# martin-velas/SLAM_plus_plus

Measured on AMD Instinct MI355X. Metric: Lambda solve GFLOP/s (algorithmic factor+solve flops / wall-clock), 100k-pose SE(3), higher is better.
Workload: dtype f64; 1 GPU; C3: synthetic 100000-pose SE(3) chain + loop closures, 6x6 blocks, 201998 upper blocks, n=600000; numeric factor + 2 substitutions per step (symbolic analysis cached, inputs resident in HBM); parallelism=1 GPU

## Files before the change

slam_plus_plus_amd/csrc/simt_factor_ahead.hip:

```cpp
#include <hip/hip_runtime.h>
#include "sparse_kernels.h"

#include <algorithm>

namespace slampp {

#include "simt_device.inl"

template <int D, int AHEAD>
struct TFactorAheadSet {
	double d[D][D];
	double b[D];
	double c[AHEAD][D / 2][D];
};

template <int D, int AHEAD>
constexpr int factor_ahead_fetch_loads()
{
	int n = D / 2;
	for(int r = 0; r < D; ++ r)
		n += r / 2 + 1;
	return n + AHEAD * (D / 2) * D;
}
template <int D> constexpr int factor_ahead_half_block_stores() { return D * ((D / 2) / 2 + (D / 2) % 2); }
template <int D> constexpr int factor_ahead_diagonal_stores() { return D / 2 + (D / 2) * (D / 2); }
template <int D> constexpr int factor_ahead_newer_stores() { return (factor_ahead_half_block_stores<D>() < factor_ahead_diagonal_stores<D>())? factor_ahead_half_block_stores<D>() : factor_ahead_diagonal_stores<D>(); }

template <int D, int AHEAD>
__device__ __forceinline__ void factor_ahead_pin(TFactorAheadSet<D, AHEAD> &s)
{
	#pragma unroll
	for(int r = 0; r < D; ++ r) {
		#pragma unroll
		for(int q = 0; q < 2 * (r / 2 + 1); ++ q)
			asm volatile("" : "+a"(s.d[r][q]));
		asm volatile("" : "+a"(s.b[r]));
	}
	#pragma unroll
	for(int k = 0; k < AHEAD; ++ k) {
		#pragma unroll
		for(int i = 0; i < D / 2; ++ i) {
			#pragma unroll
			for(int q = 0; q < D; ++ q)
				asm volatile("" : "+a"(s.c[k][i][q]));
		}
	}
}

template <int D, int W, int AHEAD>
__device__ __forceinline__ void factor_ahead_fetch(TFactorAheadSet<D, AHEAD> &s, int ci, int n_blk, int nb, int f_blk, int r0, const long long *T,
	const double *__restrict__ A, const double *__restrict__ b)
{
	{
		const long long enc = T[W * (f_blk + n_blk)];
		long long n_off = (enc < 0)? 0 : (enc >> 1);
		asm volatile("" : "+v"(n_off));
		const double *src = A + n_off;
		#pragma unroll
		for(int r = 0; r < D; ++ r) {
			#pragma unroll
			for(int i = 0; i <= r / 2; ++ i) {
				const double2 t = *reinterpret_cast<const double2*>(src + r * D + 2 * i);
				s.d[r][2 * i] = t.x;
				s.d[r][2 * i + 1] = t.y;
			}
		}
		load_column<D>(b + T[W * (4 * ci + 3)], s.b);
	}
	#pragma unroll
	for(int k = 0; k < AHEAD; ++ k) {
		const bool b_exists = k + 1 < nb;
		const long long enc = T[W * (f_blk + n_blk + (b_exists? k + 1 : 0))];
		const bool b_trans = b_exists && enc >= 0 && (enc & 1) != 0;
		long long n_off = (b_exists && enc >= 0)? (enc >> 1) : 0;
		int n_row_stride = b_trans? D : 1, n_col_stride = b_trans? 1 : D;
		asm volatile("" : "+v"(n_off), "+v"(n_row_stride), "+v"(n_col_stride));
		const double *src = A + n_off + r0 * n_row_stride;
		#pragma unroll
		for(int i = 0; i < D / 2; ++ i) {
			#pragma unroll
			for(int q = 0; q < D; ++ q)
				s.c[k][i][q] = src[i * n_row_stride + q * n_col_stride];
		}
	}
	asm volatile("" ::: "memory");
}

template <int D>
__device__ __forceinline__ void store_half_columns(double *p, const double (&m)[D][D], int n_half)
{
	double *p_out = p + n_half * (D / 2) * D;
	#pragma unroll
	for(int q = 0; q < D / 2; ++ q) {
		#pragma unroll
		for(int r = 0; r < D; r += 2)
			*reinterpret_cast<double2*>(p_out + r + q * D) = double2{n_half? m[r][q + D / 2] : m[r][q], n_half? m[r + 1][q + D / 2] : m[r + 1][q]};
	}
}

__device__ __forceinline__ void factor_ahead_stage_table(long long *p_dst, const long long *__restrict__ p_src, int n_entries, int n_lane)
{
	enum { N_FLIGHT = 8 };
	for(int n_base = 0; n_base < n_entries; n_base += N_FLIGHT * 64) {
		long long v[N_FLIGHT];
		#pragma unroll
		for(int u = 0; u < N_FLIGHT; ++ u) {
			const int i = n_base + u * 64 + n_lane;
			v[u] = p_src[(i < n_entries)? i : n_entries - 1];
		}
		#pragma unroll
		for(int u = 0; u < N_FLIGHT; ++ u) {
			const int i = n_base + u * 64 + n_lane;
			if(i < n_entries)
				p_dst[i] = v[u];
		}
	}
}

template <int D, int W, bool b_linv, int AHEAD>
__device__ __forceinline__ bool factor_ahead_columns(const int32_t *P, const long long *T, const int n_half, const double *__restrict__ A, double *L, double *Linv,
	const double *__restrict__ b, double *w, long long *p_tm, int &n_tm)
{
	enum { DD = D * D, DH = D / 2 };
	const int r0 = n_half * DH;
	const int n_cols = P[0], n_blocks = P[1], n_ops = P[2];
	const int f_blk = 4 * n_cols, f_op = f_blk + n_blocks, f_y = f_op + n_ops;
	int pc = 4, blk0 = 0;
	bool b_bad = false;
	TFactorAheadSet<D, AHEAD> t_set;
	factor_ahead_fetch<D, W, AHEAD>(t_set, 0, 0, P[pc], f_blk, r0, T, A, b);
	__builtin_amdgcn_s_waitcnt(simt_wait_imm(0));
	factor_ahead_pin<D, AHEAD>(t_set);
	for(int ci = 0; ci < n_cols; ++ ci) {
		const int nb = P[pc], nr = P[pc + 1], n_touch = P[pc + 2];
		pc += 3;
		pc += n_touch;
		const long long l_base = T[W * (4 * ci)], linv_off = T[W * (4 * ci + 1)], cs_new = T[W * (4 * ci + 2)];
		__builtin_amdgcn_s_waitcnt(simt_wait_imm(factor_ahead_newer_stores<D>()));
		factor_ahead_pin<D, AHEAD>(t_set);
		double a[D][D], y[D], acc[AHEAD][DH][D];
		{
			const long long enc = T[W * (f_blk + blk0)];
			#pragma unroll
			for(int r = 0; r < D; ++ r) {
				#pragma unroll
				for(int q = 0; q < D; ++ q)
					a[r][q] = (q <= r && enc >= 0)? t_set.d[r][q] : 0.0;
			}
			#pragma unroll
			for(int r = 0; r < D; ++ r)
				y[r] = t_set.b[r];
			#pragma unroll
			for(int k = 0; k < AHEAD; ++ k) {
				const bool b_have = k + 1 < nb && T[W * (f_blk + blk0 + ((k + 1 < nb)? k + 1 : 0))] >= 0;
				#pragma unroll
				for(int i = 0; i < DH; ++ i) {
					#pragma unroll
					for(int q = 0; q < D; ++ q)
						acc[k][i][q] = b_have? t_set.c[k][i][q] : 0.0;
				}
			}
		}
		simt_row_entries<D, W>(a, y, pc, nr, f_op, f_y, P, T, L, w);
		SIMT_TICK();
		if(ci + 1 < n_cols) {
			asm volatile("" ::: "memory");
			factor_ahead_fetch<D, W, AHEAD>(t_set, ci + 1, blk0 + nb, P[pc_next_column(P, pc, nb, 0)], f_blk, r0, T, A, b);
		}
		double x[D][D];
		simt_cholesky_inverse<D>(a, x, b_bad);
		{
			double yn[D];
			simt_forward_substitution<D>(yn, a, x, y);
			#pragma unroll
			for(int r = 0; r < D; r += 2)
				*reinterpret_cast<double2*>(w + cs_new + r) = double2{yn[r], yn[r + 1]};
			store_half_columns<D>(L + l_base, a, n_half);
			if constexpr(b_linv)
				store_half_columns<D>(Linv + linv_off, x, n_half);
		}
		SIMT_TICK();
		#pragma unroll
		for(int k = 0; k < AHEAD; ++ k) {
			if(k + 1 < nb) {
				const int np = P[pc ++];
				simt_update_pairs<D, W, 2>(acc[k], pc, np, f_op, r0, P, T, L);
				simt_block_product<D, 2>(acc[k], x, r0, L + l_base + (k + 1) * DD);
				SIMT_TICK();
			}
		}
		for(int kb = AHEAD + 1; kb < nb; ++ kb) {
			const int np = P[pc ++];
			double acc_more[DH][D];
			simt_load_lambda_block<D, 2>(acc_more, T[W * (f_blk + blk0 + kb)], r0, A);
			simt_update_pairs<D, W, 2>(acc_more, pc, np, f_op, r0, P, T, L);
			simt_block_product<D, 2>(acc_more, x, r0, L + l_base + kb * DD);
			SIMT_TICK();
		}
		blk0 += nb;
	}
	return b_bad;
}

template <int D, int W, int LPT, bool b_linv, int AHEAD>
__global__ void __launch_bounds__(64)
factor_simt_kernel_ahead(const TSimtChunk *__restrict__ chunks, const int32_t *__restrict__ prog, const long long *__restrict__ tab,
	const double *__restrict__ A, double *L, double *Linv, const double *__restrict__ b, double *w, int *p_flag,
	long long *p_timing, TBatch t_batch)
{	{ const int64_t n_member = blockIdx.y; A += n_member * t_batch.a; L += n_member * t_batch.l; Linv = Linv? Linv + n_member * t_batch.linv : Linv; b += n_member * t_batch.b; w += n_member * t_batch.w; p_flag += n_member; }

	static_assert(LPT == 2 && D % 2 == 0 && AHEAD >= 1, "two lanes per task, even block sizes");
	enum { DD = D * D, DH = D / 2 };
	extern __shared__ long long s_tab[];
	const TSimtChunk ch = chunks[blockIdx.x];
	{
		const int n_entries = (4 * prog[ch.prog_off] + prog[ch.prog_off + 1] + prog[ch.prog_off + 2] + prog[ch.prog_off + 3]) * W;
		factor_ahead_stage_table(s_tab, tab + ch.tab_off, n_entries, int(threadIdx.x));
		__syncthreads();
	}
	if(int(threadIdx.x) >= W * LPT)
		return;
	const int n_half = int(threadIdx.x) & 1;
	int n_tm = 0;
	long long *p_tm = simt_timing_begin(p_timing, n_tm);
	const bool b_bad = factor_ahead_columns<D, W, b_linv, AHEAD>(prog + ch.prog_off, s_tab + threadIdx.x / LPT, n_half, A, L, Linv, b, w, p_tm, n_tm);
	if(b_bad)
		atomicOr(p_flag, 1);
}

template <int D, int W, bool b_linv, int AHEAD>
__global__ void __launch_bounds__(128)
factor_simt_kernel_branches(const TSimtBranchGroup *__restrict__ groups, const int32_t *__restrict__ prog, const long long *__restrict__ tab,
	const double *__restrict__ A, double *L, double *Linv, const double *__restrict__ b, double *w, int *p_flag,
	long long *p_timing, TBatch t_batch, int n_region)
{	{ const int64_t n_member = blockIdx.y; A += n_member * t_batch.a; L += n_member * t_batch.l; Linv = Linv? Linv + n_member * t_batch.linv : Linv; b += n_member * t_batch.b; w += n_member * t_batch.w; p_flag += n_member; }

	static_assert(D % 2 == 0 && AHEAD >= 1 && W * 2 <= 64, "two lanes per task, even block sizes");
	extern __shared__ long long s_tab[];
	const int n_wave = __builtin_amdgcn_readfirstlane(int(threadIdx.x) >> 6), n_lane = int(threadIdx.x) & 63;
	long long *s_mine = s_tab + n_wave * n_region;
	int n_tm = 0;
	long long *p_tm = simt_timing_begin(p_timing, n_tm);
	bool b_bad = false;
	for(int n_pass = 0; n_pass < 2; ++ n_pass) {
		const TSimtChunk ch = groups[blockIdx.x].seg[n_pass? 2 : n_wave];
		if(ch.n_tasks > 0 && (n_pass == 0 || n_wave == 0)) {
			const int32_t *P = prog + ch.prog_off;
			const int n_entries = (4 * P[0] + P[1] + P[2] + P[3]) * W;
			factor_ahead_stage_table(s_mine, tab + ch.tab_off, n_entries, n_lane);
			__builtin_amdgcn_fence(__ATOMIC_ACQ_REL, "workgroup");
			__builtin_amdgcn_wave_barrier();
			if(n_lane < W * 2) {
				const bool b_bad_here = factor_ahead_columns<D, W, b_linv, AHEAD>(P, s_mine + n_lane / 2, n_lane & 1, A, L, Linv, b, w, p_tm, n_tm);
				b_bad = b_bad || b_bad_here;
			}
		}
		if(n_pass == 0)
			__syncthreads();
	}
	if(b_bad)
		atomicOr(p_flag, 1);
}

template <int W>
static const void *p_Factor_Branches_Kernel(bool b_store_linv)
{
	return b_store_linv? reinterpret_cast<const void*>(&factor_simt_kernel_branches<6, W, true, SIMT_FACTOR_AHEAD>) :
		reinterpret_cast<const void*>(&factor_simt_kernel_branches<6, W, false, SIMT_FACTOR_AHEAD>);
}

static const void *p_Factor_Branches_Kernel(int n_dim, int n_width, bool b_store_linv)
{
	if(n_dim != 6)
		return 0;
	return (n_width == 16)? p_Factor_Branches_Kernel<16>(b_store_linv) : (n_width == 32)? p_Factor_Branches_Kernel<32>(b_store_linv) : 0;
}

bool factor_simt_branches_exists(int n_dim, int n_width)
{
	return p_Factor_Branches_Kernel(n_dim, n_width, false) != 0;
}

int factor_simt_branches_groups(int n_dim, int n_width, int n_lds_bytes)
{
	if(!factor_simt_branches_exists(n_dim, n_width) || n_lds_bytes <= 0)
		return 0;
	return std::min(simt_resident_workgroups(p_Factor_Branches_Kernel(n_dim, n_width, false), 128, n_lds_bytes),
		simt_resident_workgroups(p_Factor_Branches_Kernel(n_dim, n_width, true), 128, n_lds_bytes));
}

bool launch_factor_simt_branches(const TSimtBranchGroup *groups, int n_groups, int n_width, int n_lds_bytes, const int32_t *prog, const int64_t *tab, int n_dim,
	const double *A, double *L, double *Linv, const double *b, double *w, int *p_flag, hipStream_t stream, long long *p_timing, const TBatch &t_batch)
{
	if(!factor_simt_branches_exists(n_dim, n_width) || n_groups <= 0 || n_lds_bytes <= 0 || n_lds_bytes % 16 != 0)
		return false;
	const long long *t = reinterpret_cast<const long long*>(tab);
	const int n_region = n_lds_bytes / 16;
#define BRANCHES_LAUNCH(W_, b_linv_) hipLaunchKernelGGL((factor_simt_kernel_branches<6, W_, b_linv_, SIMT_FACTOR_AHEAD>), dim3(n_groups, t_batch.n), dim3(128), n_lds_bytes, stream, \
	groups, prog, t, A, L, Linv, b, w, p_flag, p_timing, t_batch, n_region)
	if(n_width == 16) {
		if(Linv) BRANCHES_LAUNCH(16, true); else BRANCHES_LAUNCH(16, false);
	} else {
		if(Linv) BRANCHES_LAUNCH(32, true); else BRANCHES_LAUNCH(32, false);
	}
#undef BRANCHES_LAUNCH
	return true;
}

template <int W>
static const void *p_Factor_Ahead_Kernel(bool b_store_linv)
{
	return b_store_linv? reinterpret_cast<const void*>(&factor_simt_kernel_ahead<6, W, 2, true, SIMT_FACTOR_AHEAD>) :
		reinterpret_cast<const void*>(&factor_simt_kernel_ahead<6, W, 2, false, SIMT_FACTOR_AHEAD>);
}

static const void *p_Factor_Ahead_Kernel(int n_dim, int n_width, bool b_store_linv)
{
	if(n_dim != 6)
		return 0;
	return (n_width == 16)? p_Factor_Ahead_Kernel<16>(b_store_linv) : (n_width == 32)? p_Factor_Ahead_Kernel<32>(b_store_linv) : 0;
}

bool factor_simt_ahead_exists(int n_dim, int n_width)
{
	return p_Factor_Ahead_Kernel(n_dim, n_width, false) != 0;
}

int factor_simt_ahead_waves(int n_dim, int n_width, int n_lds_bytes)
{
	if(!factor_simt_ahead_exists(n_dim, n_width))
		return 0;
	return std::min(simt_resident_workgroups(p_Factor_Ahead_Kernel(n_dim, n_width, false), 64, n_lds_bytes),
		simt_resident_workgroups(p_Factor_Ahead_Kernel(n_dim, n_width, true), 64, n_lds_bytes));
}

bool launch_factor_simt_ahead(const TSimtChunk *chunks, int n_chunks, int n_width, int n_lds_bytes, const int32_t *prog, const int64_t *tab, int n_dim,
	const double *A, double *L, double *Linv, const double *b, double *w, int *p_flag, hipStream_t stream, long long *p_timing, const TBatch &t_batch)
{
	if(!factor_simt_ahead_exists(n_dim, n_width))
		return false;
	const long long *t = reinterpret_cast<const long long*>(tab);
#define AHEAD_LAUNCH(W_, b_linv_) hipLaunchKernelGGL((factor_simt_kernel_ahead<6, W_, 2, b_linv_, SIMT_FACTOR_AHEAD>), dim3(n_chunks, t_batch.n), dim3(64), n_lds_bytes, stream, \
	chunks, prog, t, A, L, Linv, b, w, p_flag, p_timing, t_batch)
	if(n_width == 16) {
		if(Linv) AHEAD_LAUNCH(16, true); else AHEAD_LAUNCH(16, false);
	} else {
		if(Linv) AHEAD_LAUNCH(32, true); else AHEAD_LAUNCH(32, false);
	}
#undef AHEAD_LAUNCH
	return true;
}

}

#include "preload.h"
SLAMPP_PRELOAD_UNIT(simt_factor_ahead)
```

slam_plus_plus_amd/csrc/simt_kernel.hip:

```cpp
#include <hip/hip_runtime.h>
#include "sparse_kernels.h"

#include <algorithm>
#include <cstdio>

namespace slampp {

#include "simt_device.inl"

template <int D, int W, int LPT, bool b_linv>
__global__ void __launch_bounds__(64)
factor_simt_kernel(const TSimtChunk *__restrict__ chunks, const int32_t *__restrict__ prog, const long long *__restrict__ tab,
	const double *__restrict__ A, double *L, double *Linv, const double *__restrict__ b, double *w, int *p_flag,
	long long *p_timing, TBatch t_batch)
{	{ const int64_t n_member = blockIdx.y; A += n_member * t_batch.a; L += n_member * t_batch.l; Linv = Linv? Linv + n_member * t_batch.linv : Linv; b += n_member * t_batch.b; w += n_member * t_batch.w; p_flag += n_member; }

	enum { DD = D * D };
	extern __shared__ long long s_tab[];
	const TSimtChunk ch = chunks[blockIdx.x];
	{
		const int n_entries = (4 * prog[ch.prog_off] + prog[ch.prog_off + 1] + prog[ch.prog_off + 2] + prog[ch.prog_off + 3]) * W;
		for(int i = threadIdx.x; i < n_entries; i += 64)
			s_tab[i] = tab[ch.tab_off + i];
		__syncthreads();
	}
	if(int(threadIdx.x) >= W * LPT)
		return;
	const int n_half = (LPT == 2)? int(threadIdx.x) & 1 : 0;
	enum { DH = (LPT == 2)? D / 2 : D };
	const int r0 = n_half * DH;
	int n_tm = 0;
	long long *p_tm = simt_timing_begin(p_timing, n_tm);
	const int32_t *P = prog + ch.prog_off;
	const long long *T = s_tab + threadIdx.x / LPT;
	const int n_cols = P[0], n_blocks = P[1], n_ops = P[2];
	const int f_blk = 4 * n_cols, f_op = f_blk + n_blocks, f_y = f_op + n_ops;
	int pc = 4, blk0 = 0;
	bool b_bad = false;
	double f_touched = 0;
	for(int ci = 0; ci < n_cols; ++ ci) {
		const int nb = P[pc], nr = P[pc + 1], n_touch = P[pc + 2];
		pc += 3;
		pc += n_touch;
		if(ci + 1 < n_cols) {
			const int nb_next = P[pc_next_column(P, pc, nb, nr)];
			for(int kb = 0; kb < nb_next; ++ kb) {
				const long long enc = T[W * (f_blk + blk0 + nb + kb)];
				const double *p_src = A + ((enc < 0)? 0 : (enc >> 1));
				f_touched += p_src[0] + p_src[16] + p_src[DD - 1];
			}
		}
		const long long l_base = T[W * (4 * ci)], linv_off = T[W * (4 * ci + 1)], cs_new = T[W * (4 * ci + 2)],
			cs_src = T[W * (4 * ci + 3)];
		double a[D][D], y[D];
		{
			const long long enc = T[W * (f_blk + blk0)];
			const double *src = A + ((enc < 0)? 0 : (enc >> 1));
			#pragma unroll
			for(int r = 0; r < D; ++ r) {
				double c[D];
				load_column<D>(src + r * D, c);
				#pragma unroll
				for(int q = 0; q < D; ++ q)
					a[r][q] = (q <= r && enc >= 0)? c[q] : 0.0;
			}
			load_column<D>(b + cs_src, y);
		}
		simt_row_entries<D, W>(a, y, pc, nr, f_op, f_y, P, T, L, w);
		SIMT_TICK();
		double x[D][D];
		simt_cholesky_inverse<D>(a, x, b_bad);
		{
			double yn[D];
			simt_forward_substitution<D>(yn, a, x, y);
			if(n_half == 0) {
				#pragma unroll
				for(int r = 0; r < D; ++ r)
					w[cs_new + r] = yn[r];
				store_block<D>(L + l_base, a);
				if constexpr(b_linv)
					store_block<D>(Linv + linv_off, x);
			}
		}
		SIMT_TICK();
		for(int kb = 1; kb < nb; ++ kb) {
			const int np = P[pc ++];
			double acc[DH][D];
			simt_load_lambda_block<D, LPT>(acc, T[W * (f_blk + blk0 + kb)], r0, A);
			simt_update_pairs<D, W, LPT>(acc, pc, np, f_op, r0, P, T, L);
			double *p_out = L + l_base + kb * DD;
			if constexpr(D % 2 == 0)
				simt_block_product<D, LPT>(acc, x, r0, p_out);
			else {
				static_assert(LPT == 1, "odd D: one lane per task, the lane has all D rows of the block");
				#pragma unroll
				for(int q = 0; q < D; ++ q) {
					double out[D];
					#pragma unroll
					for(int r = 0; r < D; ++ r) {
						double sum = 0;
						#pragma unroll
						for(int t = 0; t <= q; ++ t)
							sum += acc[r][t] * x[q][t];
						out[r] = sum;
					}
					#pragma unroll
					for(int r = 0; r < D; ++ r)
						p_out[r + q * D] = out[r];
				}
			}
			SIMT_TICK();
		}
		blk0 += nb;
	}
	if(b_bad || f_touched == 1.2345e301)
		atomicOr(p_flag, 1);
}

bool launch_factor_simt(const TSimtChunk *chunks, int n_chunks, int n_width, int n_lds_bytes, const int32_t *prog, const int64_t *tab, int n_dim,
	const double *A, double *L, double *Linv, const double *b, double *w, int *p_flag, hipStream_t stream, long long *p_timing, const TBatch &t_batch,
	int n_ahead_waves, const TSimtBranchLaunch *p_branches)
{
	if(n_chunks <= 0)
		return true;
	const long long *t = reinterpret_cast<const long long*>(tab);
#define SIMT_LAUNCH(D_, W_, LPT_) do { if(Linv) hipLaunchKernelGGL((factor_simt_kernel<D_, W_, LPT_, true>), dim3(n_chunks, t_batch.n), dim3(64), n_lds_bytes, stream, chunks, prog, t, \
	A, L, Linv, b, w, p_flag, p_timing, t_batch); else hipLaunchKernelGGL((factor_simt_kernel<D_, W_, LPT_, false>), dim3(n_chunks, t_batch.n), dim3(64), n_lds_bytes, stream, chunks, prog, t, \
	A, L, Linv, b, w, p_flag, p_timing, t_batch); } while(0)
#define SIMT_WIDTHS(D_) do { if(n_width == 16) { if(b_pairs && D_ % 2 == 0) SIMT_LAUNCH(D_, 16, (D_ % 2 == 0)? 2 : 1); else SIMT_LAUNCH(D_, 16, 1); } \
	else if(n_width == 32) { if(b_pairs && D_ % 2 == 0) SIMT_LAUNCH(D_, 32, (D_ % 2 == 0)? 2 : 1); else SIMT_LAUNCH(D_, 32, 1); } \
	else SIMT_LAUNCH(D_, 64, 1); } while(0)
	const int n_pairs_env = dev_knob("SLAMPP_HIP_DEV_SIMT_PAIRS", -1);
	const bool b_pairs = (n_pairs_env >= 0)? n_pairs_env != 0 : n_chunks <= 2048;
	const int n_ahead_env = dev_knob("SLAMPP_HIP_DEV_SIMT_FACTOR_AHEAD", -1);
	const int n_lpt = (b_pairs && n_dim % 2 == 0 && (n_width == 16 || n_width == 32))? 2 : 1;
	const bool b_ahead = n_lpt == 2 && factor_simt_ahead_exists(n_dim, n_width) &&
		((n_ahead_env >= 0)? n_ahead_env != 0 : int64_t(n_chunks) * std::max<int64_t>(t_batch.n, 1) <= n_ahead_waves);
	const int n_branches_env = dev_knob("SLAMPP_HIP_DEV_SIMT_FACTOR_BRANCHES", -1);
	const bool b_branches = p_branches && p_branches->n_groups > 0 && n_lpt == 2 && factor_simt_branches_exists(n_dim, n_width) &&
		((n_branches_env >= 0)? n_branches_env != 0 : b_ahead && int64_t(p_branches->n_groups) * std::max<int64_t>(t_batch.n, 1) <= p_branches->n_round_groups &&
		p_branches->n_tstar < p_branches->n_longest_task && p_branches->n_stage_tasks >= 2048);
	if(b_branches) {
		if(p_timing)
			fprintf(stderr, "stage_timing lane-per-task factor branches launch: %d workgroups of two waves, %d split chunks, %d whole chunks, width %d, block size %d, %d members\n",
				p_branches->n_groups, p_branches->n_split_chunks, p_branches->n_whole_chunks, n_width, n_dim, int(t_batch.n));
		return launch_factor_simt_branches(p_branches->groups, p_branches->n_groups, n_width, p_branches->n_lds_bytes, prog, tab, n_dim, A, L, Linv, b, w, p_flag,
			stream, p_timing, t_batch);
	}
	if(p_timing)
		fprintf(stderr, "stage_timing lane-per-task factor launch: %d chunks, width %d, block size %d, %d members, LPT %d, %s\n", n_chunks, n_width, n_dim,
			int(t_batch.n), n_lpt, b_ahead? "fetch ahead" : "fetch by column");
	if(b_ahead)
		return launch_factor_simt_ahead(chunks, n_chunks, n_width, n_lds_bytes, prog, tab, n_dim, A, L, Linv, b, w, p_flag, stream, p_timing, t_batch);
	switch(n_dim) {
	case 3:
		SIMT_WIDTHS(3);
		return true;
	case 6:
		SIMT_WIDTHS(6);
		return true;
	case 7:
		SIMT_WIDTHS(7);
		return true;
	default:
		return false;
	}
#undef SIMT_WIDTHS
#undef SIMT_LAUNCH
}

template <int D, int W>
__global__ void __launch_bounds__(64)
backward_simt_kernel(const TSimtChunk *__restrict__ chunks, const int32_t *__restrict__ prog, const long long *__restrict__ tab,
	const double *__restrict__ L, double *w, double *x_out, TBatch t_batch)
{	{ const int64_t n_member = blockIdx.y; L += n_member * t_batch.l; w += n_member * t_batch.w; x_out += n_member * t_batch.b; }

	enum { DD = D * D };
	extern __shared__ long long s_tab[];
	const TSimtChunk ch = chunks[blockIdx.x];
	const int32_t *P = prog + ch.prog_off;
	const int n_cols = P[0], n_below = P[1];
	{
		const int n_entries = (3 * n_cols + n_below) * W;
		for(int i = threadIdx.x; i < n_entries; i += 64)
			s_tab[i] = tab[ch.tab_off + i];
		__syncthreads();
	}
	if(int(threadIdx.x) >= W)
		return;
	const long long *T = s_tab + threadIdx.x;
	double *s_x = reinterpret_cast<double*>(s_tab + (3 * n_cols + n_below) * W) + threadIdx.x;
	const int32_t *p_local = P + 2 + n_cols;
	int n_blk_end = n_below;
	double f_touched = 0;
	for(int ci = n_cols - 1; ci >= 0; -- ci) {
		const int nb = P[2 + ci];
		const long long l_base = T[W * (3 * ci)], cs_new = T[W * (3 * ci + 1)], cs_src = T[W * (3 * ci + 2)];
		const int n_blk0 = n_blk_end - (nb - 1);
		double acc[D], a[D][D];
		load_column<D>(w + cs_new, acc);
		load_block<D>(L + l_base, a);
		asm volatile("" ::: "memory");
		double f_touch_now = 0;
		if(ci > 1 || (ci == n_cols - 1 && ci > 0)) {
			const int c_first = (ci > 1)? ci - 2 : ci - 1, c_last = (ci == n_cols - 1)? ci - 1 : c_first;
			for(int c = c_last; c >= c_first; -- c) {
				const int nb_next = P[2 + c];
				const double *p_next = L + T[W * (3 * c)];
				for(int kb = 0; kb < nb_next; ++ kb)
					f_touch_now += p_next[kb * DD] + p_next[kb * DD + 16] + p_next[kb * DD + DD - 1];
			}
		}
		asm volatile("" ::: "memory");
		double rd[D];
		#pragma unroll
		for(int q = 0; q < D; ++ q)
			rd[q] = simt_refined_rcp(a[q][q]);
		for(int kb = 1; kb < nb; ++ kb) {
			const long long xcs = T[W * (3 * n_cols + n_blk0 + kb - 1)];
			const int n_local = p_local[n_blk0 + kb - 1];
			double c[D][D], xi[D];
			load_block<D>(L + l_base + kb * DD, c);
			if(n_local >= 0)
				simt_local_x<D, W>(xi, s_x, n_local);
			else
				load_column<D>(w + xcs, xi);
			simt_backward_block<D>(acc, c, xi);
		}
		double x[D];
		simt_solve_transposed<D>(x, acc, a, rd);
		simt_store_local_x<D, W>(s_x, ci, x);
		f_touched += f_touch_now;
		simt_store_x<D>(w + cs_new, x_out + cs_src, x);
		n_blk_end = n_blk0;
	}
	if(f_touched == 1.2345e301)
		w[0] = f_touched;
}

template <int D, int AHEAD>
struct TBwdAheadSet {
	double y[D], a[D][D], c[AHEAD][D][D], xs[D];
	int nb, n_blk0;
	int n_xk;
	int n_local[AHEAD];
};

template <int D, int W, int AHEAD>
__device__ __forceinline__ void bwd_ahead_fetch(TBwdAheadSet<D, AHEAD> &s, int ci, int n_blk_end, int n_cols, const int32_t *P, const int32_t *p_local,
	const long long *T, const double *__restrict__ L, const double *w)
{
	enum { DD = D * D };
	s.nb = P[2 + ci];
	const long long l_base = T[W * (3 * ci)];
	s.n_blk0 = n_blk_end - (s.nb - 1);
	load_column<D>(w + T[W * (3 * ci + 1)], s.y);
	load_lower<D>(L + l_base, s.a);
	s.n_xk = -1;
	int n_x_field = 3 * ci + 1;
	#pragma unroll
	for(int k = 0; k < AHEAD; ++ k) {
		const bool b_have = k + 1 < s.nb;
		s.n_local[k] = b_have? p_local[s.n_blk0 + k] : 0;
		if(b_have && s.n_local[k] < 0 && s.n_xk < 0) {
			s.n_xk = k;
			n_x_field = 3 * n_cols + s.n_blk0 + k;
		}
		int n_blk_off = b_have? (k + 1) * DD : 0;
		asm volatile("" : "+s"(n_blk_off));
		load_block<D>(L + l_base + n_blk_off, s.c[k]);
	}
	asm volatile("" : "+s"(n_x_field));
	load_column<D>(w + T[W * n_x_field], s.xs);
	asm volatile("" ::: "memory");
}

template <int D, int AHEAD>
constexpr int bwd_ahead_fetch_loads()
{
	if(D % 2 != 0)
		return D + D * (D + 1) / 2 + AHEAD * (D * D) + D;
	int n = D / 2;
	for(int q = 0; q < D; ++ q)
		n += (D - (q & ~1)) / 2;
	return n + AHEAD * (D * D / 2) + D / 2;
}
template <int D> constexpr int bwd_ahead_solve_stores() { return (D % 2 == 0)? D : 2 * D; }

template <int D, int W, int AHEAD, int N_NEWER >
__device__ __forceinline__ void bwd_ahead_solve(TBwdAheadSet<D, AHEAD> &s, int ci, int n_cols, const int32_t *p_local, const long long *T, double *s_x,
	const double *__restrict__ L, double *w, double *x_out)
{
	enum { DD = D * D };
	__builtin_amdgcn_s_waitcnt(simt_wait_imm(N_NEWER));
	#pragma unroll
	for(int q = 0; q < D; ++ q)
		s.a[q][q] = simt_refined_rcp(s.a[q][q]);
	double acc[D];
	#pragma unroll
	for(int q = 0; q < D; ++ q)
		acc[q] = s.y[q];
	#pragma unroll
	for(int k = 0; k < AHEAD; ++ k) {
		if(k + 1 < s.nb) {
			double xi[D];
			if(s.n_local[k] >= 0)
				simt_local_x<D, W>(xi, s_x, s.n_local[k]);
			else if(s.n_xk == k) {
				#pragma unroll
				for(int r = 0; r < D; ++ r)
					xi[r] = s.xs[r];
			} else {
				load_column<D>(w + T[W * (3 * n_cols + s.n_blk0 + k)], xi);
				__builtin_amdgcn_s_waitcnt(simt_wait_imm(0));
			}
			simt_backward_block<D>(acc, s.c[k], xi);
		}
	}
	const long long l_base = (s.nb > AHEAD + 1)? T[W * (3 * ci)] : 0;
	for(int kb = AHEAD + 1; kb < s.nb; kb += AHEAD) {
		double xr[AHEAD][D];
		#pragma unroll
		for(int i = 0; i < AHEAD; ++ i) {
			if(kb + i < s.nb) {
				load_block<D>(L + l_base + (kb + i) * DD, s.c[i]);
				const int n_local = p_local[s.n_blk0 + kb + i - 1];
				if(n_local >= 0)
					simt_local_x<D, W>(xr[i], s_x, n_local);
				else
					load_column<D>(w + T[W * (3 * n_cols + s.n_blk0 + kb + i - 1)], xr[i]);
			}
		}
		asm volatile("" ::: "memory");
		__builtin_amdgcn_s_waitcnt(simt_wait_imm(0));
		#pragma unroll
		for(int i = 0; i < AHEAD; ++ i) {
			if(kb + i < s.nb)
				simt_backward_block<D>(acc, s.c[i], xr[i]);
		}
	}
	double x[D];
	#pragma unroll
	for(int q = D - 1; q >= 0; -- q) {
		double sum = acc[q];
		#pragma unroll
		for(int r = q + 1; r < D; ++ r)
			sum -= s.a[q][r] * x[r];
		x[q] = sum * s.a[q][q];
	}
	simt_store_local_x<D, W>(s_x, ci, x);
	const long long cs_new = T[W * (3 * ci + 1)], cs_src = T[W * (3 * ci + 2)];
	simt_store_x<D>(w + cs_new, x_out + cs_src, x);
}

template <int D, int W, int AHEAD>
__global__ void __launch_bounds__(64)
backward_simt_ahead_kernel(const TSimtChunk *__restrict__ chunks, const int32_t *__restrict__ prog, const long long *__restrict__ tab,
	const double *__restrict__ L, double *w, double *x_out, TBatch t_batch)
{	{ const int64_t n_member = blockIdx.y; L += n_member * t_batch.l; w += n_member * t_batch.w; x_out += n_member * t_batch.b; }

	extern __shared__ long long s_tab[];
	const TSimtChunk ch = chunks[blockIdx.x];
	const int32_t *P = prog + ch.prog_off;
	const int n_cols = P[0], n_below = P[1];
	{
		const int n_entries = (3 * n_cols + n_below) * W;
		for(int i = threadIdx.x; i < n_entries; i += 64)
			s_tab[i] = tab[ch.tab_off + i];
		__syncthreads();
	}
	if(int(threadIdx.x) >= W)
		return;
	const long long *T = s_tab + threadIdx.x;
	double *s_x = reinterpret_cast<double*>(s_tab + (3 * n_cols + n_below) * W) + threadIdx.x;
	const int32_t *p_local = P + 2 + n_cols;
	TBwdAheadSet<D, AHEAD> t_even, t_odd;
	enum { N_FETCH = bwd_ahead_fetch_loads<D, AHEAD>(), N_STORES = bwd_ahead_solve_stores<D>() };
	int ci = n_cols - 1;
	bwd_ahead_fetch<D, W, AHEAD>(t_even, ci, n_below, n_cols, P, p_local, T, L, w);
	for(; ci >= 2; ci -= 2) {
		bwd_ahead_fetch<D, W, AHEAD>(t_odd, ci - 1, t_even.n_blk0, n_cols, P, p_local, T, L, w);
		bwd_ahead_solve<D, W, AHEAD, N_FETCH>(t_even, ci, n_cols, p_local, T, s_x, L, w, x_out);
		bwd_ahead_fetch<D, W, AHEAD>(t_even, ci - 2, t_odd.n_blk0, n_cols, P, p_local, T, L, w);
		bwd_ahead_solve<D, W, AHEAD, N_STORES + N_FETCH>(t_odd, ci - 1, n_cols, p_local, T, s_x, L, w, x_out);
	}
	if(ci == 1) {
		bwd_ahead_fetch<D, W, AHEAD>(t_odd, 0, t_even.n_blk0, n_cols, P, p_local, T, L, w);
		bwd_ahead_solve<D, W, AHEAD, N_FETCH>(t_even, 1, n_cols, p_local, T, s_x, L, w, x_out);
		bwd_ahead_solve<D, W, AHEAD, N_STORES>(t_odd, 0, n_cols, p_local, T, s_x, L, w, x_out);
	} else
		bwd_ahead_solve<D, W, AHEAD, 0>(t_even, 0, n_cols, p_local, T, s_x, L, w, x_out);
}

template <int D> struct TBwdAheadDim { enum { b_have = (D == 6) }; };

template <int D, int W>
static const void *p_Backward_Ahead_Kernel()
{
	if constexpr(TBwdAheadDim<D>::b_have)
		return reinterpret_cast<const void*>(&backward_simt_ahead_kernel<D, W, SIMT_BWD_AHEAD>);
	else
		return 0;
}

static const void *p_Backward_Ahead_Kernel(int n_dim, int n_width)
{
#define BWD_AHEAD_WIDTHS(D_) return (n_width == 16)? p_Backward_Ahead_Kernel<D_, 16>() : (n_width == 32)? p_Backward_Ahead_Kernel<D_, 32>() : p_Backward_Ahead_Kernel<D_, 64>()
	switch(n_dim) {
	case 3:
		BWD_AHEAD_WIDTHS(3);
	case 6:
		BWD_AHEAD_WIDTHS(6);
	case 7:
		BWD_AHEAD_WIDTHS(7);
	default:
		return 0;
	}
#undef BWD_AHEAD_WIDTHS
}

template <int D, int W>
static void Launch_Backward_Simt(bool b_ahead, const TSimtChunk *chunks, int n_chunks, int n_lds_bytes, const int32_t *prog, const long long *t,
	const double *L, double *w, double *x_out, hipStream_t stream, const TBatch &t_batch)
{
	if constexpr(TBwdAheadDim<D>::b_have) {
		if(b_ahead) {
			hipLaunchKernelGGL((backward_simt_ahead_kernel<D, W, SIMT_BWD_AHEAD>), dim3(n_chunks, t_batch.n), dim3(64), n_lds_bytes, stream,
				chunks, prog, t, L, w, x_out, t_batch);
			return;
		}
	}
	hipLaunchKernelGGL((backward_simt_kernel<D, W>), dim3(n_chunks, t_batch.n), dim3(64), n_lds_bytes, stream, chunks, prog, t, L, w, x_out, t_batch);
}

int backward_simt_ahead_waves(int n_dim, int n_width, int n_lds_bytes)
{
	return simt_resident_workgroups(p_Backward_Ahead_Kernel(n_dim, n_width), 64, n_lds_bytes);
}

bool launch_backward_simt(const TSimtChunk *chunks, int n_chunks, int n_width, int n_lds_bytes, size_t n_lds_limit, int n_ahead_waves, const int32_t *prog, const int64_t *tab,
	int n_dim, const double *L, double *w, double *x_out, hipStream_t stream, const TBatch &t_batch, bool b_report)
{
	if(n_chunks <= 0)
		return true;
	if(n_lds_bytes < 0 || size_t(n_lds_bytes) > n_lds_limit)
		return false;
	const long long *t = reinterpret_cast<const long long*>(tab);
	const int n_ahead_env = dev_knob("SLAMPP_HIP_DEV_SIMT_BWD_AHEAD", -1);
	const void *p_ahead = p_Backward_Ahead_Kernel(n_dim, n_width);
	const bool b_ahead = p_ahead && ((n_ahead_env >= 0)? n_ahead_env != 0 : int64_t(n_chunks) * std::max<int64_t>(t_batch.n, 1) <= n_ahead_waves);
	if(b_report)
		fprintf(stderr, "stage_timing lane-per-task backward launch: %d chunks, width %d, block size %d, %d members, %s\n", n_chunks, n_width, n_dim,
			int(t_batch.n), b_ahead? "fetch ahead" : "fetch by column");
#define BWD_LAUNCH(D_, W_) Launch_Backward_Simt<D_, W_>(b_ahead, chunks, n_chunks, n_lds_bytes, prog, t, L, w, x_out, stream, t_batch)
#define BWD_WIDTHS(D_) do { if(n_width == 16) BWD_LAUNCH(D_, 16); else if(n_width == 32) BWD_LAUNCH(D_, 32); else BWD_LAUNCH(D_, 64); } while(0)
	switch(n_dim) {
	case 3:
		BWD_WIDTHS(3);
		break;
	case 6:
		BWD_WIDTHS(6);
		break;
	case 7:
		BWD_WIDTHS(7);
		break;
	default:
		return false;
	}
#undef BWD_WIDTHS
#undef BWD_LAUNCH
	return hipGetLastError() == hipSuccess;
}

template <int D>
__global__ void invert_diagonals_kernel(TDevPlan p, int64_t col_begin, int64_t col_end, const double *__restrict__ L, double *Linv)
{
	const int64_t c = col_begin + int64_t(blockIdx.x) * blockDim.x + threadIdx.x;
	if(c >= col_end)
		return;
	const TColDesc &cd = p.cols[c];
	const double *a = L + p.blks[cd.k0].loff;
	double x[D][D];
	#pragma unroll
	for(int q = 0; q < D; ++ q) {
		#pragma unroll
		for(int r = 0; r < D; ++ r) {
			if(r < q)
				x[r][q] = 0.0;
			else {
				double sum = (r == q)? 1.0 : 0.0;
				#pragma unroll
				for(int t = q; t < r; ++ t)
					sum -= a[r + t * D] * x[t][q];
				x[r][q] = sum / a[r + r * D];
			}
		}
	}
	double *p_out = Linv + cd.linv_off;
	#pragma unroll
	for(int q = 0; q < D; ++ q) {
		#pragma unroll
		for(int r = 0; r < D; ++ r)
			p_out[r + q * D] = x[r][q];
	}
}

bool launch_invert_diagonals(const TDevPlan &p, int64_t col_begin, int64_t col_end, const double *L, double *Linv, hipStream_t stream)
{
	if(col_end <= col_begin)
		return true;
	const unsigned n_grid = unsigned((col_end - col_begin + 127) / 128);
	switch(p.uniform_dim) {
	case 3:
		hipLaunchKernelGGL((invert_diagonals_kernel<3>), dim3(n_grid), dim3(128), 0, stream, p, col_begin, col_end, L, Linv);
		return true;
	case 6:
		hipLaunchKernelGGL((invert_diagonals_kernel<6>), dim3(n_grid), dim3(128), 0, stream, p, col_begin, col_end, L, Linv);
		return true;
	case 7:
		hipLaunchKernelGGL((invert_diagonals_kernel<7>), dim3(n_grid), dim3(128), 0, stream, p, col_begin, col_end, L, Linv);
		return true;
	default:
		return false;
	}
}

}

#include "preload.h"
SLAMPP_PRELOAD_UNIT(simt_kernel)
```

slam_plus_plus_amd/csrc/solver.h:

```cpp
#pragma once
#include <hip/hip_runtime.h>
#include <chrono>
#include <cstdint>
#include <new>
#include <stdexcept>
#include <string>
#include <vector>
#include <thread>
#include <memory>
#include <mutex>

#include "../../include/slampp_hip.h"
#include "plan.h"
#include "host_pool.h"
#include "sparse_records.h"
#include <utility>
#include "sparse_kernels.h"
#include "dense_chol.h"

namespace slampp {

struct CDeviceError : public std::runtime_error {
	explicit CDeviceError(const std::string &s) :std::runtime_error(s) {}
};

#define SLAMPP_HIP_CHECK(call) do { hipError_t e_ = (call); if(e_ != hipSuccess) { \
	throw slampp::CDeviceError(std::string(#call) + ": " + hipGetErrorString(e_)); } } while(0)

extern thread_local bool g_b_keep_device_memory;

template <class T>
class CDevArray {
	T *m_p;
	size_t m_n, m_cap;
public:
	CDevArray() :m_p(0), m_n(0), m_cap(0) {}
	~CDevArray() { Release(); }
	CDevArray(const CDevArray&) = delete;
	CDevArray &operator =(const CDevArray&) = delete;
	void Release() { if(m_p) (void)hipFree(m_p); m_p = 0; m_n = 0; m_cap = 0; }
	void Free() { m_n = 0; if(!g_b_keep_device_memory) Release(); }
	void Alloc(size_t n)
	{
		if(!n)
			n = 1;
		if(n <= m_cap && m_p) {
			m_n = std::max(m_n, n);
			return;
		}
		Release();
		hipError_t e = hipMalloc((void**)&m_p, n * sizeof(T));
		if(e == hipErrorOutOfMemory || e == hipErrorMemoryAllocation) {
			(void)hipGetLastError();
			m_p = 0;
			throw std::bad_alloc();
		}
		if(e != hipSuccess) {
			m_p = 0;
			throw CDeviceError(std::string("hipMalloc: ") + hipGetErrorString(e));
		}
		m_n = m_cap = n;
	}
	template <class CAlloc>
	void Upload(const std::vector<T, CAlloc> &v, hipStream_t s)
	{
		Alloc(v.size());
		if(!v.empty())
			SLAMPP_HIP_CHECK(hipMemcpyAsync(m_p, v.data(), v.size() * sizeof(T), hipMemcpyHostToDevice, s));
	}
	T *p() const { return m_n? m_p : 0; }
	size_t n() const { return m_n; }
	size_t n_Bytes() const { return m_p? m_n * sizeof(T) : 0; }
	void Swap(CDevArray &r_other) { std::swap(m_p, r_other.m_p); std::swap(m_n, r_other.m_n); std::swap(m_cap, r_other.m_cap); }
};


struct CKeepDeviceMemory {
	bool b_before;
	CKeepDeviceMemory() :b_before(g_b_keep_device_memory) { g_b_keep_device_memory = true; }
	~CKeepDeviceMemory() { g_b_keep_device_memory = b_before; }
};

struct CSchurState;
struct CDeviceGroup;
struct CSparseInverse;
struct CCovariance;
struct CAssemblyState;
struct CMultiplyState;
struct CPatternOuterState;

}

struct slampp_hip_assembly {
	slampp_hip_solver *p_solver;
	slampp::CAssemblyState *p_state;
	bool b_stale;
	bool b_robust = false;
	slampp_hip_robust t_robust;
	slampp::CDevArray<double> d_robust_weight;
};

struct slampp_hip_solver {
	int n_device;
	hipStream_t stream;
	std::string s_error;
	slampp::PlanOptions opt;
	int n_dense_nb;
	int b_shard_primary;
	int n_shard_rank, n_shard_world;
	int n_marginals_dense;
	int n_assembly_groups = 1 << 20;
	int n_schur_tiles = -1;
	int n_schur_incremental = 0;
	int n_schur_keep = 0;
	int n_schur_sparse;

	bool b_has_structure, b_analyzed, b_factored;
	uint64_t n_factor_gen = 0, n_schur_cov_gen = 0;
	uint64_t n_schur_keep_gen = 0;
	void Factor_Installed(bool b_resolvable = true) { b_factored = b_resolvable; ++ n_factor_gen; }
	void Factor_Dropped() { Factor_Installed(false); }
	void Schur_Kept() { n_schur_keep_gen = n_factor_gen; }
	void Schur_Cov_Left() { n_schur_cov_gen = n_factor_gen; }
	slampp::CMultiplyState *p_mul = 0;
	bool b_mul_valid = false;
	int n_multiply_long_row = SLAMPP_HIP_MULTIPLY_LONG_ROW;
	slampp::CDevArray<double> d_reduce, d_refine_r, d_mul_x, d_mul_y, d_refine_resid;
	slampp::CDevArray<double> d_gram;
	void Require_Multiply();
	slampp::CPatternOuterState *p_outer = 0;
	bool b_outer_valid = false;
	slampp::CDevArray<double> d_outer_out;
	void Require_Pattern_Outer();
	slampp::CDevArray<int64_t> d_logdet_tab;
	std::vector<int64_t> logdet_tab_host;
	bool b_logdet_valid = false;
	void Require_Logdet_Table();
	int n_mode;
	int64_t n_matrix_cut;
	std::vector<int64_t> cumsum, bcol_ptr;
	std::vector<int32_t> brow;
	int64_t n_values, n_scalars;

	bool b_refined = false;
	int64_t n_refined_values = 0;
	std::vector<int64_t> refined_cumsum, refined_bcol_ptr;
	std::vector<int32_t> refined_brow;
	slampp::CDevArray<int64_t> d_refine_map;
	slampp::CDevArray<double> d_refined;
	void Refine_Structure();
	bool b_schur_fallback = false;
	int n_staging_ahead = 0;
	int n_schur_fallback_option = 1;
	slampp::Plan plan;
	slampp::SparseLaunchLists lists;
	slampp::TDevPlan dplan;
	slampp::CDevArray<slampp::TColDesc> d_cols;
	slampp::CDevArray<slampp::TBlkDesc> d_blks;
	slampp::CDevArray<slampp::TRowEnt> d_rents;
	slampp::CDevArray<longlong2> d_pairs;
	slampp::CDevArray<int64_t> d_task_ptr, d_task_pkg;
	slampp::CDevArray<longlong2> d_pkg;
	slampp::CDevArray<long long> d_timing;
	slampp::CDevArray<slampp::TSimtChunk> d_simt_chunks;
	slampp::CDevArray<int32_t> d_simt_prog, d_simt_rest;
	int n_panel = -1;
	int n_panel_rows = -1;
	slampp::CDevArray<longlong2> d_panel_pkg;
	slampp::CDevArray<int64_t> d_panel_off, d_panel_out_off;
	slampp::CDevArray<double> d_handup;
	int n_panel_handup = 1;
	slampp::CDevArray<int32_t> d_panel_rest;
	int n_panel_backward = -1;
	size_t n_lds_limit = 0;
	slampp::CDevArray<longlong2> d_bwd_rec;
	slampp::CDevArray<int64_t> d_bwd_off;
	slampp::CDevArray<slampp::TUpdSlot> d_panel_upd_slots;
	slampp::CDevArray<slampp::TUpdEnt> d_panel_upd_ents;
	slampp::CDevArray<int64_t> d_simt_tab;
	slampp::CDevArray<slampp::TSimtChunk> d_simt_bwd_chunks;
	slampp::CDevArray<int32_t> d_simt_bwd_prog;
	slampp::CDevArray<int64_t> d_simt_bwd_tab;
	std::vector<int32_t> simt_factor_ahead_waves;
	slampp::CDevArray<slampp::TSimtBranchGroup> d_simt_br_groups;
	std::vector<int32_t> simt_branches_round_groups;
	std::vector<int32_t> simt_bwd_ahead_waves;
	bool b_leaf_linv_wanted = false, b_leaf_linv_valid = true;
	slampp::TBatch t_batch = slampp::t_No_Batch();
	slampp::CDevArray<double> d_batch_L, d_batch_Linv, d_batch_w, d_batch_handup;
	slampp::CDevArray<int> d_batch_flag;
	int n_batch_owner_member = -1;
	int *p_host_batch_flag = 0;
	int n_batch_pending = 0;
	int n_simt_backward = -1;
	void Ensure_Leaf_Inverses();
	int n_simt = -1;
	int n_wide_min_tasks = 8192;
	int n_simt_width = 32;
	int n_simt_stages = 1;
	void Upload_Simt(const slampp::SparseRecords &r_rec);
	void Report_Simt_Backward(const slampp::SparseRecords &r_rec) const;
	void Report_Simt_Factor(const slampp::SparseRecords &r_rec) const;
	slampp::CDevArray<slampp::TDenseBlk> d_dense_blks;
	slampp::CDevArray<int64_t> d_dense_blk_loff;
	slampp::CDevArray<double> d_dense, d_dense_invdiag, d_dense_z, d_dense_x;
	slampp::CDevArray<int32_t> d_dense_gaps;
	int n_dense_gaps;
	slampp::CDevArray<uint8_t> d_dense_unit;
	slampp::CDevArray<longlong2> d_dense_dst;
	slampp::CTileSchedule dense_tiles;
	bool b_dense_tiles;
	bool b_dense_clean;
	int n_dense_top_tiles;
	int n_dense_blks, n_dense_cols, n_dense_dim, n_dense_pad;
	slampp::CDevArray<double> d_A, d_rhs, d_L, d_Linv, d_w, d_cov;
	slampp::CSparseInverse *p_sinv = 0;
	bool b_sinv_tried = false;
	slampp::CCovariance *p_cov = 0;
	slampp::CDevArray<double> d_Z;
	slampp::CDevArray<double> d_Zd, d_Zd_work;
	slampp::CDevArray<int64_t> d_diag_zoff;
	slampp::CDevArray<int32_t> d_diag_dim;
	slampp::CDevArray<int64_t> d_diag_out_off;
	slampp::CDevArray<int64_t> d_damp_off;
	bool b_damp_valid = false;
	bool Require_Damping_Offsets();
	slampp::CDevArray<double> d_lm_reduce;
	slampp::CDevArray<int64_t> d_state_cumsum;
	bool b_state_cumsum_valid = false;
	slampp::CDevArray<int> d_flag;
	int *p_flag_shared = 0;
	int *p_host_flag;

	double *p_pin_values = 0, *p_pin_rhs = 0;
	size_t n_pin_values = 0, n_pin_rhs = 0;
	bool b_pin_values_registered = false, b_pin_rhs_registered = false;
	bool b_pin_values_deferred = false, b_pin_rhs_deferred = false;
	bool b_staging_ever = false;
	std::thread t_staging_registration;
	void Register_Staging_Later();
	void Join_Staging_Registration();
	slampp::CTrashList analysis_trash;
	std::thread t_discard;
	void Join_Discard() { if(t_discard.joinable()) t_discard.join(); }
	std::thread t_bringup;
	std::mutex m_bringup;
	int n_bringup_status = SLAMPP_HIP_OK;
	int n_Join_Bringup()
	{
		std::lock_guard<std::mutex> t_lock(m_bringup);
		if(t_bringup.joinable()) {
			const double t0 = slampp::wall_ms();
			t_bringup.join();
			if(getenv("SLAMPP_HIP_PLAN_TIMING"))
				fprintf(stderr, "[bring-up] waited for %.2f ms\n", slampp::wall_ms() - t0);
		}
		return n_bringup_status;
	}
	void Join_Bringup()
	{
		if(n_Join_Bringup() != SLAMPP_HIP_OK)
			throw slampp::CDeviceError("the handle's streams could not be created");
	}
	hipStream_t copy_stream = 0;
	hipEvent_t copy_done = 0;
	int64_t n_uploaded = 0;
	void Require_Staging();
	void Free_Staging();
	void Upload_Values(const double *p_values);

	slampp::CSchurState *p_schur;
	slampp::CDeviceGroup *p_group = 0;
	bool b_group_active = false;
	std::vector<int> group_devices;
	std::vector<std::pair<std::string, int64_t> > group_options;
	std::vector<slampp_hip_assembly*> assemblies;

	slampp_hip_allreduce_fn p_allreduce;
	void *p_allreduce_context;
	typedef int (*TDenseFactorFn)(void *p_context, double *p_S, int n_pad, int n, double *p_invdiag, int *p_flag, void *p_hip_stream);
	TDenseFactorFn p_dense_factor = 0;
	void *p_dense_factor_context = 0;
	int n_schur_distributed = 0;

	slampp_hip_times times;

	struct TPhaseRecord { int n_label; hipEvent_t start, stop; };
	int b_profile;
	std::vector<std::string> phase_names;
	std::vector<double> phase_ms;
	std::vector<int64_t> phase_count;
	std::vector<TPhaseRecord> phase_pending;
	std::vector<hipEvent_t> event_pool;
	int n_open_phase;
	void Phase_Begin(const char *p_s_label);
	void Phase_End();
	void Phase_Collect();

	slampp_hip_solver();
	~slampp_hip_solver();
	void Free_Device(bool b_keep_multiply = false);
	size_t n_Device_Bytes() const;
	void Analyze_Sparse();
	void Enqueue_Sparse(const double *p_values_dev, double *p_rhs_dev, bool b_factor, bool b_factor_only = false);
};


namespace slampp {

void schur_destroy(CSchurState *p);
CSchurState *schur_analyze(slampp_hip_solver &s);
void schur_enqueue(slampp_hip_solver &s, const double *p_values_dev, double *p_rhs_dev);
bool schur_keeps_for_resolve(const slampp_hip_solver &s);
void schur_resolve_enqueue(slampp_hip_solver &s, double *p_rhs_dev, bool b_from_covariance);
void schur_enqueue_marginal_poses(slampp_hip_solver &s, const double *p_values_dev, double *p_rhs_dev);
void damping_enqueue(const int64_t *p_off_dim_dev, int64_t n_first, int64_t n_last, double f_alpha, double *p_values_dev,
	hipStream_t stream);
void schur_enqueue_marginals(slampp_hip_solver &s, const double *p_values_dev, double *p_cam_cov_dev, double *p_point_cov_dev);
void schur_cov_pattern_enqueue(slampp_hip_solver &s, const double *p_values_dev, double *p_cov_dev);
void schur_cov_columns_enqueue(slampp_hip_solver &s, const double *p_values_dev, int n_cols, const int64_t *p_bcols, double *p_out_dev);
void schur_cov_pairs_enqueue(slampp_hip_solver &s, const double *p_values_dev, int64_t n_pairs, const int64_t *p_brows,
	const int64_t *p_bcols, double *p_out_dev);
size_t schur_device_bytes(const CSchurState *p);
void schur_invalidate_previous(CSchurState *p);
void schur_set_changed_points(slampp_hip_solver &s, const int64_t *p_points, int64_t n_points);
void schur_fill_stats(const CSchurState *p, slampp_hip_stats &st);
bool schur_reduced_stats(const CSchurState *p, slampp_hip_stats &st);

CDeviceGroup *group_create(const int *p_device_ids, int n_devices);
void group_destroy(CDeviceGroup *p_group);
int group_set_option(CDeviceGroup &g, const char *p_s_name, int64_t n_value);
void group_analyze(slampp_hip_solver &r_front, int64_t n_cut);
int group_factor_solve(slampp_hip_solver &r_front, const double *p_values, double *p_rhs_inout);
int group_check_staging(slampp_hip_solver &r_front, double *p_values, double *p_rhs);
int group_solve_marginal_poses(slampp_hip_solver &r_front, const double *p_values, double *p_rhs_inout);
int group_schur_marginals(slampp_hip_solver &r_front, const double *p_values, double *p_cam_cov, double *p_point_cov);
int group_free_memory(CDeviceGroup &g);
void group_fill_stats(CDeviceGroup &g, slampp_hip_stats &r_stats);
const char *group_exchange_name(const CDeviceGroup &g);
int group_member_num(const CDeviceGroup &g);
int64_t group_exchange_count(const CDeviceGroup &g);
slampp_hip_solver *group_member(CDeviceGroup &g, int n_member);
void shard_bounds(int64_t n_bcols, int64_t n_cut, const int64_t *p_bcol_ptr, int n_world, std::vector<int64_t> &r_bounds);

CAssemblyState *assembly_setup(slampp_hip_solver &s, int64_t n_edges, const int64_t *v0, const int64_t *v1, int rd);
void assembly_destroy(CAssemblyState *p);
void assembly_enqueue(CAssemblyState &a, const double *J0, const double *J1, const double *Si, const double *err,
	const double *wgt, int64_t n_unary_vertex, const double *p_unary_factor, const double *p_unary_error,
	double *values_out, double *eta_out, int b_accumulate);
size_t assembly_device_bytes(const CAssemblyState *p);
struct TAsmEdgeView {
	int64_t n_edges;
	int d0, d1, rd;
	const int64_t *p_state_off0, *p_state_off1, *p_vertex0;
};
void assembly_edge_view(const CAssemblyState &a, TAsmEdgeView &r_view);

}

void Parallel_Copy(double *p_dst, const double *p_src, size_t n);
void Upload_Rhs_And_Join(slampp_hip_solver &s, const double *p_rhs);
void Upload_Values_And_Join(slampp_hip_solver &s, const double *p_values);
```

slam_plus_plus_amd/csrc/solver.hip:

```cpp
#include <execinfo.h>
#include <signal.h>
#include <unistd.h>
#include <pthread.h>
#include "solver.h"
#include <unordered_map>
#include <sys/mman.h>
#include "sparse_inverse.h"
#include "covariance.h"
#include "multiply.h"
#include "pattern_outer.h"

#include <algorithm>
#include <atomic>
#include <chrono>
#include <cstdio>
#include <cstdlib>
#include <cstring>
#include <map>
#include <thread>
#include <mutex>
#include <condition_variable>
#include <functional>
#include <sys/mman.h>

using namespace slampp;

namespace slampp {
thread_local bool g_b_keep_device_memory = false;
}

slampp_hip_solver::slampp_hip_solver()
	:n_device(0), stream(0), n_dense_nb(64), b_shard_primary(1), n_shard_rank(-1), n_shard_world(0), n_marginals_dense(0), n_schur_sparse(-1), b_has_structure(false),
	b_analyzed(false), b_factored(false), n_mode(SLAMPP_HIP_MODE_SPARSE), n_matrix_cut(0),
	n_values(0), n_scalars(0), n_dense_gaps(0), b_dense_tiles(false), b_dense_clean(false), n_dense_top_tiles(-1), n_dense_blks(0), n_dense_cols(0),
	n_dense_dim(0), n_dense_pad(0),
	p_host_flag(0), p_schur(0), p_allreduce(0), p_allreduce_context(0),
	b_profile(0), n_open_phase(-1)
{
	memset(&dplan, 0, sizeof(dplan));
	memset(&times, 0, sizeof(times));
}

slampp_hip_solver::~slampp_hip_solver()
{
	(void)n_Join_Bringup();
	Join_Discard();
	host_pool_release();
	Free_Device();
	for(size_t i = 0; i < phase_pending.size(); ++ i) {
		(void)hipEventDestroy(phase_pending[i].start);
		(void)hipEventDestroy(phase_pending[i].stop);
	}
	for(size_t i = 0; i < event_pool.size(); ++ i)
		(void)hipEventDestroy(event_pool[i]);
	if(p_host_flag)
		(void)hipHostFree(p_host_flag);
	if(p_host_batch_flag)
		(void)hipHostFree(p_host_batch_flag);
	Free_Staging();
	if(copy_done)
		(void)hipEventDestroy(copy_done);
	if(copy_stream)
		(void)hipStreamDestroy(copy_stream);
	if(stream)
		(void)hipStreamDestroy(stream);
}

void slampp_hip_solver::Free_Device(bool b_keep_multiply)
{
	d_cols.Free(); d_blks.Free(); d_rents.Free(); d_pairs.Free(); d_task_ptr.Free(); d_task_pkg.Free(); d_pkg.Free();
	d_simt_chunks.Free(); d_simt_prog.Free(); d_simt_rest.Free(); d_simt_tab.Free();
	d_simt_bwd_chunks.Free(); d_simt_bwd_prog.Free(); d_simt_bwd_tab.Free(); d_simt_br_groups.Free();
	b_leaf_linv_valid = true;
	d_panel_pkg.Free(); d_panel_off.Free(); d_panel_out_off.Free(); d_handup.Free(); d_panel_rest.Free(); d_bwd_rec.Free(); d_bwd_off.Free(); d_panel_upd_slots.Free(); d_panel_upd_ents.Free();
	lists = SparseLaunchLists();
	d_dense_blks.Free(); d_dense_blk_loff.Free(); d_dense.Free(); d_dense_invdiag.Free(); d_dense_z.Free(); d_dense_x.Free();
	n_dense_blks = n_dense_cols = n_dense_dim = n_dense_pad = 0;
	dense_tiles.Free();
	b_dense_tiles = false;
	d_dense_gaps.Free(); d_dense_unit.Free(); d_dense_dst.Free();
	n_dense_gaps = 0;
	d_A.Free(); d_rhs.Free(); d_L.Free(); d_Linv.Free(); d_w.Free(); d_flag.Free();
	d_cov.Free(); d_damp_off.Free(); d_timing.Free();
	d_refine_map.Free(); d_refined.Free();
	b_damp_valid = false;
	d_state_cumsum.Free();
	b_state_cumsum_valid = false;
	dplan.p_timing = 0;
	n_uploaded = 0;
	if(p_sinv) {
		sparse_inverse_destroy(p_sinv);
		p_sinv = 0;
	}
	b_sinv_tried = false;
	if(p_cov) {
		covariance_destroy(p_cov);
		p_cov = 0;
	}
	d_Z.Free(); d_diag_zoff.Free(); d_diag_dim.Free(); d_diag_out_off.Free(); d_Zd.Free(); d_Zd_work.Free();
	if(p_schur) {
		schur_destroy(p_schur);
		p_schur = 0;
	}
	if(p_mul && !b_keep_multiply) {
		multiply_destroy(p_mul);
		p_mul = 0;
		b_mul_valid = false;
	}
	if(p_outer && !b_keep_multiply) {
		pattern_outer_destroy(p_outer);
		p_outer = 0;
		b_outer_valid = false;
	}
	d_outer_out.Free();
	d_logdet_tab.Free();
	std::vector<int64_t>().swap(logdet_tab_host);
	b_logdet_valid = false;
	d_reduce.Free(); d_lm_reduce.Free(); d_gram.Free(); d_refine_r.Free(); d_mul_x.Free(); d_mul_y.Free(); d_refine_resid.Free();
	b_analyzed = false;
	Factor_Dropped();
}

size_t slampp_hip_solver::n_Device_Bytes() const
{
	return d_dense_blks.n_Bytes() + d_dense_unit.n_Bytes() + d_dense_dst.n_Bytes() + d_dense.n_Bytes() + d_dense_invdiag.n_Bytes() + dense_tiles.n_Bytes() +
		d_dense_z.n_Bytes() + d_dense_x.n_Bytes() + d_cols.n_Bytes() + d_blks.n_Bytes() + d_rents.n_Bytes() +
		d_task_ptr.n_Bytes() + d_task_pkg.n_Bytes() + d_pkg.n_Bytes() + d_pairs.n_Bytes() + d_A.n_Bytes() +
		d_simt_chunks.n_Bytes() + d_simt_prog.n_Bytes() + d_simt_rest.n_Bytes() + d_simt_tab.n_Bytes() +
		d_simt_bwd_chunks.n_Bytes() + d_simt_bwd_prog.n_Bytes() + d_simt_bwd_tab.n_Bytes() + d_simt_br_groups.n_Bytes() +
		d_panel_pkg.n_Bytes() + d_panel_off.n_Bytes() + d_panel_out_off.n_Bytes() + d_handup.n_Bytes() + d_panel_rest.n_Bytes() + d_bwd_rec.n_Bytes() + d_bwd_off.n_Bytes() + d_panel_upd_slots.n_Bytes() + d_panel_upd_ents.n_Bytes() +
		d_rhs.n_Bytes() + d_L.n_Bytes() + d_Linv.n_Bytes() + d_w.n_Bytes() + d_cov.n_Bytes() + d_flag.n_Bytes() +
		d_Z.n_Bytes() + d_diag_zoff.n_Bytes() + d_Zd.n_Bytes() + d_Zd_work.n_Bytes() + sparse_inverse_bytes(p_sinv) + covariance_bytes(p_cov) +
		(p_schur? schur_device_bytes(p_schur) : 0) + multiply_device_bytes(p_mul) + pattern_outer_device_bytes(p_outer) + d_outer_out.n_Bytes() + d_logdet_tab.n_Bytes() +d_reduce.n_Bytes() + d_lm_reduce.n_Bytes() + d_refine_r.n_Bytes() +
		d_mul_x.n_Bytes() + d_mul_y.n_Bytes() + d_refine_resid.n_Bytes() + d_gram.n_Bytes();
}

void slampp_hip_solver::Phase_Begin(const char *p_s_label)
{
	if(!b_profile)
		return;
	if(b_profile == 3) {
		static const char *p_kept[] = {"factor_leaves", "schur_tiles", "schur_gather", "dense_chol"};
		bool b_kept = false;
		for(size_t i = 0; i < sizeof(p_kept) / sizeof(p_kept[0]); ++ i)
			b_kept = b_kept || !strcmp(p_s_label, p_kept[i]);
		if(!b_kept)
			return;
	}
	int n_label = -1;
	for(size_t i = 0; i < phase_names.size(); ++ i) {
		if(phase_names[i] == p_s_label)
			n_label = int(i);
	}
	if(n_label < 0) {
		n_label = int(phase_names.size());
		phase_names.push_back(p_s_label);
		phase_ms.push_back(0);
		phase_count.push_back(0);
	}
	TPhaseRecord r;
	r.n_label = n_label;
	for(int i = 0; i < 2; ++ i) {
		hipEvent_t e;
		if(!event_pool.empty()) {
			e = event_pool.back();
			event_pool.pop_back();
		} else
			SLAMPP_HIP_CHECK(hipEventCreate(&e));
		(i? r.stop : r.start) = e;
	}
	SLAMPP_HIP_CHECK(hipEventRecord(r.start, stream));
	phase_pending.push_back(r);
	n_open_phase = int(phase_pending.size()) - 1;
}

void slampp_hip_solver::Phase_End()
{
	if(!b_profile || n_open_phase < 0)
		return;
	SLAMPP_HIP_CHECK(hipEventRecord(phase_pending[n_open_phase].stop, stream));
	n_open_phase = -1;
}

void slampp_hip_solver::Phase_Collect()
{
	for(size_t i = 0; i < phase_pending.size(); ++ i) {
		float f_ms = 0;
		if(hipEventElapsedTime(&f_ms, phase_pending[i].start, phase_pending[i].stop) == hipSuccess) {
			phase_ms[phase_pending[i].n_label] += f_ms;
			++ phase_count[phase_pending[i].n_label];
		} else
			(void)hipGetLastError();
		event_pool.push_back(phase_pending[i].start);
		event_pool.push_back(phase_pending[i].stop);
	}
	phase_pending.clear();
}
```

slam_plus_plus_amd/csrc/sparse_enqueue.hip:

```cpp
#include <execinfo.h>
#include <signal.h>
#include <unistd.h>
#include <pthread.h>
#include "solver.h"
#include "sparse_inverse.h"

#include <algorithm>
#include <atomic>
#include <chrono>
#include <cstdio>
#include <cstdlib>
#include <cstring>
#include <map>
#include <thread>
#include <mutex>
#include <condition_variable>
#include <functional>
#include <sys/mman.h>

using namespace slampp;

void slampp_hip_solver::Enqueue_Sparse(const double *p_values_dev, double *p_rhs_dev, bool b_factor, bool b_factor_only)
{
	const Plan &P = plan;
	const int n_stages = int(P.stage_ptr.size()) - 1;
	int *p_flag = p_flag_shared? p_flag_shared : d_flag.p();
	if(b_factor && b_refined) {
		launch_gather_values(d_refine_map.p(), n_refined_values, p_values_dev, d_refined.p(), stream);
		p_values_dev = d_refined.p();
	}
	const bool b_simt_backward_wanted = (n_simt_backward < 0)? P.stage_ptr.size() > 1 && P.stage_ptr[1] - P.stage_ptr[0] >= 12288 : n_simt_backward != 0;
	const bool b_simt_bwd = b_simt_backward_wanted && !lists.simt_chunk_ptr.empty() && d_simt_bwd_chunks.p() &&
		(P.max_dim % 2 != 0 || ((reinterpret_cast<uintptr_t>(p_rhs_dev) & 15) == 0 && t_batch.b % 2 == 0));
	if(b_factor)
		b_leaf_linv_valid = true;
	else
		Ensure_Leaf_Inverses();
	if(b_factor) {
		const bool b_simt = !lists.simt_chunk_ptr.empty() && (P.max_dim % 2 != 0 ||
			(((reinterpret_cast<uintptr_t>(p_values_dev) | reinterpret_cast<uintptr_t>(p_rhs_dev)) & 15) == 0 && (t_batch.a | t_batch.b) % 2 == 0));
		const int n_wide_end = std::min(lists.n_bottom_stages, n_stages);
		bool b_panel_fused = false;
		for(size_t i = 0; i < lists.panel_ride.size(); ++ i)
			b_panel_fused = b_panel_fused || lists.panel_ride[i] != 0;
		b_panel_fused = b_panel_fused || lists.b_any_hand_up;
		auto Launch_Panels = [&](int s, bool b_bottom) {
			const int n_panels = lists.panel_ptr[s + 1] - lists.panel_ptr[s];
			const bool b_rode = lists.panel_ride[s] != 0;
			if(!b_rode)
				launch_panel_update(P.max_dim, d_panel_upd_slots.p() + lists.panel_upd_ptr[s], lists.panel_upd_ptr[s + 1] - lists.panel_upd_ptr[s],
					d_panel_upd_ents.p(), p_values_dev, d_L.p(), p_rhs_dev, d_w.p(), stream, t_batch);
			const int n_next = (s + 1 < n_stages && lists.panel_ride[s + 1] == 1)? lists.panel_upd_ptr[s + 2] - lists.panel_upd_ptr[s + 1] : 0;
			if(!launch_factor_panel(P.max_dim, b_panel_fused, (n_panel_rows < 0)? P.max_dim >= 6 : n_panel_rows != 0, lists.panel_cfg[s], d_panel_pkg.p(), d_panel_off.p() + lists.panel_ptr[s],
				d_panel_out_off.p() + lists.panel_ptr[s], n_panels,
				d_panel_upd_slots.p() + ((n_next > 0)? lists.panel_upd_ptr[s + 1] : 0), n_next, d_panel_upd_ents.p(), p_values_dev, p_rhs_dev,
				d_L.p(), d_Linv.p(), d_w.p(), d_handup.p(), p_flag, stream, dplan.p_timing, t_batch))
				throw CDeviceError("panel launch refused: block size or LDS request outside what the analysis planned for");
			if(lists.panel_rest_ptr[s + 1] > lists.panel_rest_ptr[s]) {
				TDevPlan t_rest = dplan;
				t_rest.task_map = d_panel_rest.p();
				launch_factor_stage(t_rest, p_values_dev, d_L.p(), d_Linv.p(), p_rhs_dev, d_w.p(), lists.panel_rest_ptr[s],
					lists.panel_rest_ptr[s + 1] - lists.panel_rest_ptr[s], b_bottom, p_flag, stream, t_batch);
			}
		};
		for(int s = 0; s < n_stages; ++ s) {
			if(s == 0)
				Phase_Begin("factor_leaves");
			else if(s == 1 && (b_profile >= 2 || n_wide_end <= 1))
				Phase_Begin((s < n_wide_end)? "factor_wide" : "factor_upper");
			else if(s == 1)
				Phase_Begin("factor_rest");
			else if(s == n_wide_end && b_profile >= 2)
				Phase_Begin("factor_upper");
			if(b_simt && s + 1 < int(lists.simt_chunk_ptr.size())) {
				const int n_chunks = lists.simt_chunk_ptr[s + 1] - lists.simt_chunk_ptr[s], n_rest = lists.simt_rest_ptr[s + 1] - lists.simt_rest_ptr[s];
				const bool b_store_linv = b_leaf_linv_wanted || !b_simt_backward_wanted;
				TSimtBranchLaunch t_branches = {0, 0, 0, 0, 0, 0, 0, 0, 0};
				if(size_t(s) < lists.simt_br.size() && size_t(s) < simt_branches_round_groups.size() && lists.simt_br[size_t(s)].n_groups > 0 && d_simt_br_groups.p()) {
					const TSimtBranchStage &r_br = lists.simt_br[size_t(s)];
					const TSimtBranchLaunch t_have = {d_simt_br_groups.p() + r_br.n_first, r_br.n_groups, r_br.n_split_chunks, r_br.n_whole_chunks, r_br.n_lds_bytes,
						simt_branches_round_groups[size_t(s)], r_br.n_tstar, r_br.n_longest_task, r_br.n_stage_tasks};
					t_branches = t_have;
				}
				launch_factor_simt(d_simt_chunks.p() + lists.simt_chunk_ptr[s], n_chunks, n_simt_width, lists.simt_lds_bytes[s], d_simt_prog.p(), d_simt_tab.p(), P.max_dim,
					p_values_dev, d_L.p(), b_store_linv? d_Linv.p() : 0, p_rhs_dev, d_w.p(), p_flag, stream, dplan.p_timing, t_batch,
					(size_t(s) < simt_factor_ahead_waves.size())? simt_factor_ahead_waves[size_t(s)] : 0, t_branches.n_groups? &t_branches : 0);
				b_leaf_linv_valid = b_leaf_linv_valid && b_store_linv;
				if(n_rest > 0) {
					TDevPlan t_rest = dplan;
					t_rest.task_map = d_simt_rest.p();
					launch_factor_stage(t_rest, p_values_dev, d_L.p(), d_Linv.p(), p_rhs_dev, d_w.p(), lists.simt_rest_ptr[s], n_rest,
						true, p_flag, stream, t_batch);
				}
			} else if(s == 0 && !lists.panel_ptr.empty() && lists.panel_ptr[1] > lists.panel_ptr[0]) {
				Launch_Panels(s, true);
			} else if(s > 0 && s < lists.n_bottom_stages && dplan.task_pkg)
				launch_factor_wide(dplan, p_values_dev, d_L.p(), d_Linv.p(), p_rhs_dev, d_w.p(), P.stage_ptr[s],
					P.stage_ptr[s + 1] - P.stage_ptr[s], p_flag, stream, t_batch);
			else if(s >= lists.n_bottom_stages && !lists.panel_ptr.empty()) {
				Launch_Panels(s, false);
			} else
			launch_factor_stage(dplan, p_values_dev, d_L.p(), d_Linv.p(), p_rhs_dev, d_w.p(), P.stage_ptr[s],
				P.stage_ptr[s + 1] - P.stage_ptr[s], s < lists.n_bottom_stages, p_flag, stream, t_batch);
			if(s == 0 || (s == n_wide_end - 1 && b_profile >= 2) || s == n_stages - 1)
				Phase_End();
		}
	} else {
		Phase_Begin("forward");
		for(int s = 0; s < n_stages; ++ s) {
			launch_forward_stage(dplan, d_L.p(), d_Linv.p(), p_rhs_dev, d_w.p(), P.stage_ptr[s],
				P.stage_ptr[s + 1] - P.stage_ptr[s], stream);
		}
		Phase_End();
	}
	if(b_factor_only && !n_dense_dim) {
		SLAMPP_HIP_CHECK(hipGetLastError());
		return;
	}
	if(n_dense_dim) {
		const int ld = n_dense_pad;
		if(b_factor) {
			Phase_Begin("dense_assemble");
			if(b_dense_tiles && b_dense_clean)
				tile_zero(dense_tiles, d_dense.p(), ld, stream, d_dense_unit.p());
			else {
				SLAMPP_HIP_CHECK(hipMemsetAsync(d_dense.p(), 0, size_t(ld) * ld * sizeof(double), stream));
				b_dense_clean = b_dense_tiles;
				dense_prepare_padding(d_dense.p(), ld, n_dense_dim, stream);
				dense_prepare_gaps(d_dense.p(), ld, d_dense_gaps.p(), n_dense_gaps, stream);
			}
			launch_dense_assemble(dplan, d_dense_blks.p(), n_dense_blks, p_values_dev, d_L.p(), p_rhs_dev, d_w.p(),
				d_dense.p(), ld, false, stream);
			Phase_End();
			Phase_Begin("dense_chol");
			if(b_dense_tiles)
				tile_cholesky(dense_tiles, d_dense.p(), ld, n_dense_dim, d_dense_invdiag.p(), p_flag, stream);
			else
				dense_cholesky(d_dense.p(), ld, n_dense_dim, d_dense_invdiag.p(), p_flag, stream);
			Phase_End();
			if(b_factor_only) {
				launch_dense_gather_factor(d_dense_blks.p(), d_dense_blk_loff.p(), n_dense_blks, d_dense.p(), ld, d_L.p(), stream);
				SLAMPP_HIP_CHECK(hipGetLastError());
				return;
			}
		} else {
			Phase_Begin("dense_forward");
			launch_dense_assemble(dplan, d_dense_blks.p(), n_dense_blks, 0, d_L.p(), p_rhs_dev, d_w.p(),
				d_dense.p(), ld, true, stream);
			dense_forwardsolve(d_dense.p(), ld, d_dense_invdiag.p(), stream);
			Phase_End();
		}
		Phase_Begin("dense_solve");
		if(b_dense_tiles)
			tile_backsolve(dense_tiles, d_dense.p(), ld, n_dense_dim, d_dense_invdiag.p(), d_dense_z.p(), d_dense_x.p(), stream,
				d_dense_dst.p(), d_w.p(), p_rhs_dev);
		else
		dense_backsolve(d_dense.p(), ld, n_dense_dim, d_dense_invdiag.p(), d_dense_z.p(), d_dense_x.p(), stream,
			d_dense_dst.p(), d_w.p(), p_rhs_dev);
		Phase_End();
	}
	const bool b_slice_bwd = n_panel_backward != 0 && !lists.panel_ptr.empty() && d_bwd_rec.p() && d_bwd_off.p() &&
		(P.max_dim == 3 || P.max_dim == 6 || P.max_dim == 7) && P.uniform_dim;
	const int n_slice_max_tasks = dev_knob("SLAMPP_HIP_DEV_BWD_SLICE_MAX_TASKS", 1024);
	Phase_Begin("backward");
	for(int s = n_stages; s > 0; -- s) {
		if(b_simt_bwd && s < int(lists.simt_chunk_ptr.size())) {
			const int n_chunks = lists.simt_chunk_ptr[s] - lists.simt_chunk_ptr[s - 1], n_rest = lists.simt_rest_ptr[s] - lists.simt_rest_ptr[s - 1];
			if(!launch_backward_simt(d_simt_bwd_chunks.p() + lists.simt_chunk_ptr[s - 1], n_chunks, n_simt_width, lists.simt_bwd_lds_bytes[s - 1], n_lds_limit,
				(size_t(s - 1) < simt_bwd_ahead_waves.size())? simt_bwd_ahead_waves[s - 1] : 0, d_simt_bwd_prog.p(), d_simt_bwd_tab.p(), P.max_dim, d_L.p(), d_w.p(), p_rhs_dev, stream, t_batch,
				dplan.p_timing != 0))
				throw CDeviceError("lane-per-task backward launch refused: block size or LDS request outside what the analysis planned for");
			if(n_rest > 0) {
				TDevPlan t_rest = dplan;
				t_rest.task_map = d_simt_rest.p();
				launch_backward_stage(t_rest, d_L.p(), d_Linv.p(), d_w.p(), p_rhs_dev, lists.simt_rest_ptr[s - 1], n_rest, stream, t_batch);
			}
			continue;
		}
		if(s < int(lists.simt_chunk_ptr.size()))
			Ensure_Leaf_Inverses();
		if(b_slice_bwd && lists.panel_ptr[s] > lists.panel_ptr[s - 1] && (n_panel_backward > 0 || P.stage_ptr[s] - P.stage_ptr[s - 1] <= n_slice_max_tasks)) {
			if(!launch_backward_slice(P.max_dim, lists.bwd_cfg[s - 1], n_lds_limit, d_bwd_rec.p(), d_bwd_off.p() + lists.panel_ptr[s - 1],
			   lists.panel_ptr[s] - lists.panel_ptr[s - 1], d_L.p(), d_Linv.p(), d_w.p(), p_rhs_dev, stream, t_batch))
				throw CDeviceError("backward slice launch refused: block size or LDS request outside what the analysis planned for");
			if(lists.panel_rest_ptr[s] > lists.panel_rest_ptr[s - 1]) {
				TDevPlan t_rest = dplan;
				t_rest.task_map = d_panel_rest.p();
				launch_backward_stage(t_rest, d_L.p(), d_Linv.p(), d_w.p(), p_rhs_dev, lists.panel_rest_ptr[s - 1],
					lists.panel_rest_ptr[s] - lists.panel_rest_ptr[s - 1], stream, t_batch);
			}
			continue;
		}
		launch_backward_stage(dplan, d_L.p(), d_Linv.p(), d_w.p(), p_rhs_dev, P.stage_ptr[s - 1],
			P.stage_ptr[s] - P.stage_ptr[s - 1], stream, t_batch);
	}
	Phase_End();
	SLAMPP_HIP_CHECK(hipGetLastError());
}
```

slam_plus_plus_amd/csrc/sparse_kernels.h:

```cpp
#pragma once
#include <hip/hip_runtime.h>
#include <stdint.h>
#include "plan.h"

namespace slampp {

struct TBatch {
	int n;
	int64_t a, l, linv, b, w, h;
};
inline TBatch t_No_Batch() { TBatch t = {1, 0, 0, 0, 0, 0, 0}; return t; }



struct TColDesc {
	int64_t k0;
	int32_t nb, dj;
	int64_t linv_off;
	int64_t cs_new;
	int64_t cs_src;
	int64_t r0;
	int32_t nr;
	int32_t np;
	int64_t p0;
};

struct TBlkDesc {
	int64_t loff;
	int64_t asrc;
	int64_t p0;
	uint32_t np_di;
	int32_t xcs;
};

struct TRowEnt {
	int64_t off;
	int32_t ycs;
	int32_t dc;
};

struct TDenseBlk {
	int64_t asrc;
	int64_t p0;
	int64_t dst;
	int64_t r0;
	int32_t np, nr;
	int32_t di, dj;
	int64_t cs_src;
	int32_t pos;
	int32_t pad;
};

struct TDenseCol {
	int64_t cs_new, cs_src;
	int32_t pos, dj;
};

enum { PANEL_W = 8, PANEL_COLS = 8, PANEL_UNITS = 1024, PANEL_UPD_W = 4 };
struct TPanelHead {
	int32_t n_cols, n_slots, n_units, n_int_rows;
	int32_t ext_ptr[12];
};
struct TPanelOut {
	int32_t op0, onp;
	int64_t dst;
};
struct TPanelCol {
	int64_t linv_off, cs_new, cs_src;
	int32_t slot0, nb;
	int32_t ir0, inr;
	int32_t sub, pad;
};
struct TPanelSlot {
	int64_t loff, asrc;
	int32_t ip0, inp;
	int64_t pad;
};
struct TPanelExt {
	int64_t a_off, b_off;
	int32_t ycs;
	uint16_t slot, kind;
	int32_t col;
	int32_t pad;
};
struct TUpdSlot {
	int64_t loff, asrc;
	int64_t e0;
	int32_t ne, kind;
	int64_t cs_src, cs_new;
	int64_t pad[2];
};
struct TUpdEnt {
	int64_t a_off;
	int64_t b_off;
};
inline int panel_slot_cap(int n_dim) { return (n_dim == 6)? 96 : (n_dim == 7)? 72 : 256; }

struct TPanelLaunch {
	int32_t n_waves, n_cap_units, n_cap_blk, n_cap_cols, n_cap_lvl;
	int32_t n_cap_out;
	int32_t b_from_lambda;
};
enum { PANEL_UPD_BATCH = 8 };
inline __host__ __device__ constexpr int panel_fresh_batch(int n_waves) { return (n_waves == 4)? 8 : 4; }
enum { PANEL_FETCH_BLOCKS = 3 };
inline __host__ __device__ constexpr int panel_fetch_pass(int n_waves) { return 2 * panel_fresh_batch(n_waves) / (2 * PANEL_FETCH_BLOCKS) * PANEL_FETCH_BLOCKS; }
inline __host__ __device__ constexpr int panel_fetch_group(int n_waves) { return (n_waves == 2)? 3 * panel_fetch_pass(n_waves) : 2 * panel_fetch_pass(n_waves); }
struct TPanelLds {
	int IMAGE, VEC, LINV, TILE, OPS, YV, OUT, TOTAL;
};
enum { PANEL_LDS_BUDGET = 156 * 1024 };
inline __host__ __device__ TPanelLds panel_lds(int D, bool b_fused, const TPanelLaunch &c)
{
	const int DD = D * D, W = c.n_waves;
	TPanelLds l;
	l.IMAGE = 2 * c.n_cap_units;
	l.VEC = l.IMAGE + c.n_cap_blk * DD;
	l.LINV = l.VEC + c.n_cap_cols * 8;
	l.TILE = l.LINV + c.n_cap_cols * 64;
	l.OPS = l.TILE + W * 64;
	l.YV = l.OPS + (b_fused? W * 2 * panel_fresh_batch(W) * DD : 0);
	l.OUT = l.YV + (b_fused? W * panel_fresh_batch(W) * 8 : 0);
	const int n_panel_end = l.OUT + 2 * c.n_cap_out;
	const int n_upd_end = b_fused? W * 2 * PANEL_UPD_BATCH * DD + W * PANEL_UPD_BATCH * 8 + W * 64 : 0;
	l.TOTAL = (n_panel_end > n_upd_end)? n_panel_end : n_upd_end;
	return l;
}

bool launch_factor_panel(int n_dim, bool b_fused, bool b_rows, const TPanelLaunch &r_cfg, const longlong2 *pkg, const int64_t *pkg_off, const int64_t *out_off,
	int n_tasks, const TUpdSlot *upd_slots, int n_upd_slots, const TUpdEnt *upd_ents, const double *A, const double *b, double *L, double *Linv, double *w,
	double *H, int *p_flag, hipStream_t stream, long long *p_timing = 0, const TBatch &t_batch = t_No_Batch());
void launch_panel_update(int n_dim, const TUpdSlot *slots, int n_slots, const TUpdEnt *ents, const double *A, double *L,
	const double *b, double *w, hipStream_t stream, const TBatch &t_batch = t_No_Batch());

enum { BWD_OFF_BITS = 48 };
struct TBwdHead {
	int32_t n_cols, n_levels, n_blks, n_units;
	int32_t lvl_ptr[PANEL_COLS + 1];
	int32_t pad[3];
};
struct TBwdCol {
	int64_t linv_off, cs_src;
	int32_t cs_new;
	int32_t blk0, nb;
	int32_t level;
};
struct TBwdBlk {
	int64_t loff;
	int32_t xsrc;
	int32_t pad;
};
struct TBwdLaunch {
	int32_t n_waves, n_cols_per_wave, n_cap_units;
};
inline size_t plain_launch_lds_limit()
{
	int n_device = 0, n_bytes = 0;
	if(hipGetDevice(&n_device) != hipSuccess || hipDeviceGetAttribute(&n_bytes, hipDeviceAttributeMaxSharedMemoryPerBlock, n_device) != hipSuccess)
		return 0;
	return size_t((n_bytes < 64 * 1024)? ((n_bytes > 0)? n_bytes : 0) : 64 * 1024);
}
inline size_t backward_slice_lds_bytes(const TBwdLaunch &c) { return size_t(c.n_cap_units) * 16 + PANEL_COLS * 8 * sizeof(double); }
bool launch_backward_slice(int n_dim, const TBwdLaunch &r_cfg, size_t n_lds_limit, const longlong2 *rec, const int64_t *rec_off, int n_tasks,
	const double *L, const double *Linv, double *w, double *x_out, hipStream_t stream, const TBatch &t_batch = t_No_Batch());

enum { UP_CHUNK = 16, UP_NR = 128, UP_NP = 512, WIDE_CHUNK = 8, WIDE_NR = 32, WIDE_NP = 48 };
enum { PKG_SPECULATIVE = 512 };

inline __host__ __device__ int package_units(int nb, int ne)
{
	return 4 + 2 * nb + ne + (ne + 3) / 4 + (ne + 15) / 16;
}

struct TDevPlan {
	const TColDesc *cols;
	const TBlkDesc *blks;
	const longlong2 *pairs;
	const TRowEnt *rents;
	const int64_t *task_ptr;
	int uniform_dim;
	int64_t n_blks, n_pairs, n_rents;
	const longlong2 *pkg;
	const int64_t *task_pkg;
	const int32_t *task_map;
	long long *p_timing;
};

struct TSimtChunk {
	int32_t prog_off;
	int32_t n_tasks;
	int64_t tab_off;
};

bool launch_factor_simt(const TSimtChunk *chunks, int n_chunks, int n_width ,
	int n_lds_bytes ,
	const int32_t *prog, const int64_t *tab, int n_dim,
	const double *A, double *L, double *Linv , const double *b, double *w, int *p_flag, hipStream_t stream,
	long long *p_timing = 0 , const TBatch &t_batch = t_No_Batch(),
	int n_ahead_waves = 0 ,
	const struct TSimtBranchLaunch *p_branches = 0 );
enum { SIMT_FACTOR_AHEAD = 2 };
bool factor_simt_ahead_exists(int n_dim, int n_width);
bool launch_factor_simt_ahead(const TSimtChunk *chunks, int n_chunks, int n_width, int n_lds_bytes, const int32_t *prog, const int64_t *tab, int n_dim,
	const double *A, double *L, double *Linv, const double *b, double *w, int *p_flag, hipStream_t stream, long long *p_timing, const TBatch &t_batch);
int factor_simt_ahead_waves(int n_dim, int n_width, int n_lds_bytes);
struct TSimtBranchGroup {
	TSimtChunk seg[3];
};
struct TSimtBranchLaunch {
	const TSimtBranchGroup *groups;
	int n_groups, n_split_chunks, n_whole_chunks;
	int n_lds_bytes;
	int n_round_groups;
	int n_tstar, n_longest_task, n_stage_tasks;
};
bool factor_simt_branches_exists(int n_dim, int n_width);
int factor_simt_branches_groups(int n_dim, int n_width, int n_lds_bytes);
bool launch_factor_simt_branches(const TSimtBranchGroup *groups, int n_groups, int n_width, int n_lds_bytes, const int32_t *prog, const int64_t *tab, int n_dim,
	const double *A, double *L, double *Linv, const double *b, double *w, int *p_flag, hipStream_t stream, long long *p_timing, const TBatch &t_batch);
enum { SIMT_BWD_AHEAD = 2 };
bool launch_backward_simt(const TSimtChunk *chunks, int n_chunks, int n_width, int n_lds_bytes, size_t n_lds_limit ,
	int n_ahead_waves, const int32_t *prog, const int64_t *tab,
	int n_dim, const double *L, double *w, double *x_out, hipStream_t stream, const TBatch &t_batch = t_No_Batch(), bool b_report = false);
int backward_simt_ahead_waves(int n_dim, int n_width, int n_lds_bytes);
bool launch_invert_diagonals(const TDevPlan &p, int64_t col_begin, int64_t col_end, const double *L, double *Linv, hipStream_t stream);

void launch_factor_stage(const TDevPlan &p, const double *A, double *L, double *Linv, const double *b,
	double *w, int task_begin, int n_tasks, bool b_bottom_stage, int *p_flag, hipStream_t stream, const TBatch &t_batch = t_No_Batch());
bool launch_factor_subtree_image(const TDevPlan &p, const double *A, double *L, double *Linv, const double *b,
	double *w, int task_begin, int n_tasks, int *p_flag, hipStream_t stream, const TBatch &t_batch = t_No_Batch());
void launch_factor_wide(const TDevPlan &p, const double *A, double *L, double *Linv, const double *b,
	double *w, int task_begin, int n_tasks, int *p_flag, hipStream_t stream, const TBatch &t_batch = t_No_Batch());
void launch_forward_stage(const TDevPlan &p, const double *L, const double *Linv, const double *b,
	double *w, int task_begin, int n_tasks, hipStream_t stream);
void launch_backward_stage(const TDevPlan &p, const double *L, const double *Linv, double *w,
	double *x_out, int task_begin, int n_tasks, hipStream_t stream, const TBatch &t_batch = t_No_Batch());

void launch_dense_assemble(const TDevPlan &p, const TDenseBlk *blks, int n_blks, const double *A, const double *L,
	const double *b, const double *w, double *Dm, int ld, bool b_rhs_only, hipStream_t stream);
void launch_dense_gather_factor(const TDenseBlk *blks, const int64_t *loffs, int n_blks, const double *Dm, int ld, double *L, hipStream_t stream);
void launch_gather_values(const int64_t *p_map, int64_t n, const double *p_src, double *p_dst, hipStream_t stream);

}
```

slam_plus_plus_amd/csrc/sparse_records.cpp:

```cpp
#include "sparse_records.h"

#include <climits>
#include <atomic>
#include <cstdio>
#include <cstring>
#include <map>
#include <stdexcept>
#include <unordered_map>

namespace slampp {

static bool b_Package_Dim(const Plan &P)
{
	return P.uniform_dim && (P.max_dim == 3 || P.max_dim == 6 || P.max_dim == 7);
}

int count_bottom_stages(const Plan &P, const SparseRecordOptions &t_opt)
{
	int n_bottom_stages = 1;
	while(n_bottom_stages < int(P.stage_ptr.size()) - 1 &&
	   P.stage_ptr[n_bottom_stages + 1] - P.stage_ptr[n_bottom_stages] > t_opt.n_wide_min_tasks)
		++ n_bottom_stages;
	return n_bottom_stages;
}
// ... 772 lines not shown
			dense_blks.push_back(b);
			r_rec.dense_blk_loff.push_back(P.loff[k]);
		}
	}
	std::vector<char> covered(size_t(P.dense_dim), 0);
	for(size_t k = 0; k < dense_cols.size(); ++ k)
		std::fill(covered.begin() + dense_cols[k].pos, covered.begin() + dense_cols[k].pos + dense_cols[k].dj, char(1));
	for(int32_t q = 0; q < P.dense_dim; ++ q) {
		if(!covered[q])
			r_rec.gaps.push_back(q);
	}
	r_rec.unit.assign(size_t(n_dense_pad), uint8_t(1));
	r_rec.dst.assign(size_t(n_dense_pad), longlong2{-1, -1});
	for(size_t k = 0; k < dense_cols.size(); ++ k) {
		for(int q = 0; q < dense_cols[k].dj; ++ q) {
			r_rec.unit[dense_cols[k].pos + q] = 0;
			r_rec.dst[dense_cols[k].pos + q] = longlong2{(long long)(dense_cols[k].cs_new + q), (long long)(dense_cols[k].cs_src + q)};
		}
	}
}


namespace {

enum { SIMT_MIN_GROUP = 1, SIMT_MAX_PROG = 4096, SIMT_MAX_TABLE_BYTES = 40960 };
struct TSimtTask { int32_t n_task; bool b_fits; uint64_t n_hash; std::vector<int32_t> prog, ops, ys; };
struct TSimtChunkJob { int32_t n_group; size_t n_first; int n_fields, n_bwd_fields; int64_t n_tab_off, n_bwd_tab_off; };

void Simt_Task_Program(const Plan &P, int32_t t, const int32_t *p_cols, int32_t n_cols, size_t W, int32_t *op_index, int32_t *y_index,
	std::vector<int32_t> &touch, std::vector<int32_t> &body, TSimtTask &tt)
{
	std::vector<int32_t> &prog = tt.prog;
	prog.assign(4, 0);
	tt.ops.clear();
	tt.ys.clear();
	tt.n_task = t;
	int32_t n_blocks = 0;
	bool b_fits = true;
	auto op_of = [&](int32_t n_blk) {
		if(op_index[n_blk] < 0) {
			op_index[n_blk] = int32_t(tt.ops.size());
			tt.ops.push_back(n_blk);
		}
		return op_index[n_blk];
	};
	for(int32_t i = 0; i < n_cols && b_fits; ++ i) {
		const int32_t j = p_cols[i];
		const int32_t nb = int32_t(P.lptr[j + 1] - P.lptr[j]), nr = int32_t(P.rptr[j + 1] - P.rptr[j]);
		prog.push_back(nb);
		prog.push_back(nr);
		const size_t n_touch_at = prog.size();
		prog.push_back(0);
		n_blocks += nb;
		touch.clear();
		body.clear();
		auto touch_op = [&](int32_t n_op) {
			if(std::find(touch.begin(), touch.end(), n_op) == touch.end())
				touch.push_back(n_op);
			return n_op;
		};
		for(int64_t e = P.rptr[j]; e < P.rptr[j + 1]; ++ e) {
			const int32_t n_blk = P.rblk[e], c = P.blk_col[n_blk];
			if(y_index[c] < 0) {
				y_index[c] = int32_t(tt.ys.size());
				tt.ys.push_back(c);
			}
			body.push_back(touch_op(op_of(n_blk)));
			body.push_back(y_index[c]);
		}
		for(int64_t k = P.lptr[j] + 1; k < P.lptr[j + 1]; ++ k) {
			body.push_back(int32_t(P.pptr[k + 1] - P.pptr[k]));
			for(int64_t e = P.pptr[k]; e < P.pptr[k + 1]; ++ e) {
				body.push_back(touch_op(op_of(P.pa[e])));
				body.push_back(touch_op(op_of(P.pb[e])));
			}
		}
		prog[n_touch_at] = int32_t(touch.size());
		prog.insert(prog.end(), touch.begin(), touch.end());
		prog.insert(prog.end(), body.begin(), body.end());
		b_fits = prog.size() <= SIMT_MAX_PROG;
	}
	for(size_t k = 0; k < tt.ops.size(); ++ k)
		op_index[tt.ops[k]] = -1;
	for(size_t k = 0; k < tt.ys.size(); ++ k)
		y_index[tt.ys[k]] = -1;
	for(int32_t i = 0; i < n_cols && b_fits; ++ i) {
		const int32_t j = p_cols[i];
		for(int64_t k = P.lptr[j] + 1; k < P.lptr[j + 1]; ++ k) {
			int32_t n_local = -1;
			for(int32_t i2 = i + 1; i2 < n_cols && n_local < 0; ++ i2) {
				if(p_cols[i2] == P.lrow[k])
					n_local = i2;
			}
			prog.push_back(n_local);
		}
	}
	prog[0] = n_cols;
	prog[1] = n_blocks;
	prog[2] = int32_t(tt.ops.size());
	prog[3] = int32_t(tt.ys.size());
	tt.b_fits = b_fits && size_t(4 * n_cols + n_blocks) + tt.ops.size() + tt.ys.size() <= SIMT_MAX_TABLE_BYTES / (8 * W);
	uint64_t h = 0x9e3779b97f4a7c15ull ^ prog.size();
	for(size_t k = 0; k < prog.size(); ++ k) {
		h ^= uint64_t(uint32_t(prog[k])) + 0x9e3779b97f4a7c15ull + (h << 6) + (h >> 2);
		h *= 0xff51afd7ed558ccdull;
	}
	tt.n_hash = h;
}

void Group_Simt_Shapes(const std::vector<TSimtTask> &tasks_all, std::vector<int32_t> &rest, std::vector<std::vector<int32_t> > &groups)
{
	std::unordered_map<uint64_t, std::vector<int32_t> > by_hash;
	for(int32_t n_i = 0; n_i < int32_t(tasks_all.size()); ++ n_i) {
		const TSimtTask &tt = tasks_all[size_t(n_i)];
		if(!tt.b_fits) {
			rest.push_back(tt.n_task);
			continue;
		}
		std::vector<int32_t> &r_shapes = by_hash[tt.n_hash];
		int32_t n_group = -1;
		for(size_t k = 0; k < r_shapes.size() && n_group < 0; ++ k) {
			if(tasks_all[size_t(groups[size_t(r_shapes[k])][0])].prog == tt.prog)
				n_group = r_shapes[k];
		}
		if(n_group < 0) {
			n_group = int32_t(groups.size());
			groups.push_back(std::vector<int32_t>());
			r_shapes.push_back(n_group);
		}
		groups[size_t(n_group)].push_back(n_i);
	}
	std::sort(groups.begin(), groups.end(), [&](const std::vector<int32_t> &r_a, const std::vector<int32_t> &r_b) {
		return tasks_all[size_t(r_a[0])].prog < tasks_all[size_t(r_b[0])].prog; });
}

std::pair<int32_t, int32_t> Layout_Simt_Chunks(const Plan &P, size_t W, const std::vector<TSimtTask> &tasks_all,
	const std::vector<std::vector<int32_t> > &groups, SparseRecords &r_rec, size_t &n_tab_size, size_t &n_bwd_tab_size, std::vector<TSimtChunkJob> &jobs)
{
	int32_t n_stage_lds = 0, n_stage_bwd_lds = 0;
	for(size_t g = 0; g < groups.size(); ++ g) {
		const std::vector<int32_t> &r_members = groups[g];
		const std::vector<int32_t> &prog = tasks_all[size_t(r_members[0])].prog;
		if(r_members.size() < SIMT_MIN_GROUP) {
			for(int32_t n_i : r_members)
				r_rec.simt_rest.push_back(tasks_all[size_t(n_i)].n_task);
			continue;
		}
		const int32_t n_prog_off = int32_t(r_rec.simt_prog.size());
		r_rec.simt_prog.insert(r_rec.simt_prog.end(), prog.begin(), prog.end());
		const int n_cols = prog[0], n_blocks = prog[1], n_ops = prog[2], n_ys = prog[3];
		const int n_fields = 4 * n_cols + n_blocks + n_ops + n_ys;
		n_stage_lds = std::max(n_stage_lds, int32_t(n_fields * W * 8));
		const int32_t n_bwd_prog_off = int32_t(r_rec.simt_bwd_prog.size());
		const int n_bwd_fields = 3 * n_cols + (n_blocks - n_cols);
		n_stage_bwd_lds = std::max(n_stage_bwd_lds, int32_t((n_bwd_fields + n_cols * P.max_dim) * W * 8));
		r_rec.simt_bwd_prog.push_back(n_cols);
		r_rec.simt_bwd_prog.push_back(n_blocks - n_cols);
		{
			const TSimtTask &tt = tasks_all[size_t(r_members[0])];
			for(int64_t i = P.task_ptr[tt.n_task]; i < P.task_ptr[tt.n_task + 1]; ++ i)
				r_rec.simt_bwd_prog.push_back(int32_t(P.lptr[P.task_cols[i] + 1] - P.lptr[P.task_cols[i]]));
			r_rec.simt_bwd_prog.insert(r_rec.simt_bwd_prog.end(), prog.end() - (n_blocks - n_cols), prog.end());
		}
		for(size_t n_first = 0; n_first < r_members.size(); n_first += W) {
			const size_t n_in_chunk = std::min<size_t>(W, r_members.size() - n_first);
			TSimtChunk ch;
			ch.prog_off = n_prog_off;
			ch.n_tasks = int32_t(n_in_chunk);
			ch.tab_off = int64_t(n_tab_size);
			r_rec.simt_chunks.push_back(ch);
			TSimtChunk ch_bwd;
			ch_bwd.prog_off = n_bwd_prog_off;
			ch_bwd.n_tasks = int32_t(n_in_chunk);
			ch_bwd.tab_off = int64_t(n_bwd_tab_size);
			r_rec.simt_bwd_chunks.push_back(ch_bwd);
			TSimtChunkJob t_job = {int32_t(g), n_first, n_fields, n_bwd_fields, ch.tab_off, ch_bwd.tab_off};
			jobs.push_back(t_job);
			n_tab_size += size_t(n_fields) * W;
			n_bwd_tab_size += size_t(n_bwd_fields) * W;
		}
	}
	return std::make_pair(n_stage_lds, n_stage_bwd_lds);
}

int Fill_Simt_Forward_Lane(const Plan &P, size_t W, int64_t *p_tab, int n_lane, const int32_t *p_cols, int32_t n_cols,
	const std::vector<int32_t> &r_ops, const std::vector<int32_t> &r_ys)
{
	int f = 0;
	for(int32_t i = 0; i < n_cols; ++ i) {
		const int32_t j = p_cols[i];
		p_tab[W * (f ++) + n_lane] = P.loff[P.lptr[j]];
		p_tab[W * (f ++) + n_lane] = P.linv_off[j];
		p_tab[W * (f ++) + n_lane] = P.cs_new[j];
		p_tab[W * (f ++) + n_lane] = P.cs_src[j];
	}
	for(int32_t i = 0; i < n_cols; ++ i) {
		const int32_t j = p_cols[i];
		for(int64_t k = P.lptr[j]; k < P.lptr[j + 1]; ++ k)
			p_tab[W * (f ++) + n_lane] = (P.asrc[k] < 0)? -1 : P.asrc[k] * 2 + P.atrans[k];
	}
	for(int32_t n_blk : r_ops)
		p_tab[W * (f ++) + n_lane] = P.loff[n_blk];
	for(int32_t c : r_ys)
		p_tab[W * (f ++) + n_lane] = P.cs_new[c];
	return f;
}

void Fill_Simt_Chunk_Tables(const Plan &P, size_t W, const std::vector<TSimtTask> &tasks_all, const std::vector<std::vector<int32_t> > &groups,
	const TSimtChunkJob &r_job, SparseRecords &r_rec)
{
	const std::vector<int32_t> &r_members = groups[size_t(r_job.n_group)];
	const size_t n_first = r_job.n_first, n_in_chunk = std::min<size_t>(W, r_members.size() - n_first);
	const int n_fields = r_job.n_fields, n_bwd_fields = r_job.n_bwd_fields;
	int64_t *p_tab = &r_rec.simt_tab[size_t(r_job.n_tab_off)];
	for(int n_lane = 0; n_lane < int(W); ++ n_lane) {
		const TSimtTask &tt = tasks_all[size_t(r_members[n_first + std::min<size_t>(n_lane, n_in_chunk - 1)])];
		const int f = Fill_Simt_Forward_Lane(P, W, p_tab, n_lane, P.task_cols.data() + P.task_ptr[tt.n_task],
			int32_t(P.task_ptr[tt.n_task + 1] - P.task_ptr[tt.n_task]), tt.ops, tt.ys);
		if(f != n_fields)
			throw std::logic_error("lane-per-task tables: field count mismatch");
	}
	int64_t *p_bwd = &r_rec.simt_bwd_tab[size_t(r_job.n_bwd_tab_off)];
	for(int n_lane = 0; n_lane < int(W); ++ n_lane) {
		const TSimtTask &tt = tasks_all[size_t(r_members[n_first + std::min<size_t>(n_lane, n_in_chunk - 1)])];
		int f = 0;
		for(int64_t i = P.task_ptr[tt.n_task]; i < P.task_ptr[tt.n_task + 1]; ++ i) {
			const int32_t j = P.task_cols[i];
			p_bwd[W * (f ++) + n_lane] = P.loff[P.lptr[j]];
			p_bwd[W * (f ++) + n_lane] = P.cs_new[j];
			p_bwd[W * (f ++) + n_lane] = P.cs_src[j];
		}
		for(int64_t i = P.task_ptr[tt.n_task]; i < P.task_ptr[tt.n_task + 1]; ++ i) {
			const int32_t j = P.task_cols[i];
			for(int64_t k = P.lptr[j] + 1; k < P.lptr[j + 1]; ++ k) {
				if(P.loff[k] != P.loff[P.lptr[j]] + (k - P.lptr[j]) * int64_t(P.max_dim) * P.max_dim)
					throw std::logic_error("lane-per-task tables: the blocks of a column are not contiguous");
				p_bwd[W * (f ++) + n_lane] = P.cs_new[P.lrow[k]];
			}
		}
		if(f != n_bwd_fields)
			throw std::logic_error("lane-per-task tables: backward field count mismatch");
	}
}

}

void simt_task_parents(const Plan &P, int32_t t, std::vector<int32_t> &r_parent)
{
	const int32_t *p_cols = P.task_cols.data() + P.task_ptr[t];
	const int32_t n_cols = int32_t(P.task_ptr[t + 1] - P.task_ptr[t]);
	r_parent.assign(size_t(n_cols), -1);
	for(int32_t i = 0; i < n_cols; ++ i) {
		const int32_t j = p_cols[i];
		for(int64_t k = P.lptr[j] + 1; k < P.lptr[j + 1]; ++ k) {
			for(int32_t i2 = i + 1; i2 < n_cols && (r_parent[size_t(i)] < 0 || i2 < r_parent[size_t(i)]); ++ i2) {
				if(p_cols[i2] == P.lrow[k])
					r_parent[size_t(i)] = i2;
			}
		}
	}
}

int32_t simt_task_segments(const std::vector<int32_t> &r_parent, TSimtSegments &r_seg)
{
	const int32_t n = int32_t(r_parent.size());
	std::vector<int32_t> n_children(size_t(n), 0);
	std::vector<char> b_join(size_t(n), 0);
	for(int32_t i = 0; i < n; ++ i) {
		if(r_parent[size_t(i)] >= 0)
			++ n_children[size_t(r_parent[size_t(i)])];
	}
	for(int32_t i = 0; i < n; ++ i) {
		b_join[size_t(i)] = b_join[size_t(i)] || n_children[size_t(i)] >= 2;
		if(b_join[size_t(i)] && r_parent[size_t(i)] >= 0)
			b_join[size_t(r_parent[size_t(i)])] = 1;
	}
	std::vector<std::vector<int32_t> > chains;
	for(int32_t i = 0; i < n; ++ i) {
		if(n_children[size_t(i)] != 0)
			continue;
		chains.push_back(std::vector<int32_t>());
		for(int32_t c = i; c >= 0 && !b_join[size_t(c)]; c = r_parent[size_t(c)])
			chains.back().push_back(c);
	}
	r_seg.n_tips = int32_t(chains.size());
	for(int k = 0; k < 3; ++ k)
		r_seg.seg[k].clear();
	std::stable_sort(chains.begin(), chains.end(), [](const std::vector<int32_t> &r_a, const std::vector<int32_t> &r_b) { return r_a.size() > r_b.size(); });
	for(size_t c = 0; c < chains.size(); ++ c) {
		std::vector<int32_t> &r_bin = r_seg.seg[(r_seg.seg[1].size() < r_seg.seg[0].size() && chains.size() > 1)? 1 : 0];
		r_bin.insert(r_bin.end(), chains[c].begin(), chains[c].end());
	}
	for(int32_t i = 0; i < n; ++ i) {
		if(b_join[size_t(i)])
			r_seg.seg[2].push_back(i);
	}
	std::sort(r_seg.seg[0].begin(), r_seg.seg[0].end());
	std::sort(r_seg.seg[1].begin(), r_seg.seg[1].end());
	return int32_t(std::max(r_seg.seg[0].size(), r_seg.seg[1].size()) + r_seg.seg[2].size());
}

namespace {

void Build_Simt_Branches(const Plan &P, size_t W, bool b_split_all, int32_t n_stage_tasks, const std::vector<TSimtTask> &tasks_all,
	const std::vector<std::vector<int32_t> > &groups, const std::vector<TSimtChunkJob> &jobs, size_t n_chunk0, raw_vector<int32_t> &index_pool,
	SparseRecords &r_rec, TSimtBranchStage &r_stage, std::vector<int32_t> &br_prog, raw_vector<int64_t> &br_tab, std::vector<char> &br_split)
{
	r_stage = TSimtBranchStage();
	r_stage.n_first = int32_t(r_rec.simt_br_groups.size());
	r_stage.n_stage_tasks = n_stage_tasks;
	std::vector<TSimtSegments> segs(groups.size());
	std::vector<int32_t> chain(groups.size(), 0), parent;
	for(size_t g = 0; g < groups.size(); ++ g) {
		const TSimtTask &tt = tasks_all[size_t(groups[g][0])];
		simt_task_parents(P, tt.n_task, parent);
		chain[g] = simt_task_segments(parent, segs[g]);
		const int32_t n_cols = int32_t(parent.size());
		if(segs[g].seg[1].empty())
			chain[g] = n_cols;
		r_stage.n_tstar = std::max(r_stage.n_tstar, std::min(n_cols, chain[g]));
		r_stage.n_longest_task = std::max(r_stage.n_longest_task, n_cols);
	}
	std::vector<char> split(groups.size(), 0);
	bool b_any_split = false;
	for(size_t g = 0; g < groups.size(); ++ g) {
		const int32_t n_cols = tasks_all[size_t(groups[g][0])].prog[0];
		split[g] = !segs[g].seg[1].empty() && chain[g] < n_cols && (b_split_all || n_cols > r_stage.n_tstar);
		b_any_split = b_any_split || split[g];
	}
	if(!b_any_split && !b_split_all)
		return;
	std::vector<TSimtTask> seg_tasks(groups.size() * 3);
	std::vector<std::vector<int32_t> > seg_op_map(groups.size() * 3), seg_y_map(groups.size() * 3);
	{
		int32_t *op_index = &index_pool[0], *y_index = op_index + P.lrow.size();
		std::vector<int32_t> touch, body, cols;
		for(size_t g = 0; g < groups.size(); ++ g) {
			if(!split[g])
				continue;
			const TSimtTask &r_first = tasks_all[size_t(groups[g][0])];
			for(size_t k = 0; k < 3; ++ k) {
				const std::vector<int32_t> &r_local = segs[g].seg[k];
				cols.resize(r_local.size());
				for(size_t i = 0; i < r_local.size(); ++ i)
					cols[i] = P.task_cols[size_t(P.task_ptr[r_first.n_task] + r_local[i])];
				TSimtTask &r_seg = seg_tasks[g * 3 + k];
				Simt_Task_Program(P, r_first.n_task, cols.data(), int32_t(cols.size()), W, op_index, y_index, touch, body, r_seg);
				for(int32_t n_blk : r_seg.ops) {
					const size_t n_at = size_t(std::find(r_first.ops.begin(), r_first.ops.end(), n_blk) - r_first.ops.begin());
					if(n_at == r_first.ops.size())
						throw std::logic_error("lane-per-task segments: an operand the whole task does not have");
					seg_op_map[g * 3 + k].push_back(int32_t(n_at));
				}
				for(int32_t c : r_seg.ys) {
					const size_t n_at = size_t(std::find(r_first.ys.begin(), r_first.ys.end(), c) - r_first.ys.begin());
					if(n_at == r_first.ys.size())
						throw std::logic_error("lane-per-task segments: a y column the whole task does not have");
					seg_y_map[g * 3 + k].push_back(int32_t(n_at));
				}
			}
		}
	}
	struct TItem { int32_t n_chain; TSimtBranchGroup t_group; char b_split; };
	struct TSegJob { size_t n_group, n_first; int n_seg, n_fields; int64_t n_tab_off; };
	std::vector<TItem> items;
	std::vector<std::pair<int32_t, size_t> > whole;
	std::vector<TSegJob> seg_jobs;
	std::map<std::pair<int32_t, int32_t>, int32_t> split_by;
	int32_t n_region_bytes = 0;
	const TSimtChunk t_none = {0, 0, 0};
	for(size_t n_job = 0; n_job < jobs.size(); ) {
		const size_t g = size_t(jobs[n_job].n_group);
		const int32_t n_cols = tasks_all[size_t(groups[g][0])].prog[0];
		if(!split[g]) {
			for(; n_job < jobs.size() && size_t(jobs[n_job].n_group) == g; ++ n_job) {
				whole.push_back(std::make_pair(n_cols, n_chunk0 + n_job));
				n_region_bytes = std::max(n_region_bytes, int32_t(jobs[n_job].n_fields * W * 8));
			}
			continue;
		}
		int32_t n_seg_prog_off[3] = {0, 0, 0};
		int n_seg_fields[3] = {0, 0, 0};
		for(size_t k = 0; k < 3; ++ k) {
			const std::vector<int32_t> &prog = seg_tasks[g * 3 + k].prog;
			n_seg_prog_off[k] = int32_t(br_prog.size());
			n_seg_fields[k] = 4 * prog[0] + prog[1] + prog[2] + prog[3];
			if(prog[0] > 0) {
				br_prog.insert(br_prog.end(), prog.begin(), prog.end());
				n_region_bytes = std::max(n_region_bytes, int32_t(n_seg_fields[k] * W * 8));
			}
		}
		const int32_t n_bin = int32_t(std::max(segs[g].seg[0].size(), segs[g].seg[1].size())), n_joins = int32_t(segs[g].seg[2].size());
		split_by[std::make_pair(n_bin, n_joins)] += int32_t(groups[g].size());
		r_stage.n_split_tasks += int32_t(groups[g].size());
		for(; n_job < jobs.size() && size_t(jobs[n_job].n_group) == g; ++ n_job) {
			const size_t n_first = jobs[n_job].n_first;
			TItem t_item;
			t_item.n_chain = chain[g];
			t_item.b_split = 1;
			for(size_t k = 0; k < 3; ++ k) {
				TSimtChunk &ch = t_item.t_group.seg[k];
				ch = t_none;
				if(!n_seg_fields[k])
					continue;
				ch.prog_off = n_seg_prog_off[k];
				ch.n_tasks = int32_t(std::min<size_t>(W, groups[g].size() - n_first));
				ch.tab_off = int64_t(br_tab.size());
				const TSegJob t_seg_job = {g, n_first, int(k), n_seg_fields[k], ch.tab_off};
				seg_jobs.push_back(t_seg_job);
				br_tab.resize(br_tab.size() + size_t(n_seg_fields[k]) * W);
			}
			items.push_back(t_item);
			++ r_stage.n_split_chunks;
		}
	}
	Parallel_Ranges(int64_t(seg_jobs.size()), 32, [&](int64_t n_b, int64_t n_e) {
		std::vector<int32_t> cols, ops, ys;
		for(int64_t n_j = n_b; n_j < n_e; ++ n_j) {
			const TSegJob &r_job = seg_jobs[size_t(n_j)];
			const std::vector<int32_t> &r_local = segs[r_job.n_group].seg[r_job.n_seg], &r_members = groups[r_job.n_group];
			const std::vector<int32_t> &r_op_map = seg_op_map[r_job.n_group * 3 + size_t(r_job.n_seg)], &r_y_map = seg_y_map[r_job.n_group * 3 + size_t(r_job.n_seg)];
			const size_t n_in_chunk = std::min<size_t>(W, r_members.size() - r_job.n_first);
			cols.resize(r_local.size());
			ops.resize(r_op_map.size());
			ys.resize(r_y_map.size());
			for(int n_lane = 0; n_lane < int(W); ++ n_lane) {
				const TSimtTask &tt = tasks_all[size_t(r_members[r_job.n_first + std::min<size_t>(size_t(n_lane), n_in_chunk - 1)])];
				for(size_t i = 0; i < r_local.size(); ++ i)
					cols[i] = P.task_cols[size_t(P.task_ptr[tt.n_task] + r_local[i])];
				for(size_t i = 0; i < r_op_map.size(); ++ i)
					ops[i] = tt.ops[size_t(r_op_map[i])];
				for(size_t i = 0; i < r_y_map.size(); ++ i)
					ys[i] = tt.ys[size_t(r_y_map[i])];
				if(Fill_Simt_Forward_Lane(P, W, &br_tab[size_t(r_job.n_tab_off)], n_lane, cols.data(), int32_t(cols.size()), ops, ys) != r_job.n_fields)
					throw std::logic_error("lane-per-task segments: field count mismatch");
			}
		}
	}, 8);
	std::stable_sort(whole.begin(), whole.end(), [](const std::pair<int32_t, size_t> &r_a, const std::pair<int32_t, size_t> &r_b) { return r_a.first > r_b.first; });
	for(size_t i = 0; i < whole.size(); i += 2) {
		TItem t_item;
		t_item.n_chain = whole[i].first;
		t_item.b_split = 0;
		t_item.t_group.seg[0] = r_rec.simt_chunks[whole[i].second];
		t_item.t_group.seg[1] = (i + 1 < whole.size())? r_rec.simt_chunks[whole[i + 1].second] : t_none;
		t_item.t_group.seg[2] = t_none;
		items.push_back(t_item);
	}
	r_stage.n_whole_chunks = int32_t(whole.size());
	std::stable_sort(items.begin(), items.end(), [](const TItem &r_a, const TItem &r_b) { return r_a.n_chain > r_b.n_chain; });
	if(2 * int64_t(n_region_bytes) > 64 * 1024) {
		r_stage.n_split_tasks = r_stage.n_split_chunks = r_stage.n_whole_chunks = 0;
		return;
	}
	for(size_t i = 0; i < items.size(); ++ i) {
		r_rec.simt_br_groups.push_back(items[i].t_group);
		br_split.push_back(items[i].b_split);
		r_stage.n_longest_chain = std::max(r_stage.n_longest_chain, items[i].n_chain);
	}
	r_stage.n_groups = int32_t(items.size());
	r_stage.n_lds_bytes = 2 * n_region_bytes;
	for(std::map<std::pair<int32_t, int32_t>, int32_t>::const_iterator p = split_by.begin(); p != split_by.end(); ++ p) {
		r_stage.split_by.push_back(p->first.first);
		r_stage.split_by.push_back(p->first.second);
		r_stage.split_by.push_back(p->second);
	}
}

}

void build_simt_tables(const Plan &P, const SparseRecordOptions &t_opt, SparseRecords &r_rec, SparseLaunchLists &r_lists)
{
	r_lists.simt_chunk_ptr.clear();
	r_lists.simt_rest_ptr.clear();
	r_lists.simt_lds_bytes.clear();
	r_rec.simt_chunks.clear(); r_rec.simt_prog.clear(); r_rec.simt_tab.clear(); r_rec.simt_rest.clear();
	r_lists.simt_bwd_lds_bytes.clear();
	r_lists.simt_br.clear();
	r_rec.simt_br_groups.clear();
	r_rec.simt_bwd_chunks.clear(); r_rec.simt_bwd_prog.clear(); r_rec.simt_bwd_tab.clear();
	if(!t_opt.n_simt || !b_Package_Dim(P))
		return;
	if(t_opt.n_simt < 0 && P.stage_ptr.size() > 1 && P.stage_ptr[1] - P.stage_ptr[0] < 2048)
		return;
	const int n_stages = int(P.stage_ptr.size()) - 1;
	std::vector<int32_t> &rest = r_rec.simt_rest;
	size_t n_tab_size = 0, n_bwd_tab_size = 0;
	r_lists.simt_chunk_ptr.push_back(0);
	r_lists.simt_rest_ptr.push_back(0);
	const size_t W = size_t(t_opt.n_simt_width);
	const int n_branches_env = dev_knob("SLAMPP_HIP_DEV_SIMT_FACTOR_BRANCHES", -1);
	const bool b_branches = n_branches_env != 0 && P.uniform_dim && P.max_dim == 6 && (W == 16 || W == 32);
	std::vector<int32_t> br_prog;
	raw_vector<int64_t> br_tab;
	std::vector<char> br_split;
	for(int s = 0; s < r_lists.n_bottom_stages && s < n_stages && s < t_opt.n_simt_stages; ++ s) {
		const int32_t t0 = P.stage_ptr[s], n_stage_tasks = P.stage_ptr[s + 1] - P.stage_ptr[s];
		double t_simt_phase = wall_ms();
		auto Simt_Phase = [&](const char *p_s_name) { if(t_opt.b_timing) { const double t_ = wall_ms();
			fprintf(stderr, "[shapes] stage %d %-12s %8.2f ms\n", s, p_s_name, t_ - t_simt_phase); t_simt_phase = t_; } };
		std::vector<TSimtTask> tasks_all(size_t(std::max(n_stage_tasks, 0)));
		enum { SIMT_THREADS = 8 };
		raw_vector<int32_t> index_pool((P.lrow.size() + size_t(P.n)) * SIMT_THREADS);
		std::atomic<int> n_next_slice(0);
		Parallel_Ranges(n_stage_tasks, 512, [&](int64_t n_b, int64_t n_e) {
			const size_t n_slice = size_t(n_next_slice.fetch_add(1)) % SIMT_THREADS;
			int32_t *op_index = &index_pool[(P.lrow.size() + size_t(P.n)) * n_slice], *y_index = op_index + P.lrow.size();
			std::fill(op_index, op_index + P.lrow.size() + size_t(P.n), -1);
			std::vector<int32_t> touch, body;
			for(int64_t n_i = n_b; n_i < n_e; ++ n_i)
				Simt_Task_Program(P, t0 + int32_t(n_i), P.task_cols.data() + P.task_ptr[t0 + n_i], int32_t(P.task_ptr[t0 + n_i + 1] - P.task_ptr[t0 + n_i]), W,
					op_index, y_index, touch, body, tasks_all[size_t(n_i)]);
		}, 8);
		Simt_Phase("programs");
		std::vector<std::vector<int32_t> > groups;
		Group_Simt_Shapes(tasks_all, rest, groups);
		Simt_Phase("grouping");
		std::vector<TSimtChunkJob> jobs;
		const std::pair<int32_t, int32_t> t_stage_lds = Layout_Simt_Chunks(P, W, tasks_all, groups, r_rec, n_tab_size, n_bwd_tab_size, jobs);
		if(b_branches) {
			r_rec.simt_tab.reserve(2 * n_tab_size);
			br_tab.reserve(n_tab_size);
		}
		r_rec.simt_tab.resize(n_tab_size);
		r_rec.simt_bwd_tab.resize(n_bwd_tab_size);
		Simt_Phase("layout");
		Parallel_Ranges(int64_t(jobs.size()), 32, [&](int64_t n_b, int64_t n_e) {
			for(int64_t n_job = n_b; n_job < n_e; ++ n_job)
				Fill_Simt_Chunk_Tables(P, W, tasks_all, groups, jobs[size_t(n_job)], r_rec);
		}, 8);
		Simt_Phase("tables");
		r_lists.simt_br.push_back(TSimtBranchStage());
		if(b_branches) {
			Build_Simt_Branches(P, W, n_branches_env == 1, n_stage_tasks, tasks_all, groups, jobs, r_rec.simt_chunks.size() - jobs.size(), index_pool,
				r_rec, r_lists.simt_br.back(), br_prog, br_tab, br_split);
			Simt_Phase("branches");
		}
		std::sort(rest.begin() + r_lists.simt_rest_ptr.back(), rest.end());
		r_lists.simt_chunk_ptr.push_back(int32_t(r_rec.simt_chunks.size()));
		r_lists.simt_rest_ptr.push_back(int32_t(rest.size()));
		r_lists.simt_lds_bytes.push_back(t_stage_lds.first);
		r_lists.simt_bwd_lds_bytes.push_back(t_stage_lds.second);
	}
	if(r_rec.simt_chunks.empty()) {
		r_lists.simt_chunk_ptr.clear();
		r_lists.simt_rest_ptr.clear();
	}
	if(r_rec.simt_br_groups.empty())
		r_lists.simt_br.clear();
	else {
		const int32_t n_prog_base = int32_t(r_rec.simt_prog.size());
		const int64_t n_tab_base = int64_t(r_rec.simt_tab.size());
		r_rec.simt_prog.insert(r_rec.simt_prog.end(), br_prog.begin(), br_prog.end());
		r_rec.simt_tab.resize(size_t(n_tab_base) + br_tab.size());
		std::copy(br_tab.begin(), br_tab.end(), r_rec.simt_tab.begin() + n_tab_base);
		for(size_t i = 0; i < r_rec.simt_br_groups.size(); ++ i) {
			for(int k = 0; k < 3 && br_split[i]; ++ k) {
				TSimtChunk &ch = r_rec.simt_br_groups[i].seg[k];
				if(ch.n_tasks > 0) {
					ch.prog_off += n_prog_base;
					ch.tab_off += n_tab_base;
				}
			}
		}
	}
}

}
```

slam_plus_plus_amd/csrc/sparse_records.h:

```cpp
#pragma once
#include "plan.h"
#include "sparse_kernels.h"
#include "host_pool.h"
#include "host_threads.h"

#include <algorithm>

namespace slampp {

struct SparseRecordOptions {
	int n_panel;
	int n_panel_handup;
	int n_simt;
	int n_simt_width;
	int n_simt_stages;
	int n_wide_min_tasks;
	bool b_small;
	bool b_timing;
};

struct TSimtBranchStage {
	int32_t n_first = 0, n_groups = 0;
	int32_t n_split_tasks = 0, n_split_chunks = 0, n_whole_chunks = 0;
	int32_t n_tstar = 0;
	int32_t n_longest_chain = 0;
	int32_t n_longest_task = 0, n_stage_tasks = 0;
	int32_t n_lds_bytes = 0;
	std::vector<int32_t> split_by;
};

struct SparseLaunchLists {
	int n_bottom_stages = 1;
	std::vector<int32_t> panel_ptr, panel_rest_ptr, panel_upd_ptr;
	std::vector<TPanelLaunch> panel_cfg;
	std::vector<TBwdLaunch> bwd_cfg;
	std::vector<char> panel_ride;
	bool b_any_hand_up = false;
	std::vector<int32_t> simt_chunk_ptr, simt_rest_ptr;
	std::vector<int32_t> simt_lds_bytes, simt_bwd_lds_bytes;
	std::vector<TSimtBranchStage> simt_br;
};

struct SparseRecords {
	raw_vector<TColDesc> cols;
	raw_vector<TBlkDesc> blks;
	raw_vector<longlong2> pairs;
	raw_vector<TRowEnt> rents;
	raw_vector<longlong2> pkg;
	std::vector<int64_t> task_pkg;
	raw_vector<longlong2> panel_pkg;
	std::vector<int64_t> panel_off, panel_out_off;
	std::vector<int32_t> panel_units;
	std::vector<int32_t> panel_rest;
	raw_vector<longlong2> bwd_rec;
	std::vector<int64_t> bwd_off;
	raw_vector<TUpdSlot> upd_slots;
	raw_vector<TUpdEnt> upd_ents;
	int64_t n_handup_doubles = 0;
	std::vector<TDenseBlk> dense_blks;
	std::vector<TDenseCol> dense_cols;
	std::vector<int64_t> dense_blk_loff;
	std::vector<int32_t> gaps;
	std::vector<uint8_t> unit;
	std::vector<longlong2> dst;
	std::vector<TSimtChunk> simt_chunks, simt_bwd_chunks;
	std::vector<int32_t> simt_prog, simt_rest, simt_bwd_prog;
	raw_vector<int64_t> simt_tab, simt_bwd_tab;
	std::vector<TSimtBranchGroup> simt_br_groups;
};

template <class F>
void Parallel_Ranges(int64_t n, int64_t n_min_per_thread, F f, int n_max_threads = 4)
{
	for_ranges(0, n, host_thread_count(n, n_min_per_thread, n_max_threads), [&](int, int64_t n_b, int64_t n_e) { f(n_b, n_e); });
}


int count_bottom_stages(const Plan &P, const SparseRecordOptions &t_opt);
int64_t first_upper_column(const Plan &P, const SparseRecordOptions &t_opt, const SparseLaunchLists &r_lists);
void alloc_column_records(const Plan &P, SparseRecords &r_rec);
void fill_column_records(const Plan &P, SparseRecords &r_rec, int64_t i_begin, int64_t i_end);
void fill_dense_top_column_records(const Plan &P, SparseRecords &r_rec);
void reserve_panel_packages(const Plan &P, const SparseLaunchLists &r_lists, int64_t n_upper_begin, SparseRecords &r_rec);
void build_panel_packages(const Plan &P, const SparseRecordOptions &t_opt, SparseRecords &r_rec, SparseLaunchLists &r_lists);
void build_column_packages(const Plan &P, const SparseLaunchLists &r_lists, SparseRecords &r_rec);
void build_dense_top_records(const Plan &P, int n_dense_pad, SparseRecords &r_rec);
struct TSimtSegments {
	std::vector<int32_t> seg[3];
	int32_t n_tips = 0;
};
void simt_task_parents(const Plan &P, int32_t t, std::vector<int32_t> &r_parent);
int32_t simt_task_segments(const std::vector<int32_t> &r_parent, TSimtSegments &r_seg);
void build_simt_tables(const Plan &P, const SparseRecordOptions &t_opt, SparseRecords &r_rec, SparseLaunchLists &r_lists);

}
```

slam_plus_plus_amd/csrc/sparse_setup.hip:

```cpp
#include <execinfo.h>
#include <signal.h>
#include <unistd.h>
#include <pthread.h>
#include "solver.h"
#include "sparse_inverse.h"
#include "sparse_records.h"

#include <algorithm>
#include <atomic>
#include <chrono>
#include <cstdio>
#include <cstdlib>
#include <cstring>
#include <map>
#include <string>
#include <unordered_map>
#include <thread>
#include <mutex>
#include <condition_variable>
#include <functional>
#include <sys/mman.h>

using namespace slampp;

// ... 137 lines not shown
	Phase("dense lists");
	s.d_dense.Alloc(size_t(n_dense_pad) * n_dense_pad);
	s.b_dense_clean = false;
	s.d_dense_invdiag.Alloc(size_t(n_dense_pad / dense_NB) * dense_NB * dense_NB);
	s.d_dense_z.Alloc(n_dense_pad);
	s.d_dense_x.Alloc(n_dense_pad);
	Phase("dense allocs");
	s.b_dense_tiles = false;
	if(s.n_dense_top_tiles == 0)
		return;
	std::vector<char> nonzero;
	const int T = dense_top_tile_pattern(P, nonzero);
	if(T != n_dense_pad / dense_NB)
		throw std::logic_error("dense top: tile count mismatch");
	if(s.dense_tiles.Build(T, nonzero, s.stream))
		s.b_dense_tiles = s.n_dense_top_tiles > 0 || 100 * s.dense_tiles.n_levels <= 85 * T;
	if(Phase.b_timing) {
		size_t n_nz = 0;
		for(size_t k = 0; k < nonzero.size(); ++ k)
			n_nz += nonzero[k];
		fprintf(stderr, "[setup] dense top: %d tiles per side, %zu of %d lower tiles nonzero before fill, %d levels, "
			"%d trsm tiles, %d update targets -> %s schedule\n", T, n_nz, T * (T + 1) / 2, s.dense_tiles.n_levels,
			s.dense_tiles.level_trsm_ptr.empty()? 0 : s.dense_tiles.level_trsm_ptr.back(),
			s.dense_tiles.level_tgt_ptr.empty()? 0 : s.dense_tiles.level_tgt_ptr.back(), s.b_dense_tiles? "tile" : "dense");
	}
}

}

void slampp_hip_solver::Analyze_Sparse()
{
	Join_Discard();
	if(p_sinv) {
		sparse_inverse_destroy(p_sinv);
		p_sinv = 0;
	}
	b_sinv_tried = false;
	TSetupPhases Phase = {getenv("SLAMPP_HIP_PLAN_TIMING") != 0, wall_ms()};
	const bool b_timing = Phase.b_timing;

	Build_Sparse_Plan(*this);
	Phase("build_plan");
	const Plan &P = plan;
	const int64_t n_lblocks = int64_t(P.lrow.size());
	const SparseRecordOptions t_opt = t_Record_Options(*this, b_timing);
	const bool b_small = t_opt.b_small;
	lists.n_bottom_stages = count_bottom_stages(P, t_opt);
	SparseRecords rec;

	std::exception_ptr p_simt_error;
	CJoinedThread t_simt_thread;
	const double t_simt = wall_ms();
	if(b_small)
		build_simt_tables(P, t_opt, rec, lists);
	else {
		t_simt_thread.t = std::thread([&]() {
			try {
				build_simt_tables(P, t_opt, rec, lists);
			} catch(...) {
				p_simt_error = std::current_exception();
			}
		});
	}

	alloc_column_records(P, rec);
	const int64_t n_upper_begin = first_upper_column(P, t_opt, lists), n_sched = int64_t(rec.cols.size());
	fill_column_records(P, rec, n_upper_begin, n_sched);
	reserve_panel_packages(P, lists, n_upper_begin, rec);

	std::exception_ptr p_panel_error;
	CJoinedThread t_panel_thread;
	if(b_small)
		build_panel_packages(P, t_opt, rec, lists);
	else {
		t_panel_thread.t = std::thread([&]() {
			try {
				const double t_panel = wall_ms();
				build_panel_packages(P, t_opt, rec, lists);
				if(b_timing)
					fprintf(stderr, "[setup] %-12s %8.2f ms on their own thread\n", "panel pkgs", wall_ms() - t_panel);
			} catch(...) {
				p_panel_error = std::current_exception();
			}
		});
	}

	Parallel_Ranges(n_upper_begin, 4096, [&](int64_t i_begin, int64_t i_end) { fill_column_records(P, rec, i_begin, i_end); }, 8);
	fill_dense_top_column_records(P, rec);

	build_column_packages(P, lists, rec);
	Phase("records");

	std::exception_ptr p_upload_error;
	CJoinedThread t_upload_thread;
	if(b_small) {
		Upload_Records(*this, rec);
		Phase("record uploads");
	} else {
		t_upload_thread.t = std::thread([&]() {
			try {
				Upload_Records(*this, rec);
			} catch(...) {
				p_upload_error = std::current_exception();
			}
		});
	}
	Join_Bringup();

	n_dense_dim = P.dense_dim;
	n_dense_pad = n_dense_dim? dense_padded_dim(n_dense_dim) : 0;
	build_dense_top_records(P, n_dense_pad, rec);
	if(n_dense_dim)
		Setup_Dense_Top(*this, rec, Phase);
	n_dense_blks = int(rec.dense_blks.size());
	n_dense_cols = int(rec.dense_cols.size());
	Phase("tile schedule");

	if(t_panel_thread.t.joinable())
		t_panel_thread.t.join();
	if(p_panel_error)
		std::rethrow_exception(p_panel_error);
	Phase("packages");
	d_panel_upd_slots.Upload(rec.upd_slots, stream);
	d_panel_upd_ents.Upload(rec.upd_ents, stream);
	d_panel_pkg.Upload(rec.panel_pkg, stream);
	d_panel_off.Upload(rec.panel_off, stream);
	d_panel_out_off.Upload(rec.panel_out_off, stream);
	d_handup.Alloc(size_t(std::max<int64_t>(rec.n_handup_doubles, int64_t(P.max_dim) * P.max_dim + 8)));
	d_panel_rest.Upload(rec.panel_rest, stream);
	n_lds_limit = plain_launch_lds_limit();
	d_bwd_rec.Upload(rec.bwd_rec, stream);
	d_bwd_off.Upload(rec.bwd_off, stream);
	if(t_upload_thread.t.joinable())
		t_upload_thread.t.join();
	if(p_upload_error)
		std::rethrow_exception(p_upload_error);
	Phase("uploads");
	d_L.Alloc(size_t(P.loff[n_lblocks]));
	d_Linv.Alloc(size_t(P.linv_off[P.n]));
	d_w.Alloc(size_t(P.cs_new[P.n]));
	d_flag.Alloc(1);
	SLAMPP_HIP_CHECK(hipMemsetAsync(d_flag.p(), 0, sizeof(int), stream));
	Phase("allocs");
	SLAMPP_HIP_CHECK(hipStreamSynchronize(stream));
	Phase("sync");

	dplan.cols = d_cols.p(); dplan.blks = d_blks.p(); dplan.pairs = d_pairs.p(); dplan.rents = d_rents.p();
	dplan.task_ptr = d_task_ptr.p();
	dplan.uniform_dim = P.uniform_dim? P.max_dim : 0;
	dplan.pkg = d_pkg.p();
	dplan.task_pkg = d_pkg.p()? d_task_pkg.p() : 0;
	dplan.n_blks = n_lblocks;
	dplan.n_pairs = int64_t(rec.pairs.size());
	dplan.n_rents = int64_t(rec.rents.size());
	dplan.p_timing = 0;
	dplan.task_map = 0;
	{
		const double t_wait = wall_ms();
		if(t_simt_thread.t.joinable())
			t_simt_thread.t.join();
		if(p_simt_error)
			std::rethrow_exception(p_simt_error);
		Upload_Simt(rec);
		if(b_timing)
			fprintf(stderr, "[setup] %-12s %8.2f ms since it was started, %.2f ms of them waited for\n", "shapes", wall_ms() - t_simt, wall_ms() - t_wait);
	}
	if(getenv("SLAMPP_HIP_STAGE_TIMING")) {
		d_timing.Alloc(1 + 32 * 4096);
		SLAMPP_HIP_CHECK(hipMemsetAsync(d_timing.p(), 0, (1 + 32 * 4096) * sizeof(long long), stream));
		dplan.p_timing = d_timing.p();
	}

	if(!b_small) {
		Join_Discard();
		Discard_Later(analysis_trash, rec.cols); Discard_Later(analysis_trash, rec.blks); Discard_Later(analysis_trash, rec.pairs);
		Discard_Later(analysis_trash, rec.rents); Discard_Later(analysis_trash, rec.pkg); Discard_Later(analysis_trash, rec.task_pkg);
		Discard_Later(analysis_trash, rec.panel_pkg); Discard_Later(analysis_trash, rec.upd_slots); Discard_Later(analysis_trash, rec.upd_ents);
		Discard_Later(analysis_trash, rec.simt_tab); Discard_Later(analysis_trash, rec.simt_bwd_tab);
		try {
			t_discard = std::thread([this]() { analysis_trash.clear(); host_pool_release(); });
		} catch(std::system_error&) {
			analysis_trash.clear();
			host_pool_release();
		}
	}
}

void slampp_hip_solver::Ensure_Leaf_Inverses()
{
	b_leaf_linv_wanted = true;
	if(b_leaf_linv_valid || lists.simt_chunk_ptr.empty())
		return;
	const Plan &P = plan;
	const int n_simt_stages_used = int(lists.simt_chunk_ptr.size()) - 1;
	const int64_t n_col_end = P.task_ptr[size_t(P.stage_ptr[size_t(n_simt_stages_used)])];
	launch_invert_diagonals(dplan, 0, n_col_end, d_L.p(), d_Linv.p(), stream);
	b_leaf_linv_valid = true;
}

void slampp_hip_solver::Report_Simt_Backward(const SparseRecords &r_rec) const
{
	enum { N_MAX = 16 };
	for(size_t s = 0; s + 1 < lists.simt_chunk_ptr.size(); ++ s) {
		long long n_by_cols[N_MAX + 1] = {0}, n_by_blocks[N_MAX + 1] = {0}, n_by_outside[SIMT_BWD_AHEAD + 1] = {0}, n_inside = 0, n_outside = 0, n_tasks = 0;
		int n_spare_chunks = 0;
		for(int32_t c = lists.simt_chunk_ptr[s]; c < lists.simt_chunk_ptr[s + 1]; ++ c) {
			const TSimtChunk &ch = r_rec.simt_bwd_chunks[size_t(c)];
			const int32_t *P = &r_rec.simt_bwd_prog[size_t(ch.prog_off)];
			const int n_cols = P[0], n_below = P[1];
			n_tasks += ch.n_tasks;
			n_spare_chunks += ch.n_tasks < n_simt_width;
			n_by_cols[std::min(n_cols, int(N_MAX))] += ch.n_tasks;
			for(int i = 0, n_blk0 = 0; i < n_cols; n_blk0 += P[2 + i] - 1, ++ i) {
				n_by_blocks[std::min(P[2 + i] - 1, int(N_MAX))] += ch.n_tasks;
				int n_set_outside = 0;
				for(int k = 0; k < SIMT_BWD_AHEAD && k < P[2 + i] - 1; ++ k)
					n_set_outside += P[2 + n_cols + n_blk0 + k] < 0;
				n_by_outside[n_set_outside] += ch.n_tasks;
			}
			for(int b = 0; b < n_below; ++ b)
				((P[2 + n_cols + b] >= 0)? n_inside : n_outside) += ch.n_tasks;
		}
		std::string s_cols, s_blocks, s_outside;
		for(int i = 0; i <= SIMT_BWD_AHEAD; ++ i)
			s_outside += " " + std::to_string(i) + ":" + std::to_string(n_by_outside[i]);
		for(int i = 0; i <= N_MAX; ++ i) {
			if(n_by_cols[i])
				s_cols += " " + std::to_string(i) + ":" + std::to_string(n_by_cols[i]);
			if(n_by_blocks[i])
				s_blocks += " " + std::to_string(i) + ":" + std::to_string(n_by_blocks[i]);
		}
		fprintf(stderr, "[setup] stage %zu backward lanes: %lld tasks in %d chunks of width %d, %d chunks with spare lanes, fetch ahead holds %d blocks, one round holds %d waves; "
			"tasks by columns:%s; columns by sub-diagonal blocks:%s; columns by rows outside the task among the blocks held:%s; blocks with the row inside the task: %lld, outside: %lld\n", s, n_tasks,
			lists.simt_chunk_ptr[s + 1] - lists.simt_chunk_ptr[s], n_simt_width, n_spare_chunks, int(SIMT_BWD_AHEAD),
			(s < simt_bwd_ahead_waves.size())? simt_bwd_ahead_waves[s] : 0, s_cols.c_str(), s_blocks.c_str(), s_outside.c_str(), n_inside, n_outside);
	}
}

void slampp_hip_solver::Report_Simt_Factor(const SparseRecords &r_rec) const
{
	enum { N_MAX = 16 };
	for(size_t s = 0; s + 1 < lists.simt_chunk_ptr.size(); ++ s) {
		long long n_by_cols[N_MAX + 1] = {0}, n_by_blocks[N_MAX + 1] = {0}, n_by_sources[N_MAX + 1] = {0}, n_by_fill[N_MAX + 1] = {0}, n_held_fill = 0, n_tasks = 0;
		int n_spare_chunks = 0;
		for(int32_t c = lists.simt_chunk_ptr[s]; c < lists.simt_chunk_ptr[s + 1]; ++ c) {
			const TSimtChunk &ch = r_rec.simt_chunks[size_t(c)];
			const int32_t *P = &r_rec.simt_prog[size_t(ch.prog_off)];
			const int64_t *T = &r_rec.simt_tab[size_t(ch.tab_off)];
			const int n_cols = P[0];
			n_tasks += ch.n_tasks;
			n_spare_chunks += ch.n_tasks < n_simt_width;
			n_by_cols[std::min(n_cols, int(N_MAX))] += ch.n_tasks;
			for(int i = 0, pc = 4, n_blk0 = 0; i < n_cols; ++ i) {
				const int nb = P[pc], nr = P[pc + 1], n_touch = P[pc + 2];
				pc += 3 + n_touch + 2 * nr;
				for(int kb = 1; kb < nb; ++ kb)
					pc += 1 + 2 * P[pc];
				n_by_blocks[std::min(nb - 1, int(N_MAX))] += ch.n_tasks;
				for(int t = 0; t < ch.n_tasks; ++ t) {
					int n_sources = 0, n_fill = 0;
					for(int kb = 1; kb < nb; ++ kb) {
						const bool b_fill = T[size_t(4 * n_cols + n_blk0 + kb) * size_t(n_simt_width) + size_t(t)] < 0;
						(b_fill? n_fill : n_sources) ++;
						n_held_fill += b_fill && kb <= int(SIMT_FACTOR_AHEAD);
					}
					n_by_sources[std::min(n_sources, int(N_MAX))] ++;
					n_by_fill[std::min(n_fill, int(N_MAX))] ++;
				}
				n_blk0 += nb;
			}
		}
		std::string s_cols, s_blocks, s_sources, s_fill;
		for(int i = 0; i <= N_MAX; ++ i) {
			if(n_by_cols[i])
				s_cols += " " + std::to_string(i) + ":" + std::to_string(n_by_cols[i]);
			if(n_by_blocks[i])
				s_blocks += " " + std::to_string(i) + ":" + std::to_string(n_by_blocks[i]);
			if(n_by_sources[i])
				s_sources += " " + std::to_string(i) + ":" + std::to_string(n_by_sources[i]);
			if(n_by_fill[i])
				s_fill += " " + std::to_string(i) + ":" + std::to_string(n_by_fill[i]);
		}
		fprintf(stderr, "[setup] stage %zu factor lanes: %lld tasks in %d chunks of width %d, %d chunks with spare lanes, fetch ahead holds %d blocks, one round holds %d waves; "
			"tasks by columns:%s; columns by sub-diagonal blocks:%s; columns by sub-diagonal blocks with a source in Lambda:%s; columns by fill-in blocks:%s; "
			"fill-in blocks among the blocks held: %lld\n", s, n_tasks, lists.simt_chunk_ptr[s + 1] - lists.simt_chunk_ptr[s], n_simt_width, n_spare_chunks,
			int(SIMT_FACTOR_AHEAD), (s < simt_factor_ahead_waves.size())? simt_factor_ahead_waves[s] : 0, s_cols.c_str(), s_blocks.c_str(), s_sources.c_str(),
			s_fill.c_str(), n_held_fill);
	}
}

void slampp_hip_solver::Upload_Simt(const SparseRecords &r_rec)
{
	const Plan &P = plan;
	if(r_rec.simt_chunks.empty())
		return;
	d_simt_chunks.Upload(r_rec.simt_chunks, stream);
	d_simt_prog.Upload(r_rec.simt_prog, stream);
	d_simt_tab.Upload(r_rec.simt_tab, stream);
	d_simt_rest.Upload(r_rec.simt_rest, stream);
	d_simt_bwd_chunks.Upload(r_rec.simt_bwd_chunks, stream);
	d_simt_bwd_prog.Upload(r_rec.simt_bwd_prog, stream);
	d_simt_bwd_tab.Upload(r_rec.simt_bwd_tab, stream);
	d_simt_br_groups.Upload(r_rec.simt_br_groups, stream);
	SLAMPP_HIP_CHECK(hipStreamSynchronize(stream));
	simt_branches_round_groups.clear();
	for(size_t s = 0; s < lists.simt_br.size(); ++ s)
		simt_branches_round_groups.push_back((lists.simt_br[s].n_groups > 0)? factor_simt_branches_groups(P.max_dim, n_simt_width, lists.simt_br[s].n_lds_bytes) : 0);
	simt_bwd_ahead_waves.clear();
	for(size_t s = 0; s < lists.simt_bwd_lds_bytes.size(); ++ s)
		simt_bwd_ahead_waves.push_back(backward_simt_ahead_waves(P.max_dim, n_simt_width, lists.simt_bwd_lds_bytes[s]));
	simt_factor_ahead_waves.clear();
	for(size_t s = 0; s < lists.simt_lds_bytes.size(); ++ s)
		simt_factor_ahead_waves.push_back(factor_simt_ahead_waves(P.max_dim, n_simt_width, lists.simt_lds_bytes[s]));
	if(getenv("SLAMPP_HIP_PLAN_TIMING")) {
		Report_Simt_Backward(r_rec);
		Report_Simt_Factor(r_rec);
		for(size_t s = 0; s < lists.simt_br.size(); ++ s) {
			const TSimtBranchStage &r_br = lists.simt_br[s];
			if(!r_br.n_groups)
				continue;
			std::string s_by;
			for(size_t i = 0; i + 2 < r_br.split_by.size(); i += 3)
				s_by += " (" + std::to_string(r_br.split_by[i]) + "," + std::to_string(r_br.split_by[i + 1]) + "):" + std::to_string(r_br.split_by[i + 2]);
			fprintf(stderr, "[setup] stage %zu factor branches: %d split tasks in %d split chunks, %d whole chunks, %d workgroups of two waves, T* %d, longest chain %d, "
				"longest task %d; split tasks by (longer bin, join columns):%s; LDS %d bytes, one round holds %d workgroups\n", s, r_br.n_split_tasks, r_br.n_split_chunks,
				r_br.n_whole_chunks, r_br.n_groups, r_br.n_tstar, r_br.n_longest_chain, r_br.n_longest_task, s_by.c_str(), r_br.n_lds_bytes,
				(s < simt_branches_round_groups.size())? simt_branches_round_groups[s] : 0);
		}
		for(size_t s = 0; s + 1 < lists.simt_chunk_ptr.size(); ++ s) {
			fprintf(stderr, "[setup] stage %zu: %d tasks -> %d chunks of 64 lanes, %d tasks left to the wave-per-task kernel\n", s,
				P.stage_ptr[s + 1] - P.stage_ptr[s], lists.simt_chunk_ptr[s + 1] - lists.simt_chunk_ptr[s], lists.simt_rest_ptr[s + 1] - lists.simt_rest_ptr[s]);
		}
	}
}
```

Baseline: 614.4 GFLOP/s.

## Add split-branch backward substitution kernel and share batched table staging

Adds a backward-substitution kernel that mirrors the factor's branch grouping. A long task's tree branches are split across two waves of a workgroup, and a shared join segment is solved first by one wave, so the critical chain of the bottom stages gets shorter. The host builds separate backward branch programs and tables and uploads them, and a heuristic picks this path when the stage fits in one residency round and has enough tasks. It also replaces the simple LDS table staging loops with a shared routine that keeps eight loads in flight per lane. The cost is extra setup work, more LDS per workgroup and a more complex launch decision.

```diff
diff --git a/slam_plus_plus_amd/csrc/simt_factor_ahead.hip b/slam_plus_plus_amd/csrc/simt_factor_ahead.hip
--- a/slam_plus_plus_amd/csrc/simt_factor_ahead.hip
+++ b/slam_plus_plus_amd/csrc/simt_factor_ahead.hip
@@ -95,25 +95,6 @@
 		#pragma unroll
 		for(int r = 0; r < D; r += 2)
 			*reinterpret_cast<double2*>(p_out + r + q * D) = double2{n_half? m[r][q + D / 2] : m[r][q], n_half? m[r + 1][q + D / 2] : m[r + 1][q]};
-	}
-}
-
-__device__ __forceinline__ void factor_ahead_stage_table(long long *p_dst, const long long *__restrict__ p_src, int n_entries, int n_lane)
-{
-	enum { N_FLIGHT = 8 };
-	for(int n_base = 0; n_base < n_entries; n_base += N_FLIGHT * 64) {
-		long long v[N_FLIGHT];
-		#pragma unroll
-		for(int u = 0; u < N_FLIGHT; ++ u) {
-			const int i = n_base + u * 64 + n_lane;
-			v[u] = p_src[(i < n_entries)? i : n_entries - 1];
-		}
-		#pragma unroll
-		for(int u = 0; u < N_FLIGHT; ++ u) {
-			const int i = n_base + u * 64 + n_lane;
-			if(i < n_entries)
-				p_dst[i] = v[u];
-		}
 	}
 }
 
@@ -215,7 +196,7 @@
 	const TSimtChunk ch = chunks[blockIdx.x];
 	{
 		const int n_entries = (4 * prog[ch.prog_off] + prog[ch.prog_off + 1] + prog[ch.prog_off + 2] + prog[ch.prog_off + 3]) * W;
-		factor_ahead_stage_table(s_tab, tab + ch.tab_off, n_entries, int(threadIdx.x));
+		simt_stage_table(s_tab, tab + ch.tab_off, n_entries, int(threadIdx.x));
 		__syncthreads();
 	}
 	if(int(threadIdx.x) >= W * LPT)
@@ -247,7 +228,7 @@
 		if(ch.n_tasks > 0 && (n_pass == 0 || n_wave == 0)) {
 			const int32_t *P = prog + ch.prog_off;
 			const int n_entries = (4 * P[0] + P[1] + P[2] + P[3]) * W;
-			factor_ahead_stage_table(s_mine, tab + ch.tab_off, n_entries, n_lane);
+			simt_stage_table(s_mine, tab + ch.tab_off, n_entries, n_lane);
 			__builtin_amdgcn_fence(__ATOMIC_ACQ_REL, "workgroup");
 			__builtin_amdgcn_wave_barrier();
 			if(n_lane < W * 2) {
diff --git a/slam_plus_plus_amd/csrc/simt_kernel.hip b/slam_plus_plus_amd/csrc/simt_kernel.hip
--- a/slam_plus_plus_amd/csrc/simt_kernel.hip
+++ b/slam_plus_plus_amd/csrc/simt_kernel.hip
@@ -20,8 +20,7 @@
 	const TSimtChunk ch = chunks[blockIdx.x];
 	{
 		const int n_entries = (4 * prog[ch.prog_off] + prog[ch.prog_off + 1] + prog[ch.prog_off + 2] + prog[ch.prog_off + 3]) * W;
-		for(int i = threadIdx.x; i < n_entries; i += 64)
-			s_tab[i] = tab[ch.tab_off + i];
+		simt_stage_table(s_tab, tab + ch.tab_off, n_entries, int(threadIdx.x));
 		__syncthreads();
 	}
 	if(int(threadIdx.x) >= W * LPT)
@@ -182,8 +181,7 @@
 	const int n_cols = P[0], n_below = P[1];
 	{
 		const int n_entries = (3 * n_cols + n_below) * W;
-		for(int i = threadIdx.x; i < n_entries; i += 64)
-			s_tab[i] = tab[ch.tab_off + i];
+		simt_stage_table(s_tab, tab + ch.tab_off, n_entries, int(threadIdx.x));
 		__syncthreads();
 	}
 	if(int(threadIdx.x) >= W)
@@ -287,9 +285,10 @@
 }
 template <int D> constexpr int bwd_ahead_solve_stores() { return (D % 2 == 0)? D : 2 * D; }
 
-template <int D, int W, int AHEAD, int N_NEWER >
+template <int D, int W, int AHEAD, int N_NEWER ,
+	bool b_slots = false >
 __device__ __forceinline__ void bwd_ahead_solve(TBwdAheadSet<D, AHEAD> &s, int ci, int n_cols, const int32_t *p_local, const long long *T, double *s_x,
-	const double *__restrict__ L, double *w, double *x_out)
+	const double *__restrict__ L, double *w, double *x_out, const int32_t *p_slot = 0)
 {
 	enum { DD = D * D };
 	__builtin_amdgcn_s_waitcnt(simt_wait_imm(N_NEWER));
@@ -348,9 +347,29 @@
 			sum -= s.a[q][r] * x[r];
 		x[q] = sum * s.a[q][q];
 	}
-	simt_store_local_x<D, W>(s_x, ci, x);
+	simt_store_local_x<D, W>(s_x, b_slots? p_slot[ci] : ci, x);
 	const long long cs_new = T[W * (3 * ci + 1)], cs_src = T[W * (3 * ci + 2)];
 	simt_store_x<D>(w + cs_new, x_out + cs_src, x);
+}
+
+template <int D, int W, int AHEAD, bool b_slots>
+__device__ __forceinline__ void bwd_ahead_columns(TBwdAheadSet<D, AHEAD> &t_even, TBwdAheadSet<D, AHEAD> &t_odd, int n_cols, const int32_t *P, const int32_t *p_local,
+	const int32_t *p_slot, const long long *T, double *s_x, const double *__restrict__ L, double *w, double *x_out)
+{
+	enum { N_FETCH = bwd_ahead_fetch_loads<D, AHEAD>(), N_STORES = bwd_ahead_solve_stores<D>() };
+	int ci = n_cols - 1;
+	for(; ci >= 2; ci -= 2) {
+		bwd_ahead_fetch<D, W, AHEAD>(t_odd, ci - 1, t_even.n_blk0, n_cols, P, p_local, T, L, w);
+		bwd_ahead_solve<D, W, AHEAD, N_FETCH, b_slots>(t_even, ci, n_cols, p_local, T, s_x, L, w, x_out, p_slot);
+		bwd_ahead_fetch<D, W, AHEAD>(t_even, ci - 2, t_odd.n_blk0, n_cols, P, p_local, T, L, w);
+		bwd_ahead_solve<D, W, AHEAD, N_STORES + N_FETCH, b_slots>(t_odd, ci - 1, n_cols, p_local, T, s_x, L, w, x_out, p_slot);
+	}
+	if(ci == 1) {
+		bwd_ahead_fetch<D, W, AHEAD>(t_odd, 0, t_even.n_blk0, n_cols, P, p_local, T, L, w);
+		bwd_ahead_solve<D, W, AHEAD, N_FETCH, b_slots>(t_even, 1, n_cols, p_local, T, s_x, L, w, x_out, p_slot);
+		bwd_ahead_solve<D, W, AHEAD, N_STORES, b_slots>(t_odd, 0, n_cols, p_local, T, s_x, L, w, x_out, p_slot);
+	} else
+		bwd_ahead_solve<D, W, AHEAD, 0, b_slots>(t_even, 0, n_cols, p_local, T, s_x, L, w, x_out, p_slot);
 }
 
 template <int D, int W, int AHEAD>
@@ -365,8 +384,7 @@
 	const int n_cols = P[0], n_below = P[1];
 	{
 		const int n_entries = (3 * n_cols + n_below) * W;
-		for(int i = threadIdx.x; i < n_entries; i += 64)
-			s_tab[i] = tab[ch.tab_off + i];
+		simt_stage_table(s_tab, tab + ch.tab_off, n_entries, int(threadIdx.x));
 		__syncthreads();
 	}
 	if(int(threadIdx.x) >= W)
@@ -375,21 +393,65 @@
 	double *s_x = reinterpret_cast<double*>(s_tab + (3 * n_cols + n_below) * W) + threadIdx.x;
 	const int32_t *p_local = P + 2 + n_cols;
 	TBwdAheadSet<D, AHEAD> t_even, t_odd;
-	enum { N_FETCH = bwd_ahead_fetch_loads<D, AHEAD>(), N_STORES = bwd_ahead_solve_stores<D>() };
-	int ci = n_cols - 1;
-	bwd_ahead_fetch<D, W, AHEAD>(t_even, ci, n_below, n_cols, P, p_local, T, L, w);
-	for(; ci >= 2; ci -= 2) {
-		bwd_ahead_fetch<D, W, AHEAD>(t_odd, ci - 1, t_even.n_blk0, n_cols, P, p_local, T, L, w);
-		bwd_ahead_solve<D, W, AHEAD, N_FETCH>(t_even, ci, n_cols, p_local, T, s_x, L, w, x_out);
-		bwd_ahead_fetch<D, W, AHEAD>(t_even, ci - 2, t_odd.n_blk0, n_cols, P, p_local, T, L, w);
-		bwd_ahead_solve<D, W, AHEAD, N_STORES + N_FETCH>(t_odd, ci - 1, n_cols, p_local, T, s_x, L, w, x_out);
-	}
-	if(ci == 1) {
-		bwd_ahead_fetch<D, W, AHEAD>(t_odd, 0, t_even.n_blk0, n_cols, P, p_local, T, L, w);
-		bwd_ahead_solve<D, W, AHEAD, N_FETCH>(t_even, 1, n_cols, p_local, T, s_x, L, w, x_out);
-		bwd_ahead_solve<D, W, AHEAD, N_STORES>(t_odd, 0, n_cols, p_local, T, s_x, L, w, x_out);
-	} else
-		bwd_ahead_solve<D, W, AHEAD, 0>(t_even, 0, n_cols, p_local, T, s_x, L, w, x_out);
+	bwd_ahead_fetch<D, W, AHEAD>(t_even, n_cols - 1, n_below, n_cols, P, p_local, T, L, w);
+	bwd_ahead_columns<D, W, AHEAD, false>(t_even, t_odd, n_cols, P, p_local, 0, T, s_x, L, w, x_out);
+}
+
+template <int D, int W, int AHEAD>
+__global__ void __launch_bounds__(128)
+backward_simt_kernel_branches(const TSimtBranchGroup *__restrict__ groups, const int32_t *__restrict__ prog, const long long *__restrict__ tab,
+	const double *__restrict__ L, double *w, double *x_out, TBatch t_batch, int n_tab_region, int n_x_region)
+{	{ const int64_t n_member = blockIdx.y; L += n_member * t_batch.l; w += n_member * t_batch.w; x_out += n_member * t_batch.b; }
+
+	extern __shared__ long long s_tab[];
+	const int n_wave = __builtin_amdgcn_readfirstlane(int(threadIdx.x) >> 6), n_lane = int(threadIdx.x) & 63;
+	const TSimtBranchGroup &r_group = groups[blockIdx.x];
+	const bool b_shared_x = r_group.seg[2].n_tasks > 0;
+	for(int k = n_wave; k < 3; k += 2) {
+		const TSimtChunk ch = r_group.seg[k];
+		if(ch.n_tasks > 0) {
+			const int32_t *P = prog + ch.prog_off;
+			simt_stage_table(s_tab + k * n_tab_region, tab + ch.tab_off, (3 * P[0] + P[1]) * W, n_lane);
+		}
+	}
+	__builtin_amdgcn_fence(__ATOMIC_ACQ_REL, "workgroup");
+	__builtin_amdgcn_wave_barrier();
+	TBwdAheadSet<D, AHEAD> t_even, t_odd;
+	t_even.nb = t_even.n_blk0 = t_even.n_xk = 0;
+	#pragma unroll
+	for(int i = 0; i < AHEAD; ++ i)
+		t_even.n_local[i] = 0;
+	const bool b_my_lane = (int(threadIdx.x) & 63) < W;
+	double *s_x = reinterpret_cast<double*>(s_tab + 3 * n_tab_region) + (b_shared_x? 0 : n_wave * n_x_region) + n_lane;
+	{
+		const TSimtChunk ch = r_group.seg[2];
+		if(ch.n_tasks > 0 && !n_wave && b_my_lane) {
+			const int32_t *P = prog + ch.prog_off;
+			const int n_cols = P[0], n_below = P[1];
+			const long long *T = s_tab + 2 * n_tab_region + n_lane;
+			const int32_t *p_local = P + 2 + n_cols;
+			bwd_ahead_fetch<D, W, AHEAD>(t_even, n_cols - 1, n_below, n_cols, P, p_local, T, L, w);
+			bwd_ahead_columns<D, W, AHEAD, true>(t_even, t_odd, n_cols, P, p_local, p_local + n_below, T, s_x, L, w, x_out);
+		}
+	}
+	t_even.nb = __builtin_amdgcn_readfirstlane(t_even.nb);
+	t_even.n_blk0 = __builtin_amdgcn_readfirstlane(t_even.n_blk0);
+	t_even.n_xk = __builtin_amdgcn_readfirstlane(t_even.n_xk);
+	#pragma unroll
+	for(int i = 0; i < AHEAD; ++ i)
+		t_even.n_local[i] = __builtin_amdgcn_readfirstlane(t_even.n_local[i]);
+	__syncthreads();
+	{
+		const TSimtChunk ch = r_group.seg[n_wave];
+		if(ch.n_tasks > 0 && b_my_lane) {
+			const int32_t *P = prog + ch.prog_off;
+			const int n_cols = P[0], n_below = P[1];
+			const long long *T = s_tab + (n_wave * n_tab_region - n_wave * 64) + int(threadIdx.x);
+			const int32_t *p_local = P + 2 + n_cols;
+			bwd_ahead_fetch<D, W, AHEAD>(t_even, n_cols - 1, n_below, n_cols, P, p_local, T, L, w);
+			bwd_ahead_columns<D, W, AHEAD, true>(t_even, t_odd, n_cols, P, p_local, p_local + n_below, T, s_x, L, w, x_out);
+		}
+	}
 }
 
 template <int D> struct TBwdAheadDim { enum { b_have = (D == 6) }; };
@@ -438,14 +500,57 @@
 	return simt_resident_workgroups(p_Backward_Ahead_Kernel(n_dim, n_width), 64, n_lds_bytes);
 }
 
+static const void *p_Backward_Branches_Kernel(int n_dim, int n_width)
+{
+	if(n_dim != 6)
+		return 0;
+	return (n_width == 16)? reinterpret_cast<const void*>(&backward_simt_kernel_branches<6, 16, SIMT_BWD_AHEAD>) :
+		(n_width == 32)? reinterpret_cast<const void*>(&backward_simt_kernel_branches<6, 32, SIMT_BWD_AHEAD>) : 0;
+}
+
+bool backward_simt_branches_exists(int n_dim, int n_width)
+{
+	return p_Backward_Branches_Kernel(n_dim, n_width) != 0;
+}
+
+int backward_simt_branches_groups(int n_dim, int n_width, int n_lds_bytes)
+{
+	if(!backward_simt_branches_exists(n_dim, n_width) || n_lds_bytes <= 0)
+		return 0;
+	return simt_resident_workgroups(p_Backward_Branches_Kernel(n_dim, n_width), 128, n_lds_bytes);
+}
+
 bool launch_backward_simt(const TSimtChunk *chunks, int n_chunks, int n_width, int n_lds_bytes, size_t n_lds_limit, int n_ahead_waves, const int32_t *prog, const int64_t *tab,
-	int n_dim, const double *L, double *w, double *x_out, hipStream_t stream, const TBatch &t_batch, bool b_report)
+	int n_dim, const double *L, double *w, double *x_out, hipStream_t stream, const TBatch &t_batch, bool b_report, const TSimtBwdBranchLaunch *p_branches)
 {
 	if(n_chunks <= 0)
 		return true;
 	if(n_lds_bytes < 0 || size_t(n_lds_bytes) > n_lds_limit)
 		return false;
 	const long long *t = reinterpret_cast<const long long*>(tab);
+	{
+		const int n_branches_env = dev_knob("SLAMPP_HIP_DEV_SIMT_BWD_BRANCHES", -1);
+		const int n_ahead_knob = dev_knob("SLAMPP_HIP_DEV_SIMT_BWD_AHEAD", -1);
+		const bool b_would_fetch_ahead = p_Backward_Ahead_Kernel(n_dim, n_width) &&
+			((n_ahead_knob >= 0)? n_ahead_knob != 0 : int64_t(n_chunks) * std::max<int64_t>(t_batch.n, 1) <= n_ahead_waves);
+		const bool b_branches = p_branches && p_branches->n_groups > 0 && backward_simt_branches_exists(n_dim, n_width) &&
+			p_branches->n_lds_bytes > 0 && size_t(p_branches->n_lds_bytes) <= n_lds_limit &&
+			((n_branches_env >= 0)? n_branches_env != 0 : b_would_fetch_ahead &&
+			int64_t(p_branches->n_groups) * std::max<int64_t>(t_batch.n, 1) <= p_branches->n_round_groups &&
+			p_branches->n_tstar < p_branches->n_longest_task && p_branches->n_stage_tasks >= 2048);
+		if(b_branches) {
+			if(b_report)
+				fprintf(stderr, "stage_timing lane-per-task backward branches launch: %d workgroups of two waves, %d split chunks, %d whole chunks, width %d, block size %d, %d members\n",
+					p_branches->n_groups, p_branches->n_split_chunks, p_branches->n_whole_chunks, n_width, n_dim, int(t_batch.n));
+			if(n_width == 16)
+				hipLaunchKernelGGL((backward_simt_kernel_branches<6, 16, SIMT_BWD_AHEAD>), dim3(p_branches->n_groups, t_batch.n), dim3(128), p_branches->n_lds_bytes, stream,
+					p_branches->groups, prog, t, L, w, x_out, t_batch, p_branches->n_tab_region, p_branches->n_x_region);
+			else
+				hipLaunchKernelGGL((backward_simt_kernel_branches<6, 32, SIMT_BWD_AHEAD>), dim3(p_branches->n_groups, t_batch.n), dim3(128), p_branches->n_lds_bytes, stream,
+					p_branches->groups, prog, t, L, w, x_out, t_batch, p_branches->n_tab_region, p_branches->n_x_region);
+			return hipGetLastError() == hipSuccess;
+		}
+	}
 	const int n_ahead_env = dev_knob("SLAMPP_HIP_DEV_SIMT_BWD_AHEAD", -1);
 	const void *p_ahead = p_Backward_Ahead_Kernel(n_dim, n_width);
 	const bool b_ahead = p_ahead && ((n_ahead_env >= 0)? n_ahead_env != 0 : int64_t(n_chunks) * std::max<int64_t>(t_batch.n, 1) <= n_ahead_waves);
diff --git a/slam_plus_plus_amd/csrc/solver.h b/slam_plus_plus_amd/csrc/solver.h
--- a/slam_plus_plus_amd/csrc/solver.h
+++ b/slam_plus_plus_amd/csrc/solver.h
@@ -183,6 +183,8 @@
 	slampp::CDevArray<int64_t> d_simt_bwd_tab;
 	std::vector<int32_t> simt_factor_ahead_waves;
 	slampp::CDevArray<slampp::TSimtBranchGroup> d_simt_br_groups;
+	slampp::CDevArray<slampp::TSimtBranchGroup> d_simt_bwd_br_groups;
+	std::vector<int32_t> simt_bwd_branches_round_groups;
 	std::vector<int32_t> simt_branches_round_groups;
 	std::vector<int32_t> simt_bwd_ahead_waves;
 	bool b_leaf_linv_wanted = false, b_leaf_linv_valid = true;
diff --git a/slam_plus_plus_amd/csrc/solver.hip b/slam_plus_plus_amd/csrc/solver.hip
--- a/slam_plus_plus_amd/csrc/solver.hip
+++ b/slam_plus_plus_amd/csrc/solver.hip
@@ -70,7 +70,7 @@
 {
 	d_cols.Free(); d_blks.Free(); d_rents.Free(); d_pairs.Free(); d_task_ptr.Free(); d_task_pkg.Free(); d_pkg.Free();
 	d_simt_chunks.Free(); d_simt_prog.Free(); d_simt_rest.Free(); d_simt_tab.Free();
-	d_simt_bwd_chunks.Free(); d_simt_bwd_prog.Free(); d_simt_bwd_tab.Free(); d_simt_br_groups.Free();
+	d_simt_bwd_chunks.Free(); d_simt_bwd_prog.Free(); d_simt_bwd_tab.Free(); d_simt_br_groups.Free(); d_simt_bwd_br_groups.Free();
 	b_leaf_linv_valid = true;
 	d_panel_pkg.Free(); d_panel_off.Free(); d_panel_out_off.Free(); d_handup.Free(); d_panel_rest.Free(); d_bwd_rec.Free(); d_bwd_off.Free(); d_panel_upd_slots.Free(); d_panel_upd_ents.Free();
 	lists = SparseLaunchLists();
@@ -127,7 +127,7 @@
 		d_dense_z.n_Bytes() + d_dense_x.n_Bytes() + d_cols.n_Bytes() + d_blks.n_Bytes() + d_rents.n_Bytes() +
 		d_task_ptr.n_Bytes() + d_task_pkg.n_Bytes() + d_pkg.n_Bytes() + d_pairs.n_Bytes() + d_A.n_Bytes() +
 		d_simt_chunks.n_Bytes() + d_simt_prog.n_Bytes() + d_simt_rest.n_Bytes() + d_simt_tab.n_Bytes() +
-		d_simt_bwd_chunks.n_Bytes() + d_simt_bwd_prog.n_Bytes() + d_simt_bwd_tab.n_Bytes() + d_simt_br_groups.n_Bytes() +
+		d_simt_bwd_chunks.n_Bytes() + d_simt_bwd_prog.n_Bytes() + d_simt_bwd_tab.n_Bytes() + d_simt_br_groups.n_Bytes() + d_simt_bwd_br_groups.n_Bytes() +
 		d_panel_pkg.n_Bytes() + d_panel_off.n_Bytes() + d_panel_out_off.n_Bytes() + d_handup.n_Bytes() + d_panel_rest.n_Bytes() + d_bwd_rec.n_Bytes() + d_bwd_off.n_Bytes() + d_panel_upd_slots.n_Bytes() + d_panel_upd_ents.n_Bytes() +
 		d_rhs.n_Bytes() + d_L.n_Bytes() + d_Linv.n_Bytes() + d_w.n_Bytes() + d_cov.n_Bytes() + d_flag.n_Bytes() +
 		d_Z.n_Bytes() + d_diag_zoff.n_Bytes() + d_Zd.n_Bytes() + d_Zd_work.n_Bytes() + sparse_inverse_bytes(p_sinv) + covariance_bytes(p_cov) +
diff --git a/slam_plus_plus_amd/csrc/sparse_enqueue.hip b/slam_plus_plus_amd/csrc/sparse_enqueue.hip
--- a/slam_plus_plus_amd/csrc/sparse_enqueue.hip
+++ b/slam_plus_plus_amd/csrc/sparse_enqueue.hip
@@ -166,9 +166,16 @@
 	for(int s = n_stages; s > 0; -- s) {
 		if(b_simt_bwd && s < int(lists.simt_chunk_ptr.size())) {
 			const int n_chunks = lists.simt_chunk_ptr[s] - lists.simt_chunk_ptr[s - 1], n_rest = lists.simt_rest_ptr[s] - lists.simt_rest_ptr[s - 1];
+			TSimtBwdBranchLaunch t_branches = {0, 0, 0, 0, 0, 0, 0, 0, 0, 0, 0};
+			if(size_t(s - 1) < lists.simt_br.size() && size_t(s - 1) < simt_bwd_branches_round_groups.size() && lists.simt_br[size_t(s - 1)].n_bwd_groups > 0 && d_simt_bwd_br_groups.p()) {
+				const TSimtBranchStage &r_br = lists.simt_br[size_t(s - 1)];
+				const TSimtBwdBranchLaunch t_have = {d_simt_bwd_br_groups.p() + r_br.n_bwd_first, r_br.n_bwd_groups, r_br.n_split_chunks, r_br.n_whole_chunks, r_br.n_bwd_lds_bytes,
+					r_br.n_bwd_tab_region, r_br.n_bwd_x_region, simt_bwd_branches_round_groups[size_t(s - 1)], r_br.n_tstar, r_br.n_longest_task, r_br.n_stage_tasks};
+				t_branches = t_have;
+			}
 			if(!launch_backward_simt(d_simt_bwd_chunks.p() + lists.simt_chunk_ptr[s - 1], n_chunks, n_simt_width, lists.simt_bwd_lds_bytes[s - 1], n_lds_limit,
 				(size_t(s - 1) < simt_bwd_ahead_waves.size())? simt_bwd_ahead_waves[s - 1] : 0, d_simt_bwd_prog.p(), d_simt_bwd_tab.p(), P.max_dim, d_L.p(), d_w.p(), p_rhs_dev, stream, t_batch,
-				dplan.p_timing != 0))
+				dplan.p_timing != 0, t_branches.n_groups? &t_branches : 0))
 				throw CDeviceError("lane-per-task backward launch refused: block size or LDS request outside what the analysis planned for");
 			if(n_rest > 0) {
 				TDevPlan t_rest = dplan;
diff --git a/slam_plus_plus_amd/csrc/sparse_kernels.h b/slam_plus_plus_amd/csrc/sparse_kernels.h
--- a/slam_plus_plus_amd/csrc/sparse_kernels.h
+++ b/slam_plus_plus_amd/csrc/sparse_kernels.h
@@ -219,9 +219,21 @@
 bool launch_factor_simt_branches(const TSimtBranchGroup *groups, int n_groups, int n_width, int n_lds_bytes, const int32_t *prog, const int64_t *tab, int n_dim,
 	const double *A, double *L, double *Linv, const double *b, double *w, int *p_flag, hipStream_t stream, long long *p_timing, const TBatch &t_batch);
 enum { SIMT_BWD_AHEAD = 2 };
+struct TSimtBwdBranchLaunch {
+	const TSimtBranchGroup *groups;
+	int n_groups, n_split_chunks, n_whole_chunks;
+	int n_lds_bytes;
+	int n_tab_region;
+	int n_x_region;
+	int n_round_groups;
+	int n_tstar, n_longest_task, n_stage_tasks;
+};
+bool backward_simt_branches_exists(int n_dim, int n_width);
+int backward_simt_branches_groups(int n_dim, int n_width, int n_lds_bytes);
 bool launch_backward_simt(const TSimtChunk *chunks, int n_chunks, int n_width, int n_lds_bytes, size_t n_lds_limit ,
 	int n_ahead_waves, const int32_t *prog, const int64_t *tab,
-	int n_dim, const double *L, double *w, double *x_out, hipStream_t stream, const TBatch &t_batch = t_No_Batch(), bool b_report = false);
+	int n_dim, const double *L, double *w, double *x_out, hipStream_t stream, const TBatch &t_batch = t_No_Batch(), bool b_report = false,
+	const TSimtBwdBranchLaunch *p_branches = 0);
 int backward_simt_ahead_waves(int n_dim, int n_width, int n_lds_bytes);
 bool launch_invert_diagonals(const TDevPlan &p, int64_t col_begin, int64_t col_end, const double *L, double *Linv, hipStream_t stream);
 
diff --git a/slam_plus_plus_amd/csrc/sparse_records.cpp b/slam_plus_plus_amd/csrc/sparse_records.cpp
--- a/slam_plus_plus_amd/csrc/sparse_records.cpp
+++ b/slam_plus_plus_amd/csrc/sparse_records.cpp
@@ -1098,9 +1098,112 @@
 
 namespace {
 
+struct TSimtBranchItem {
+	int32_t n_chain;
+	TSimtBranchGroup t_group;
+	char b_split;
+	size_t n_group;
+	size_t n_chunk[2];
+};
+
+void Build_Simt_Bwd_Branches(const Plan &P, size_t W, const std::vector<TSimtSegments> &segs, const std::vector<TSimtBranchItem> &items,
+	SparseRecords &r_rec, TSimtBranchStage &r_stage, std::vector<int32_t> &bwd_prog, std::vector<int64_t> &bwd_tab, std::vector<char> &bwd_split)
+{
+	const size_t n_prog0 = bwd_prog.size(), n_tab0 = bwd_tab.size();
+	std::map<std::pair<int32_t, int>, int32_t> prog_of;
+	std::vector<TSimtBranchGroup> records;
+	std::vector<int32_t> blk0;
+	size_t n_tab_region = 0;
+	int32_t n_x_cols = 0;
+	const TSimtChunk t_none = {0, 0, 0};
+	for(size_t n_item = 0; n_item < items.size(); ++ n_item) {
+		const TSimtBranchItem &r_item = items[n_item];
+		TSimtBranchGroup t_record = {{t_none, t_none, t_none}};
+		for(int n_half = 0; n_half < 2; ++ n_half) {
+			if(r_item.n_chunk[n_half] == size_t(-1))
+				continue;
+			const TSimtChunk ch = r_rec.simt_bwd_chunks[r_item.n_chunk[n_half]];
+			const int32_t *p_whole = &r_rec.simt_bwd_prog[size_t(ch.prog_off)];
+			const int32_t n_cols = p_whole[0], n_below = p_whole[1];
+			const int32_t *p_nb = p_whole + 2, *p_local = p_nb + n_cols;
+			n_x_cols = std::max(n_x_cols, n_cols);
+			r_stage.n_bwd_spare_chunks += size_t(ch.n_tasks) < W;
+			blk0.assign(size_t(n_cols) + 1, 0);
+			for(int32_t i = 0; i < n_cols; ++ i)
+				blk0[size_t(i) + 1] = blk0[size_t(i)] + p_nb[i] - 1;
+			for(int32_t i = 0; i < n_cols; ++ i) {
+				int n_outside = 0;
+				for(int32_t b = blk0[size_t(i)]; b < blk0[size_t(i) + 1]; ++ b)
+					n_outside += p_local[b] < 0;
+				r_stage.n_bwd_two_outside_columns += (n_outside >= 2)? ch.n_tasks : 0;
+			}
+			if(!r_item.b_split) {
+				std::pair<std::map<std::pair<int32_t, int>, int32_t>::iterator, bool> t_at = prog_of.insert(std::make_pair(std::make_pair(ch.prog_off, 3), int32_t(bwd_prog.size())));
+				if(t_at.second) {
+					bwd_prog.insert(bwd_prog.end(), p_whole, p_whole + 2 + n_cols + n_below);
+					for(int32_t i = 0; i < n_cols; ++ i)
+						bwd_prog.push_back(i);
+				}
+				const TSimtChunk t_seg = {t_at.first->second, ch.n_tasks, ch.tab_off};
+				t_record.seg[n_half] = t_seg;
+				n_tab_region = std::max(n_tab_region, size_t(3 * n_cols + n_below) * W);
+				continue;
+			}
+			const TSimtSegments &r_segs = segs[r_item.n_group];
+			r_stage.n_bwd_tip3_tasks += (r_segs.n_tips >= 3)? ch.n_tasks : 0;
+			for(int k = 0; k < 3; ++ k) {
+				const std::vector<int32_t> &r_cols = r_segs.seg[k];
+				if(r_cols.empty())
+					continue;
+				int32_t n_seg_below = 0;
+				for(int32_t c : r_cols) {
+					n_seg_below += p_nb[c] - 1;
+					r_stage.n_bwd_long_columns += (p_nb[c] > int32_t(SIMT_BWD_AHEAD) + 1)? ch.n_tasks : 0;
+				}
+				std::pair<std::map<std::pair<int32_t, int>, int32_t>::iterator, bool> t_at = prog_of.insert(std::make_pair(std::make_pair(ch.prog_off, k), int32_t(bwd_prog.size())));
+				if(t_at.second) {
+					bwd_prog.push_back(int32_t(r_cols.size()));
+					bwd_prog.push_back(n_seg_below);
+					for(int32_t c : r_cols)
+						bwd_prog.push_back(p_nb[c]);
+					for(int32_t c : r_cols)
+						bwd_prog.insert(bwd_prog.end(), p_local + blk0[size_t(c)], p_local + blk0[size_t(c) + 1]);
+					bwd_prog.insert(bwd_prog.end(), r_cols.begin(), r_cols.end());
+				}
+				const TSimtChunk t_seg = {t_at.first->second, ch.n_tasks, int64_t(bwd_tab.size())};
+				t_record.seg[k] = t_seg;
+				const int64_t *p_tab = &r_rec.simt_bwd_tab[size_t(ch.tab_off)];
+				for(int32_t c : r_cols)
+					bwd_tab.insert(bwd_tab.end(), p_tab + size_t(3 * c) * W, p_tab + size_t(3 * c + 3) * W);
+				for(int32_t c : r_cols)
+					bwd_tab.insert(bwd_tab.end(), p_tab + size_t(3 * n_cols + blk0[size_t(c)]) * W, p_tab + size_t(3 * n_cols + blk0[size_t(c) + 1]) * W);
+				n_tab_region = std::max(n_tab_region, (3 * r_cols.size() + size_t(n_seg_below)) * W);
+			}
+		}
+		records.push_back(t_record);
+	}
+	const size_t n_x_region = size_t(n_x_cols) * size_t(P.max_dim) * W;
+	const size_t n_lds_bytes = (3 * n_tab_region + 2 * n_x_region) * 8;
+	if(n_lds_bytes > 64 * 1024) {
+		bwd_prog.resize(n_prog0);
+		bwd_tab.resize(n_tab0);
+		r_stage.n_bwd_tip3_tasks = r_stage.n_bwd_long_columns = r_stage.n_bwd_two_outside_columns = r_stage.n_bwd_spare_chunks = 0;
+		return;
+	}
+	r_stage.n_bwd_first = int32_t(r_rec.simt_bwd_br_groups.size());
+	r_stage.n_bwd_groups = int32_t(records.size());
+	r_stage.n_bwd_tab_region = int32_t(n_tab_region);
+	r_stage.n_bwd_x_region = int32_t(n_x_region);
+	r_stage.n_bwd_lds_bytes = int32_t(n_lds_bytes);
+	r_rec.simt_bwd_br_groups.insert(r_rec.simt_bwd_br_groups.end(), records.begin(), records.end());
+	for(size_t n_item = 0; n_item < items.size(); ++ n_item)
+		bwd_split.push_back(items[n_item].b_split);
+}
+
 void Build_Simt_Branches(const Plan &P, size_t W, bool b_split_all, int32_t n_stage_tasks, const std::vector<TSimtTask> &tasks_all,
 	const std::vector<std::vector<int32_t> > &groups, const std::vector<TSimtChunkJob> &jobs, size_t n_chunk0, raw_vector<int32_t> &index_pool,
-	SparseRecords &r_rec, TSimtBranchStage &r_stage, std::vector<int32_t> &br_prog, raw_vector<int64_t> &br_tab, std::vector<char> &br_split)
+	SparseRecords &r_rec, TSimtBranchStage &r_stage, std::vector<int32_t> &br_prog, raw_vector<int64_t> &br_tab, std::vector<char> &br_split,
+	std::vector<int32_t> &bwd_br_prog, std::vector<int64_t> &bwd_br_tab, std::vector<char> &bwd_br_split)
 {
 	r_stage = TSimtBranchStage();
 	r_stage.n_first = int32_t(r_rec.simt_br_groups.size());
@@ -1157,7 +1260,7 @@
 			}
 		}
 	}
-	struct TItem { int32_t n_chain; TSimtBranchGroup t_group; char b_split; };
+	typedef TSimtBranchItem TItem;
 	struct TSegJob { size_t n_group, n_first; int n_seg, n_fields; int64_t n_tab_off; };
 	std::vector<TItem> items;
 	std::vector<std::pair<int32_t, size_t> > whole;
@@ -1194,6 +1297,9 @@
 			TItem t_item;
 			t_item.n_chain = chain[g];
 			t_item.b_split = 1;
+			t_item.n_group = g;
+			t_item.n_chunk[0] = n_chunk0 + n_job;
+			t_item.n_chunk[1] = size_t(-1);
 			for(size_t k = 0; k < 3; ++ k) {
 				TSimtChunk &ch = t_item.t_group.seg[k];
 				ch = t_none;
@@ -1238,6 +1344,9 @@
 		TItem t_item;
 		t_item.n_chain = whole[i].first;
 		t_item.b_split = 0;
+		t_item.n_group = size_t(-1);
+		t_item.n_chunk[0] = whole[i].second;
+		t_item.n_chunk[1] = (i + 1 < whole.size())? whole[i + 1].second : size_t(-1);
 		t_item.t_group.seg[0] = r_rec.simt_chunks[whole[i].second];
 		t_item.t_group.seg[1] = (i + 1 < whole.size())? r_rec.simt_chunks[whole[i + 1].second] : t_none;
 		t_item.t_group.seg[2] = t_none;
@@ -1256,6 +1365,7 @@
 	}
 	r_stage.n_groups = int32_t(items.size());
 	r_stage.n_lds_bytes = 2 * n_region_bytes;
+	Build_Simt_Bwd_Branches(P, W, segs, items, r_rec, r_stage, bwd_br_prog, bwd_br_tab, bwd_br_split);
 	for(std::map<std::pair<int32_t, int32_t>, int32_t>::const_iterator p = split_by.begin(); p != split_by.end(); ++ p) {
 		r_stage.split_by.push_back(p->first.first);
 		r_stage.split_by.push_back(p->first.second);
@@ -1274,6 +1384,7 @@
 	r_lists.simt_bwd_lds_bytes.clear();
 	r_lists.simt_br.clear();
 	r_rec.simt_br_groups.clear();
+	r_rec.simt_bwd_br_groups.clear();
 	r_rec.simt_bwd_chunks.clear(); r_rec.simt_bwd_prog.clear(); r_rec.simt_bwd_tab.clear();
 	if(!t_opt.n_simt || !b_Package_Dim(P))
 		return;
@@ -1285,11 +1396,12 @@
 	r_lists.simt_chunk_ptr.push_back(0);
 	r_lists.simt_rest_ptr.push_back(0);
 	const size_t W = size_t(t_opt.n_simt_width);
-	const int n_branches_env = dev_knob("SLAMPP_HIP_DEV_SIMT_FACTOR_BRANCHES", -1);
-	const bool b_branches = n_branches_env != 0 && P.uniform_dim && P.max_dim == 6 && (W == 16 || W == 32);
-	std::vector<int32_t> br_prog;
+	const int n_branches_env = dev_knob("SLAMPP_HIP_DEV_SIMT_FACTOR_BRANCHES", -1), n_bwd_branches_env = dev_knob("SLAMPP_HIP_DEV_SIMT_BWD_BRANCHES", -1);
+	const bool b_branches = (n_branches_env != 0 || n_bwd_branches_env == 1) && P.uniform_dim && P.max_dim == 6 && (W == 16 || W == 32);
+	std::vector<int32_t> br_prog, bwd_br_prog;
 	raw_vector<int64_t> br_tab;
-	std::vector<char> br_split;
+	std::vector<int64_t> bwd_br_tab;
+	std::vector<char> br_split, bwd_br_split;
 	for(int s = 0; s < r_lists.n_bottom_stages && s < n_stages && s < t_opt.n_simt_stages; ++ s) {
 		const int32_t t0 = P.stage_ptr[s], n_stage_tasks = P.stage_ptr[s + 1] - P.stage_ptr[s];
 		double t_simt_phase = wall_ms();
@@ -1328,8 +1440,8 @@
 		Simt_Phase("tables");
 		r_lists.simt_br.push_back(TSimtBranchStage());
 		if(b_branches) {
-			Build_Simt_Branches(P, W, n_branches_env == 1, n_stage_tasks, tasks_all, groups, jobs, r_rec.simt_chunks.size() - jobs.size(), index_pool,
-				r_rec, r_lists.simt_br.back(), br_prog, br_tab, br_split);
+			Build_Simt_Branches(P, W, n_branches_env == 1 || n_bwd_branches_env == 1, n_stage_tasks, tasks_all, groups, jobs, r_rec.simt_chunks.size() - jobs.size(), index_pool,
+				r_rec, r_lists.simt_br.back(), br_prog, br_tab, br_split, bwd_br_prog, bwd_br_tab, bwd_br_split);
 			Simt_Phase("branches");
 		}
 		std::sort(rest.begin() + r_lists.simt_rest_ptr.back(), rest.end());
@@ -1360,6 +1472,23 @@
 			}
 		}
 	}
-}
-
-}
+	if(!r_rec.simt_bwd_br_groups.empty()) {
+		const int32_t n_prog_base = int32_t(r_rec.simt_bwd_prog.size());
+		const int64_t n_tab_base = int64_t(r_rec.simt_bwd_tab.size());
+		r_rec.simt_bwd_prog.insert(r_rec.simt_bwd_prog.end(), bwd_br_prog.begin(), bwd_br_prog.end());
+		r_rec.simt_bwd_tab.resize(size_t(n_tab_base) + bwd_br_tab.size());
+		std::copy(bwd_br_tab.begin(), bwd_br_tab.end(), r_rec.simt_bwd_tab.begin() + n_tab_base);
+		for(size_t i = 0; i < r_rec.simt_bwd_br_groups.size(); ++ i) {
+			for(int k = 0; k < 3; ++ k) {
+				TSimtChunk &ch = r_rec.simt_bwd_br_groups[i].seg[k];
+				if(ch.n_tasks > 0) {
+					ch.prog_off += n_prog_base;
+					if(bwd_br_split[i])
+						ch.tab_off += n_tab_base;
+				}
+			}
+		}
+	}
+}
+
+}
diff --git a/slam_plus_plus_amd/csrc/sparse_records.h b/slam_plus_plus_amd/csrc/sparse_records.h
--- a/slam_plus_plus_amd/csrc/sparse_records.h
+++ b/slam_plus_plus_amd/csrc/sparse_records.h
@@ -27,6 +27,9 @@
 	int32_t n_longest_task = 0, n_stage_tasks = 0;
 	int32_t n_lds_bytes = 0;
 	std::vector<int32_t> split_by;
+	int32_t n_bwd_first = 0, n_bwd_groups = 0;
+	int32_t n_bwd_tab_region = 0, n_bwd_x_region = 0, n_bwd_lds_bytes = 0;
+	int32_t n_bwd_tip3_tasks = 0, n_bwd_long_columns = 0, n_bwd_two_outside_columns = 0, n_bwd_spare_chunks = 0;
 };
 
 struct SparseLaunchLists {
@@ -67,6 +70,7 @@
 	std::vector<int32_t> simt_prog, simt_rest, simt_bwd_prog;
 	raw_vector<int64_t> simt_tab, simt_bwd_tab;
 	std::vector<TSimtBranchGroup> simt_br_groups;
+	std::vector<TSimtBranchGroup> simt_bwd_br_groups;
 };
 
 template <class F>
diff --git a/slam_plus_plus_amd/csrc/sparse_setup.hip b/slam_plus_plus_amd/csrc/sparse_setup.hip
--- a/slam_plus_plus_amd/csrc/sparse_setup.hip
+++ b/slam_plus_plus_amd/csrc/sparse_setup.hip
@@ -463,10 +463,14 @@
 	d_simt_bwd_prog.Upload(r_rec.simt_bwd_prog, stream);
 	d_simt_bwd_tab.Upload(r_rec.simt_bwd_tab, stream);
 	d_simt_br_groups.Upload(r_rec.simt_br_groups, stream);
+	d_simt_bwd_br_groups.Upload(r_rec.simt_bwd_br_groups, stream);
 	SLAMPP_HIP_CHECK(hipStreamSynchronize(stream));
 	simt_branches_round_groups.clear();
 	for(size_t s = 0; s < lists.simt_br.size(); ++ s)
 		simt_branches_round_groups.push_back((lists.simt_br[s].n_groups > 0)? factor_simt_branches_groups(P.max_dim, n_simt_width, lists.simt_br[s].n_lds_bytes) : 0);
+	simt_bwd_branches_round_groups.clear();
+	for(size_t s = 0; s < lists.simt_br.size(); ++ s)
+		simt_bwd_branches_round_groups.push_back((lists.simt_br[s].n_bwd_groups > 0)? backward_simt_branches_groups(P.max_dim, n_simt_width, lists.simt_br[s].n_bwd_lds_bytes) : 0);
 	simt_bwd_ahead_waves.clear();
 	for(size_t s = 0; s < lists.simt_bwd_lds_bytes.size(); ++ s)
 		simt_bwd_ahead_waves.push_back(backward_simt_ahead_waves(P.max_dim, n_simt_width, lists.simt_bwd_lds_bytes[s]));
@@ -487,6 +491,14 @@
 				"longest task %d; split tasks by (longer bin, join columns):%s; LDS %d bytes, one round holds %d workgroups\n", s, r_br.n_split_tasks, r_br.n_split_chunks,
 				r_br.n_whole_chunks, r_br.n_groups, r_br.n_tstar, r_br.n_longest_chain, r_br.n_longest_task, s_by.c_str(), r_br.n_lds_bytes,
 				(s < simt_branches_round_groups.size())? simt_branches_round_groups[s] : 0);
+			if(!r_br.n_bwd_groups)
+				continue;
+			fprintf(stderr, "[setup] stage %zu backward branches: %d split tasks in %d split chunks, %d whole chunks, %d workgroups of two waves, width %d, T* %d, longest chain %d, "
+				"longest task %d; split tasks by (longer bin, join columns):%s; split tasks with three tips or more: %d; segment columns with more than %d blocks: %d; "
+				"columns with two rows outside the task or more: %d; chunks with spare lanes: %d; LDS %d bytes (three table regions of %d entries, two x regions of %d doubles), "
+				"one round holds %d workgroups\n", s, r_br.n_split_tasks, r_br.n_split_chunks, r_br.n_whole_chunks, r_br.n_bwd_groups, n_simt_width, r_br.n_tstar, r_br.n_longest_chain,
+				r_br.n_longest_task, s_by.c_str(), r_br.n_bwd_tip3_tasks, int(SIMT_BWD_AHEAD) + 1, r_br.n_bwd_long_columns, r_br.n_bwd_two_outside_columns, r_br.n_bwd_spare_chunks,
+				r_br.n_bwd_lds_bytes, r_br.n_bwd_tab_region, r_br.n_bwd_x_region, (s < simt_bwd_branches_round_groups.size())? simt_bwd_branches_round_groups[s] : 0);
 		}
 		for(size_t s = 0; s + 1 < lists.simt_chunk_ptr.size(); ++ s) {
 			fprintf(stderr, "[setup] stage %zu: %d tasks -> %d chunks of 64 lanes, %d tasks left to the wave-per-task kernel\n", s,
```

Measured after the change: 628.6 GFLOP/s (median of 6 runs). 1.02x the previous value.
